# johannesschaeufele/CPUPathTrace

Hardware: AMD Instinct MI355X
Metric: Msamples/s (all bounces) (higher is better)
Workload: dtype f32

## Files before the change

cpupathtrace_amd/csrc/pt_api.cpp:

```cpp
#include "pt_host.h"

namespace pth {

thread_local std::string g_last_error;

int fail(int code, const std::string &msg) {
    g_last_error = msg;
    return code;
}

const std::string &last_error() {
    return g_last_error;
}

int device_count_quiet() {
    int n = 0;
    if(hipGetDeviceCount(&n) != hipSuccess) {
        (void)hipGetLastError();
        return 0;
    }
    return n;
}

int check_device(int device) {
// ... 367 lines not shown
            const float *sp = d->sph + 4 * static_cast<size_t>(i);
            spheres[i] = {sp[0], sp[1], sp[2], sp[3]};
            tris[PT_TRI_QUADS * (static_cast<size_t>(d->n_triangles) + 1 + i)] = spheres[i];
            sph_meta[i] = make_uint2(d->sph_material[i], s->sph_obj[i]);
        }
        std::vector<F4> pairs(4 * static_cast<size_t>(flat.n_pairs));
        std::memcpy(pairs.data(), flat.pairs.data(), flat.pairs.size() * sizeof(float));
        PT_HIP(s->pairs.upload(pairs));
        PT_HIP(s->tris.upload(tris));
        PT_HIP(s->tri_shade.upload(shade));
        PT_HIP(s->spheres.upload(spheres));
        PT_HIP(s->sph_meta.upload(sph_meta));
        s->build_ms[1] = ms_since(t_upload);
    }
    const auto t_rest = clock::now();

    std::vector<F4> materials(4 * static_cast<size_t>(d->n_materials));
    for(uint32_t i = 0; i < d->n_materials; i++) {
        const pt_material &m = d->materials[i];
        materials[4 * static_cast<size_t>(i) + 0] = {m.diffuse[0], m.diffuse[1], m.diffuse[2], m.diffuse[3]};
        materials[4 * static_cast<size_t>(i) + 1] = {m.specular[0], m.specular[1], m.specular[2], m.specular[3]};
        materials[4 * static_cast<size_t>(i) + 2] = {m.emission[0], m.emission[1], m.emission[2], m.emission[3]};
        materials[4 * static_cast<size_t>(i) + 3] = {m.ior, from_bits(static_cast<uint32_t>(m.bsdf)), from_bits(static_cast<uint32_t>(m.one_way != 0)), 0.0F};
        if(m.bsdf < PT_BSDF_LAMBERTIAN || m.bsdf > PT_BSDF_MIRROR) {
            return fail(PT_ERR_INVALID, "unknown BSDF kind");
        }
    }
    std::vector<F4> lights(2 * static_cast<size_t>(d->n_point_lights));
    for(uint32_t i = 0; i < d->n_point_lights; i++) {
        const float *p = d->light_pos + 3 * static_cast<size_t>(i);
        const float *c = d->light_spectrum + 4 * static_cast<size_t>(i);
        lights[2 * static_cast<size_t>(i) + 0] = {p[0], p[1], p[2], 0.0F};
        lights[2 * static_cast<size_t>(i) + 1] = {c[0], c[1], c[2], c[3]};
    }

    std::vector<F4> emis;
    std::vector<float> cdf;
    const float pi = static_cast<float>(M_PI);
    for(int32_t obj : dfs) {
        const uint32_t ref = leaf_ref[obj];
        const uint32_t idx = ref & PT_REF_INDEX;
        const bool is_sphere = (ref & PT_REF_SPHERE) != 0;
        const uint32_t mat = is_sphere ? d->sph_material[idx] : d->tri_material[idx];
        if(mat == PT_NO_MATERIAL) {
            continue;
        }
        const float *e = d->materials[mat].emission;
        const float emissive_power = (e[0] + e[1] + e[2]) * e[3];
        if(emissive_power <= 0.0F) {
            continue;
        }
        float area;
        if(is_sphere) {
            const float r = d->sph[4 * static_cast<size_t>(idx) + 3];
            area = 4.0F * pi * (r * r);
        }
        else {
            const float *p = d->tri_pos + 9 * static_cast<size_t>(idx);
            const Vec3 c = cross(sub(ld(p + 3), ld(p)), sub(ld(p + 6), ld(p)));
            area = std::sqrt(dot(c, c)) / 2.0F;
        }
        const float object_probability = emissive_power * area;
        if(object_probability <= 0.0F) {
            continue;
        }
        if(is_sphere) {
            const float *sp = d->sph + 4 * static_cast<size_t>(idx);
            emis.push_back({sp[0], sp[1], sp[2], sp[3]});
            emis.push_back({0.0F, 0.0F, 0.0F, 0.0F});
            emis.push_back({0.0F, from_bits(ref), 0.0F, from_bits(mat)});
        }
        else {
            const float *p = d->tri_pos + 9 * static_cast<size_t>(idx);
            emis.push_back({p[0], p[1], p[2], p[3]});
            emis.push_back({p[4], p[5], p[6], p[7]});
            emis.push_back({p[8], from_bits(ref), from_bits(d->tri_cull[idx] != 0 ? 1U : 0U), from_bits(mat)});
        }
        emis.push_back({e[0], e[1], e[2], e[3]});
        cdf.push_back(object_probability);
        s->emissive_obj.push_back(obj);
    }
    {
        float cumulative_probability = 0.0F;
        for(float &v : cdf) {
            const float probability = v;
            v += cumulative_probability;
            cumulative_probability += probability;
        }
        for(float &v : cdf) {
            v /= cumulative_probability;
        }
    }
    s->n_emissive = static_cast<uint32_t>(cdf.size());
    s->emissive_cdf = cdf;
    const int emissive_object_count = static_cast<int>(cdf.size());
    const int object_sample_count = std::min(2 + static_cast<int>(std::log10(emissive_object_count + 1)), emissive_object_count);
    if(d->n_point_lights + static_cast<uint32_t>(object_sample_count) > PT_MAX_NEE) {
        return fail(PT_ERR_UNSUPPORTED, "more than 32 light samples per path vertex (" + std::to_string(d->n_point_lights) + " point lights + " + std::to_string(object_sample_count) +
                                        " emitter samples): the visibility mask of a path vertex has 32 bits");
    }

    PT_HIP(s->materials.upload(materials));
    PT_HIP(s->lights.upload(lights));
    PT_HIP(s->emis.upload(emis));
    PT_HIP(s->emis_cdf.upload(cdf));

    const uint32_t sphere_base = d->n_triangles + 1U, leaf_count = sphere_base + d->n_spheres, pair_base = (leaf_count + 1U) & ~1U;
    if(static_cast<uint64_t>(pair_base) + n_pairs > PT_REF_INDEX) {
        return fail(PT_ERR_UNSUPPORTED, "too many records for 30-bit references");
    }
    PT_HIP(s->recs.ensure(4 * (static_cast<size_t>(pair_base) + n_pairs)));
    PT_HIP(hipMemcpyAsync(s->recs.ptr, s->tris.ptr, 4 * static_cast<size_t>(leaf_count) * sizeof(F4), hipMemcpyDeviceToDevice, s->stream));
    if(pair_base > leaf_count) {
        PT_HIP(hipMemsetAsync(s->recs.ptr + 4 * static_cast<size_t>(leaf_count), 0, 4 * sizeof(F4), s->stream));
    }
    if(n_pairs > 0) {
        PT_HIP(hipMemcpyAsync(s->recs.ptr + 4 * static_cast<size_t>(pair_base), s->pairs.ptr, 4 * static_cast<size_t>(n_pairs) * sizeof(F4), hipMemcpyDeviceToDevice, s->stream));
        PT_HIP(pt_link_records(s->stream, reinterpret_cast<float4 *>(s->recs.ptr), pair_base, n_pairs, sphere_base));
    }
    PT_HIP(hipStreamSynchronize(s->stream));
    s->tris.release();
    s->pairs.release();
    if(root_ref != PT_REF_NONE) {
        root_ref += (root_ref & PT_REF_LEAF) == 0 ? pair_base : ((root_ref & PT_REF_SPHERE) != 0 ? sphere_base : 0U);
    }

    PtDevScene &dev = s->dev;
    dev.recs = reinterpret_cast<const float4 *>(s->recs.ptr);
    dev.pairs = dev.recs + 4 * static_cast<size_t>(pair_base);
    dev.tris = dev.recs;
    dev.pair_base = pair_base;
    dev.tri_shade = reinterpret_cast<const float4 *>(s->tri_shade.ptr);
    dev.spheres = reinterpret_cast<const float4 *>(s->spheres.ptr);
    dev.sph_meta = s->sph_meta.ptr;
    dev.materials = reinterpret_cast<const float4 *>(s->materials.ptr);
    dev.lights = reinterpret_cast<const float4 *>(s->lights.ptr);
    dev.emis = reinterpret_cast<const float4 *>(s->emis.ptr);
    dev.emis_cdf = s->emis_cdf.ptr;
    for(int k = 0; k < 3; k++) {
        dev.root_lo[k] = root_lo[k];
        dev.root_hi[k] = root_hi[k];
    }
    dev.root_ref = root_ref;
    dev.n_pairs = n_pairs;
    dev.n_tris = d->n_triangles;
    dev.n_spheres = d->n_spheres;
    dev.n_lights = d->n_point_lights;
    dev.n_emis = s->n_emissive;
    dev.n_materials = d->n_materials;
    dev.n_object_samples = static_cast<uint32_t>(object_sample_count);
    const size_t small_bytes = (static_cast<size_t>(n_pairs) + pair_base) * 64;
    const int wide_word = d->n_point_lights + static_cast<uint32_t>(object_sample_count) > 8U ? 1 : 0;
    const size_t other_lds = pt_path_lds_bytes(wide_word, std::min(std::max(env_int("PT_ROWS", 4), 1), PT_MAX_ROWS), 4, 0U, 0U);
    const size_t room = other_lds < 40960 ? 40960 - other_lds : 0;
    if(small_bytes <= static_cast<size_t>(std::max(env_int("PT_LDS_SMALL_BYTES", static_cast<int>(room)), 0)) && env_int("PT_LDS_SMALL", 1) != 0) {
        dev.n_lds_pairs = n_pairs;
        dev.n_lds_tris = d->n_triangles;
    }
    else {
        dev.n_lds_pairs = 0;
        dev.n_lds_tris = 0;
    }

    int rc = setup_path(s.get());
    if(rc != PT_OK) {
        return rc;
    }
    s->build_ms[3] = ms_since(t_rest);
    if(env_int("PT_DEBUG", 0) != 0) {
        std::fprintf(stderr, "[pt] scene build (%s): %u objects, %u pair records, depth %u; host preparation %.1f ms, upload %.1f ms, device tree %.1f ms, rest %.1f ms\n",
                     s->device_built ? "device" : "host", d->n_objects, n_pairs, s->depth, s->build_ms[0], s->build_ms[1], s->build_ms[2], s->build_ms[3]);
    }
    *out = s.release();
    return PT_OK;
}

void pt_scene_destroy(pt_scene *scene) {
    if(scene == nullptr) {
        return;
    }
    (void)hipSetDevice(scene->device);
    if(scene->stream != nullptr) {
        (void)hipStreamSynchronize(scene->stream);
    }
    delete scene;
}

int pt_scene_info(const pt_scene *scene, uint64_t *n_nodes, uint32_t *depth, uint32_t *n_emissive) {
    if(scene == nullptr) {
        return fail(PT_ERR_INVALID, "null scene");
    }
    if(n_nodes != nullptr) {
        *n_nodes = scene->n_nodes;
    }
    if(depth != nullptr) {
        *depth = scene->depth;
    }
    if(n_emissive != nullptr) {
        *n_emissive = scene->n_emissive;
    }
    return PT_OK;
}

int pt_scene_emissive(const pt_scene *scene, int32_t *out_obj, float *out_cdf, uint64_t capacity, uint64_t *n_written) {
    if(scene == nullptr) {
        return fail(PT_ERR_INVALID, "null scene");
    }
    const uint64_t n = std::min<uint64_t>(scene->emissive_obj.size(), capacity);
    for(uint64_t i = 0; i < n; i++) {
        if(out_obj != nullptr) {
            out_obj[i] = scene->emissive_obj[i];
        }
        if(out_cdf != nullptr) {
            out_cdf[i] = scene->emissive_cdf[i];
        }
    }
    if(n_written != nullptr) {
        *n_written = scene->emissive_obj.size();
    }
    return PT_OK;
}

int pt_scene_bvh_dump(const pt_scene *scene, int32_t *out_obj, float *out_box, uint64_t capacity, uint64_t *n_written) {
    if(scene == nullptr || out_obj == nullptr || out_box == nullptr) {
        return fail(PT_ERR_INVALID, "null argument");
    }
    std::vector<int32_t> obj;
    std::vector<ptb::Box> box;
    if(!scene->device_built) {
        ptb::dump_preorder(scene->tree, obj, box);
    }
    else {
        const uint32_t pair_base = scene->dev.pair_base, sphere_base = scene->dev.n_tris + 1U;
        std::vector<F4> pairs(4 * static_cast<size_t>(scene->dev.n_pairs));
        if(hipSetDevice(scene->device) != hipSuccess ||
           hipMemcpy(pairs.data(), scene->dev.pairs, pairs.size() * sizeof(F4), hipMemcpyDeviceToHost) != hipSuccess) {
            return fail(PT_ERR_HIP, "downloading the pair records failed");
        }
        struct Item {
            uint32_t ref;
            ptb::Box box;
        };
        ptb::Box root;
        for(int k = 0; k < 3; k++) {
            root.lo[k] = scene->dev.root_lo[k];
            root.hi[k] = scene->dev.root_hi[k];
        }
        std::vector<Item> stack{{scene->dev.root_ref, root}};
        obj.reserve(scene->n_nodes);
        box.reserve(scene->n_nodes);
        while(!stack.empty()) {
            const Item it = stack.back();
            stack.pop_back();
            box.push_back(it.box);
            if((it.ref & PT_REF_LEAF) != 0) {
                const uint32_t idx = it.ref & PT_REF_INDEX;
                obj.push_back(static_cast<int32_t>((it.ref & PT_REF_SPHERE) != 0 ? scene->sph_obj[idx - sphere_base] : scene->tri_obj[idx]));
            }
            else {
                obj.push_back(-1);
                const float *q = &pairs[4 * static_cast<size_t>(it.ref - pair_base)].x;
                Item l, r;
                std::memcpy(&l.box, q, 24);
                std::memcpy(&r.box, q + 6, 24);
                std::memcpy(&l.ref, q + 12, 4);
                std::memcpy(&r.ref, q + 13, 4);
                stack.push_back(r);
                stack.push_back(l);
            }
        }
    }
    const uint64_t n = std::min<uint64_t>(obj.size(), capacity);
    for(uint64_t i = 0; i < n; i++) {
        out_obj[i] = obj[i];
        std::memcpy(out_box + 6 * i, &box[i], sizeof(float) * 6);
    }
    if(n_written != nullptr) {
        *n_written = obj.size();
    }
    return PT_OK;
}

int pt_intersect_batch(pt_scene *s, const float *rays, size_t n, float *out_t, int32_t *out_obj) {
    if(s == nullptr || (n > 0 && (rays == nullptr || out_t == nullptr || out_obj == nullptr))) {
        return fail(PT_ERR_INVALID, "null argument");
    }
    if(n == 0) {
        return PT_OK;
    }
    if(n > 0x7fffffffULL) {
        return fail(PT_ERR_INVALID, "too many rays in one batch");
    }
    std::lock_guard<std::mutex> lock(s->render_mutex);
    PT_HIP(hipSetDevice(s->device));
    const uint32_t n32 = static_cast<uint32_t>(n);
    {
        int rc = setup_path(s);
        if(rc != PT_OK) {
            return rc;
        }
        PtPathConfig cfg = s->path_cfg;
        PT_HIP(s->batch_rays.ensure(6 * n));
        PT_HIP(s->closest_out.ensure(n));
        PT_HIP(s->path_spill.ensure(((n + 255) / 256) * 256 * cfg.spill_depth));
        cfg.spill = s->path_spill.ptr;
        hipStream_t st = s->stream;
        PT_HIP(hipMemcpyAsync(s->batch_rays.ptr, rays, 6 * n * sizeof(float), hipMemcpyHostToDevice, st));
        pt_launch_closest(st, s->dev, s->batch_rays.ptr, n32, s->closest_out.ptr, cfg);
        PT_HIP(hipGetLastError());
        std::vector<uint2> hits(n);
        PT_HIP(hipMemcpyAsync(hits.data(), s->closest_out.ptr, n * sizeof(uint2), hipMemcpyDeviceToHost, st));
        PT_HIP(hipStreamSynchronize(st));
        for(size_t i = 0; i < n; i++) {
            const float t = from_bits(hits[i].x);
            const uint32_t ref = hits[i].y;
            out_t[i] = t;
            out_obj[i] = (t < 0.0F || ref == PT_REF_NONE) ? -1 : static_cast<int32_t>((ref & PT_REF_SPHERE) ? s->sph_obj[(ref & PT_REF_INDEX) - (s->dev.n_tris + 1U)] : s->tri_obj[ref & PT_REF_INDEX]);
        }
        return PT_OK;
    }
}

}
```

cpupathtrace_amd/csrc/pt_image.cpp:

```cpp
#include "pt_host.h"

using namespace pth;


static int post_check(int device, const float *rgba, int32_t width, int32_t height, uint32_t steps, float gamma) {
    if(width < 0 || height < 0 || (rgba == nullptr && static_cast<long long>(width) * height > 0)) {
        return fail(PT_ERR_INVALID, "bad image");
    }
    if((steps & ~(PT_POST_TONE_MAP | PT_POST_GAMMA)) != 0 || steps == 0) {
        return fail(PT_ERR_INVALID, "steps must be PT_POST_TONE_MAP and/or PT_POST_GAMMA");
    }
    if((steps & PT_POST_GAMMA) != 0 && !(gamma == gamma)) {
        return fail(PT_ERR_INVALID, "gamma is NaN");
    }
    return check_device(device);
}

extern "C" {

int pt_post_process_device(int device, float *d_rgba, int32_t width, int32_t height, uint32_t steps, float gamma, void *stream) {
    PT_TRY(post_check(device, d_rgba, width, height, steps, gamma));
    PT_HIP(hipSetDevice(device));
    static_assert(PT_POST_TONE_MAP == PT_POST_STEP_TONE_MAP && PT_POST_GAMMA == PT_POST_STEP_GAMMA, "step bits");
    PT_HIP(pt_post_run(static_cast<hipStream_t>(stream), reinterpret_cast<float4 *>(d_rgba), width, height, steps, gamma));
    return PT_OK;
}

int pt_post_process(int device, float *rgba, int32_t width, int32_t height, uint32_t steps, float gamma) {
    PT_TRY(post_check(device, rgba, width, height, steps, gamma));
    const size_t count = static_cast<size_t>(width) * static_cast<size_t>(height);
    if(count == 0) {
        return PT_OK;
    }
    PT_HIP(hipSetDevice(device));
    DevBuf<F4> frame;
    PT_HIP(frame.ensure(count));
    PT_HIP(hipMemcpy(frame.ptr, rgba, count * sizeof(F4), hipMemcpyHostToDevice));
    PT_HIP(pt_post_run(nullptr, reinterpret_cast<float4 *>(frame.ptr), width, height, steps, gamma));
    PT_HIP(hipMemcpy(rgba, frame.ptr, count * sizeof(F4), hipMemcpyDeviceToHost));
    return PT_OK;
}

}


static int features_launch(pt_scene *s, const pt_camera_params *camera, const pt_options *options, float4 *d_out) {
    PT_TRY(setup_path(s));
    PtDevCamera cam = derive_camera(camera);
    cam.aperture_kind = PT_APERTURE_NONE;
    PtPathConfig cfg = s->path_cfg;
    const size_t n = static_cast<size_t>(options->image_width) * static_cast<size_t>(options->image_height);
    PT_HIP(s->feature_spill.ensure(((n + 255) / 256) * 256 * cfg.spill_depth));
    cfg.spill = s->feature_spill.ptr;
    pt_launch_features(s->stream, s->dev, cam, options->image_width, options->image_height, d_out, cfg);
    PT_HIP(hipGetLastError());
    return PT_OK;
}

static int features_views_check(pt_scene *s, const pt_camera_params *cameras, int32_t n_views, const pt_options *options, const float *out) {
    if(n_views <= 0) {
        return fail(PT_ERR_INVALID, "a view batch needs at least one view");
    }
    if(options != nullptr && options->image_width > 0 && options->image_height > 0 &&
       static_cast<uint64_t>(n_views) * static_cast<uint64_t>(options->image_height) * static_cast<uint64_t>(options->image_width) > 0x0fffffffULL) {
        return fail(PT_ERR_INVALID, "more than 0x0fffffff pixels");
    }
    PT_TRY(check_render_args(s, cameras, options));
    if(out == nullptr) {
        return fail(PT_ERR_INVALID, "null argument");
    }
    return PT_OK;
}

int pth::features_views_launch(pt_scene *s, const pt_camera_params *cameras, int32_t n_views, const pt_options *options, float4 *d_out) {
    if(n_views == 1) {
        return features_launch(s, cameras, options, d_out);
    }
    PT_TRY(setup_path(s));
    std::vector<PtViewCamera> table(static_cast<size_t>(n_views));
    for(int32_t v = 0; v < n_views; v++) {
        table[static_cast<size_t>(v)] = PtViewCamera{derive_camera(cameras + v), {0, 0, 0}};
        table[static_cast<size_t>(v)].cam.aperture_kind = PT_APERTURE_NONE;
    }
    PT_HIP(s->feature_cams.ensure(table.size()));
    PT_HIP(hipMemcpyAsync(s->feature_cams.ptr, table.data(), table.size() * sizeof(PtViewCamera), hipMemcpyHostToDevice, s->stream));
    PT_HIP(hipStreamSynchronize(s->stream));
    PtPathConfig cfg = s->path_cfg;
    const size_t n = static_cast<size_t>(n_views) * static_cast<size_t>(options->image_width) * static_cast<size_t>(options->image_height);
    PT_HIP(s->feature_spill.ensure(((n + 255) / 256) * 256 * cfg.spill_depth));
    cfg.spill = s->feature_spill.ptr;
    pt_launch_features_views(s->stream, s->dev, s->feature_cams.ptr, n_views, options->image_width, options->image_height, d_out, cfg);
    PT_HIP(hipGetLastError());
    return PT_OK;
}

namespace pth {

DenoiseWorkspace &denoise_workspace(int device) {
    static std::mutex table_mutex;
    static std::vector<DenoiseWorkspace *> table;
    std::lock_guard<std::mutex> lock(table_mutex);
    if(static_cast<size_t>(device) >= table.size()) {
        table.resize(static_cast<size_t>(device) + 1, nullptr);
    }
    if(table[static_cast<size_t>(device)] == nullptr) {
        table[static_cast<size_t>(device)] = new DenoiseWorkspace();
    }
    return *table[static_cast<size_t>(device)];
}

template<typename T>
hipError_t regrow(T **p, size_t count) {
    if(*p != nullptr) {
        hipError_t e = hipFree(*p);
        *p = nullptr;
        if(e != hipSuccess) {
            return e;
        }
    }
    return hipMalloc(reinterpret_cast<void **>(p), std::max<size_t>(count, 1) * sizeof(T));
}

int denoise_ensure(DenoiseWorkspace &ws, size_t n, bool staged) {
    PtDenoiseScratch &d = ws.scratch;
    if(n > ws.pixels) {
        ws.pixels = 0;
        PT_HIP(regrow(&d.col[0], n));
        PT_HIP(regrow(&d.col[1], n));
        PT_HIP(regrow(&d.var[0], n));
        PT_HIP(regrow(&d.var[1], n));
        PT_HIP(regrow(&d.guide, n));
        PT_HIP(regrow(&d.grad, n));
        PT_HIP(regrow(&d.cls, n));
        ws.pixels = n;
    }
    if(staged && n > ws.staged) {
        ws.staged = 0;
        PT_HIP(regrow(&ws.in_rgba, n));
        PT_HIP(regrow(&ws.in_features, 3 * n));
        ws.staged = n;
    }
    return PT_OK;
}

int denoise_params_resolve(const pt_denoise_params *params, PtDenoiseParams *resolved) {
    pt_denoise_params p{};
    pt_denoise_params_default(&p);
    if(params != nullptr) {
        p = *params;
    }
    if(p.iterations < 0 || p.iterations > 10) {
        return fail(PT_ERR_INVALID, "iterations must be 0..10");
    }
    for(float sigma : {p.sigma_luminance, p.sigma_normal, p.sigma_depth}) {
        if(!std::isfinite(sigma) || sigma < 0.0F) {
            return fail(PT_ERR_INVALID, "sigmas must be finite and not negative");
        }
    }
    *resolved = PtDenoiseParams{p.iterations, p.sigma_luminance, p.sigma_normal, p.sigma_depth};
    return PT_OK;
}

int denoise_measured_params_resolve(const pt_denoise_measured_params *params, PtDenoiseParams *resolved, float *sigma_measured) {
    pt_denoise_measured_params p{};
    pt_denoise_measured_params_default(&p);
    if(params != nullptr) {
        p = *params;
    }
    PT_TRY(denoise_params_resolve(&p.base, resolved));
    if(!std::isfinite(p.sigma_measured) || p.sigma_measured < 0.0F) {
        return fail(PT_ERR_INVALID, "sigmas must be finite and not negative");
    }
    *sigma_measured = p.sigma_measured;
    return PT_OK;
}

}

static int denoise_views_check(int device, const void *rgba, const void *features, int32_t width, int32_t height, int32_t n_views, const pt_denoise_params *params,
                               const void *out, PtDenoiseParams *resolved) {
    if(n_views <= 0) {
        return fail(PT_ERR_INVALID, "a view batch needs at least one view");
    }
    if(width > 0 && height > 0 && static_cast<uint64_t>(n_views) * static_cast<uint64_t>(width) * static_cast<uint64_t>(height) > 0x0fffffffULL) {
        return fail(PT_ERR_INVALID, "more than 0x0fffffff pixels");
    }
    if(rgba == nullptr || features == nullptr || out == nullptr) {
        return fail(PT_ERR_INVALID, "null argument");
    }
    if(width <= 0 || height <= 0) {
        return fail(PT_ERR_INVALID, "image size must be positive");
    }
    PtDenoiseParams p{};
    PT_TRY(denoise_params_resolve(params, &p));
    PT_TRY(check_device(device));
    *resolved = p;
    return PT_OK;
}

extern "C" {

int pt_denoise_params_default(pt_denoise_params *out) {
    if(out == nullptr) {
        return fail(PT_ERR_INVALID, "null argument");
    }
    out->iterations = 5;
    out->sigma_luminance = 32.0F;
    out->sigma_normal = 128.0F;
    out->sigma_depth = 1.0F;
    return PT_OK;
}

int pt_render_features(pt_scene *s, const pt_camera_params *camera, const pt_options *options, float *out_features) {
    return pt_render_features_views(s, camera, 1, options, out_features);
}

int pt_render_features_device(pt_scene *s, const pt_camera_params *camera, const pt_options *options, float *d_out_features, void *stream) {
    return pt_render_features_views_device(s, camera, 1, options, d_out_features, stream);
}

int pt_render_features_views(pt_scene *s, const pt_camera_params *cameras, int32_t n_views, const pt_options *options, float *out_features) {
    PT_TRY(features_views_check(s, cameras, n_views, options, out_features));
    const size_t n = static_cast<size_t>(n_views) * static_cast<size_t>(options->image_width) * static_cast<size_t>(options->image_height);
    std::lock_guard<std::mutex> lock(s->render_mutex);
    PT_HIP(hipSetDevice(s->device));
    PT_HIP(s->features.ensure(3 * n));
    PT_TRY(features_views_launch(s, cameras, n_views, options, reinterpret_cast<float4 *>(s->features.ptr)));
    PT_HIP(hipMemcpyAsync(out_features, s->features.ptr, 3 * n * sizeof(F4), hipMemcpyDeviceToHost, s->stream));
    PT_HIP(hipStreamSynchronize(s->stream));
    return PT_OK;
}

int pt_render_features_views_device(pt_scene *s, const pt_camera_params *cameras, int32_t n_views, const pt_options *options, float *d_out_features, void *stream) {
    PT_TRY(features_views_check(s, cameras, n_views, options, d_out_features));
    std::lock_guard<std::mutex> lock(s->render_mutex);
    PT_HIP(hipSetDevice(s->device));
    StreamOrder order;
    PT_TRY(order.begin(stream, s->stream));
    PT_TRY(features_views_launch(s, cameras, n_views, options, reinterpret_cast<float4 *>(d_out_features)));
    PT_TRY(order.end());
    if(order.caller == nullptr) {
        PT_HIP(hipStreamSynchronize(s->stream));
    }
    return PT_OK;
}

int pt_denoise_device(int device, const float *d_rgba, const float *d_features, int32_t width, int32_t height, const pt_denoise_params *params, float *d_out_rgba,
                      void *stream) {
    return pt_denoise_views_device(device, d_rgba, d_features, width, height, 1, params, d_out_rgba, stream);
}

int pt_denoise(int device, const float *rgba, const float *features, int32_t width, int32_t height, const pt_denoise_params *params, float *out_rgba) {
    return pt_denoise_views(device, rgba, features, width, height, 1, params, out_rgba);
}

int pt_denoise_views_device(int device, const float *d_rgba, const float *d_features, int32_t width, int32_t height, int32_t n_views, const pt_denoise_params *params,
                            float *d_out_rgba, void *stream) {
    PtDenoiseParams p{};
    PT_TRY(denoise_views_check(device, d_rgba, d_features, width, height, n_views, params, d_out_rgba, &p));
    const size_t n = static_cast<size_t>(n_views) * static_cast<size_t>(width) * static_cast<size_t>(height);
    DenoiseWorkspace &ws = denoise_workspace(device);
    std::lock_guard<std::mutex> lock(ws.mutex);
    PT_HIP(hipSetDevice(device));
    PT_TRY(denoise_ensure(ws, n, false));
    hipStream_t st = static_cast<hipStream_t>(stream);
    PT_HIP(pt_denoise_views_run(st, reinterpret_cast<const float4 *>(d_rgba), reinterpret_cast<const float4 *>(d_features), nullptr, width, height, n_views, p,
                                ws.scratch, reinterpret_cast<float4 *>(d_out_rgba)));
    PT_HIP(hipStreamSynchronize(st));
    return PT_OK;
}

int pt_denoise_views(int device, const float *rgba, const float *features, int32_t width, int32_t height, int32_t n_views, const pt_denoise_params *params,
                     float *out_rgba) {
    PtDenoiseParams p{};
    PT_TRY(denoise_views_check(device, rgba, features, width, height, n_views, params, out_rgba, &p));
    const size_t n = static_cast<size_t>(n_views) * static_cast<size_t>(width) * static_cast<size_t>(height);
    DenoiseWorkspace &ws = denoise_workspace(device);
    std::lock_guard<std::mutex> lock(ws.mutex);
    PT_HIP(hipSetDevice(device));
    PT_TRY(denoise_ensure(ws, n, true));
    PT_HIP(hipMemcpy(ws.in_rgba, rgba, n * sizeof(F4), hipMemcpyHostToDevice));
    PT_HIP(hipMemcpy(ws.in_features, features, 3 * n * sizeof(F4), hipMemcpyHostToDevice));
    PT_HIP(pt_denoise_views_run(nullptr, ws.in_rgba, ws.in_features, nullptr, width, height, n_views, p, ws.scratch, ws.in_rgba));
    PT_HIP(hipMemcpy(out_rgba, ws.in_rgba, n * sizeof(F4), hipMemcpyDeviceToHost));
    return PT_OK;
}

static int denoise_measured_check(int device, const void *rgba, const void *features, const void *variance, int32_t width, int32_t height,
                                  const pt_denoise_measured_params *params, const void *out, PtDenoiseParams *resolved, float *sigma_measured) {
    if(rgba == nullptr || features == nullptr || variance == nullptr || out == nullptr) {
        return fail(PT_ERR_INVALID, "null argument");
    }
    if(width <= 0 || height <= 0) {
        return fail(PT_ERR_INVALID, "image size must be positive");
    }
    if(static_cast<uint64_t>(width) * static_cast<uint64_t>(height) > 0x0fffffffULL) {
        return fail(PT_ERR_INVALID, "more than 0x0fffffff pixels");
    }
    PT_TRY(denoise_measured_params_resolve(params, resolved, sigma_measured));
    return check_device(device);
}

int pt_denoise_measured_params_default(pt_denoise_measured_params *out) {
    if(out == nullptr) {
        return fail(PT_ERR_INVALID, "null argument");
    }
    pt_denoise_params_default(&out->base);
    out->sigma_measured = 16.0F;
    return PT_OK;
}

int pt_denoise_measured_device(int device, const float *d_rgba, const float *d_features, const float *d_variance, const int32_t *d_mask, int32_t width,
                               int32_t height, const pt_denoise_measured_params *params, float *d_out_rgba, void *stream) {
    PtDenoiseParams p{};
    float sigma_measured = 0.0F;
    PT_TRY(denoise_measured_check(device, d_rgba, d_features, d_variance, width, height, params, d_out_rgba, &p, &sigma_measured));
    const size_t n = static_cast<size_t>(width) * static_cast<size_t>(height);
    DenoiseWorkspace &ws = denoise_workspace(device);
    std::lock_guard<std::mutex> lock(ws.mutex);
    PT_HIP(hipSetDevice(device));
    PT_TRY(denoise_ensure(ws, n, false));
    hipStream_t st = static_cast<hipStream_t>(stream);
    PT_HIP(pt_denoise_measured_run(st, reinterpret_cast<const float4 *>(d_rgba), reinterpret_cast<const float4 *>(d_features),
                                   reinterpret_cast<const float4 *>(d_variance), d_mask, width, height, p, sigma_measured, ws.scratch,
                                   reinterpret_cast<float4 *>(d_out_rgba)));
    PT_HIP(hipStreamSynchronize(st));
    return PT_OK;
}

int pt_denoise_measured(int device, const float *rgba, const float *features, const float *variance, const int32_t *mask, int32_t width, int32_t height,
                        const pt_denoise_measured_params *params, float *out_rgba) {
    PtDenoiseParams p{};
    float sigma_measured = 0.0F;
    PT_TRY(denoise_measured_check(device, rgba, features, variance, width, height, params, out_rgba, &p, &sigma_measured));
    const size_t n = static_cast<size_t>(width) * static_cast<size_t>(height);
    DenoiseWorkspace &ws = denoise_workspace(device);
    std::lock_guard<std::mutex> lock(ws.mutex);
    PT_HIP(hipSetDevice(device));
    PT_TRY(denoise_ensure(ws, n, true));
    if(n > ws.staged_variance) {
        ws.staged_variance = 0;
        PT_HIP(regrow(&ws.in_variance, n));
        ws.staged_variance = n;
    }
    DevBuf<int32_t> d_mask;
    if(mask != nullptr) {
        PT_HIP(d_mask.ensure(n));
        PT_HIP(hipMemcpy(d_mask.ptr, mask, n * sizeof(int32_t), hipMemcpyHostToDevice));
    }
    PT_HIP(hipMemcpy(ws.in_rgba, rgba, n * sizeof(F4), hipMemcpyHostToDevice));
    PT_HIP(hipMemcpy(ws.in_features, features, 3 * n * sizeof(F4), hipMemcpyHostToDevice));
    PT_HIP(hipMemcpy(ws.in_variance, variance, n * sizeof(F4), hipMemcpyHostToDevice));
    PT_HIP(pt_denoise_measured_run(nullptr, ws.in_rgba, ws.in_features, ws.in_variance, mask != nullptr ? d_mask.ptr : nullptr, width, height, p, sigma_measured,
                                   ws.scratch, ws.in_rgba));
    PT_HIP(hipMemcpy(out_rgba, ws.in_rgba, n * sizeof(F4), hipMemcpyDeviceToHost));
    return PT_OK;
}

}


struct pt_temporal {
    int device = 0;
    int32_t width = 0, height = 0;
    PtTemporalParams params{};
    std::mutex mutex;
    DevBuf<float4> col[2], guide, col_hist, pos[2], nrm[2], in_rgba, in_features;
    DevBuf<float> var[2];
    DevBuf<float2> grad, moments[2];
    DevBuf<int32_t> len[2];
    DevBuf<uint32_t> cls[2];
    int cur = 0;
    bool has_prev = false;
    PtDevCamera prev{};
    float prev_rows[3][3] = {};
    PtDevCamera pending{};
    float pending_rows[3][3] = {};
};

namespace {

int temporal_camera(const pt_camera_params *c, int32_t height, PtDevCamera *cam, float rows[3][3], float *footprint) {
    const float scalars[] = {c->origin[0], c->origin[1], c->origin[2], c->look_at[0], c->look_at[1], c->look_at[2], c->up[0], c->up[1], c->up[2],
                             c->focal_length, c->height, c->aspect_ratio};
    for(float v : scalars) {
        if(!std::isfinite(v)) {
            return fail(PT_ERR_INVALID, "camera: non-finite parameter");
        }
    }
    *cam = derive_camera(c);
    const Vec3 f = ld(cam->forward), u = ld(cam->up), r = ld(cam->right);
    Vec3 row[3] = {cross(u, r), cross(r, f), cross(f, u)};
// ... 217 lines not shown
```

cpupathtrace_amd/csrc/pt_kernels.h:

```cpp
#ifndef PT_KERNELS_H
#define PT_KERNELS_H

#include <hip/hip_runtime.h>

#include "pt_types.h"

#define PT_F_DONE 1u
#define PT_F_IN_FLIGHT 2u
#define PT_F_HAS_EXT 4u
#define PT_F_COLLECTED 8u
#define PT_F_PIXEL 16u
#define PT_F_SAFE 64u
#define PT_F_OVERLAP 32u

#define PT_DEST_SHADOW 0x80000000u
#define PT_DEST_NULL 0xffffffffu


#define PT_LDS_TABLE_MAX 16
#define PT_LDS_TABLE_BYTES (PT_LDS_TABLE_MAX * (4 + 64 + 96 + 64))
#define PT_WALK_SAVE_WORDS 17
#define PT_MAX_ROWS 8
#define PT_F_STREAM 128u

#define PT_PLANE_RAY_O 0
#define PT_PLANE_RAY_D 1
#define PT_PLANE_PD 2
#define PT_PLANE_ENGINE 3
#define PT_PLANE_SPECTRUM 4
#define PT_PLANE_OUT 5
#define PT_PLANE_RECT 6
#define PT_SLOT_PLANES 7
struct PtSlots {
    uint32_t total;
    float4 *state;
    float4 *nee;
    uint32_t *nee_mask;
    uint32_t *cost;
    PtEstimator *est;
    PtCandidate *cand;
};

struct PtStreams {
    uint32_t n;
    const int4 *rect;
    uint64_t *rng;
    const int4 *tiles;
    const uint32_t *tile_offset;
    uint32_t n_tiles;
    uint64_t base_seed;
    uint32_t first_total;
    uint32_t first_lanes;
    uint32_t first_shift;
    uint32_t n_waves, first_spread;
    uint32_t tiles_per_row, chunks_per_tile;
    uint32_t *next;
    uint32_t *tile_left;
    uint32_t *tiles_done;
    uint32_t *cost;
    const uint32_t *place;
    const uint32_t *cancel;
    const uint2 *todo;
    const PtParkRecord *park_in;
    PtParkRecord *park_out;
    uint32_t *park_count;
    uint32_t park_cap;
    uint32_t *status;
    int32_t yield_at;
    uint32_t n_views, view_height;
    const PtViewCamera *views;
    const uint64_t *view_seed;
};

struct PtLocalQueue {
    float4 *ray_o;
    float4 *ray_d;
    uint32_t cap;
};

struct PtPathConfig {
    int grid;
    int rows;
    int slots_per_wave;
    int wide;
    int stack_lds;
    uint32_t spill_depth;
    uint2 *spill;
    uint32_t *walk_save;
    size_t lds_bytes;
    int in_lds;
    int refill_idle;
    int min_ready;
    int ready_shift;
    int pass_q_low;
    int early_ready;
    int compact_passes;
    int debug_lanes;
    int burst_steps;
    int first_lanes;
    int leaf_min;
    unsigned long long *wave_counters;
};

struct PtPathArgs {
    PtDevScene sc;
    PtDevCamera cam;
    PtDevOptions opt;
    PtSlots S;
    PtStreams T;
    PtLocalQueue Q;
    int rows, slots_per_wave, refill_idle, min_ready, burst_steps, leaf_min, ready_shift, pass_q_low, early_ready, compact_passes, debug_lanes;
    uint2 *spill;
    uint32_t spill_depth;
    uint32_t save_stride;
    uint32_t *walk_save;
    float4 *image;
    PtDevCounters *counters;
    unsigned long long *wave_counters;
};

void pt_launch_path(hipStream_t stream, const PtDevScene &scene, const PtDevCamera &camera, const PtDevOptions &options, PtSlots slots, PtStreams streams,
                    PtLocalQueue queue, const PtPathConfig &cfg, float4 *image, PtDevCounters *counters, PtPathArgs *host_args, PtPathArgs *d_args);
struct PtNoiseRule {
    PtDevOptions opt;
    float target;
    float floor;
};
int pt_launch_frame_compact(hipStream_t stream, const uint2 *todo, uint32_t n, uint32_t *status, const PtParkRecord *parked, uint2 *todo_out, uint32_t *block_counts,
                            unsigned long long *result, int32_t target, const PtParkRecord *park_in, PtParkRecord *park_out, uint32_t *park_count, uint32_t park_cap,
                            const PtNoiseRule &noise, int resort);
#define PT_NOISE_SUMMARY_WORDS 68
int pt_launch_frame_rate(hipStream_t stream, const uint2 *todo, uint32_t n, const PtParkRecord *park, const int4 *tiles, const uint32_t *tile_offset, uint32_t n_tiles,
                         int32_t width, const PtNoiseRule &noise, uint2 *out, uint32_t *summary);
int pt_launch_frame_noise_base(hipStream_t stream, float *map, const uint8_t *cover, uint32_t n_pixels);
int pt_launch_frame_noise_scatter(hipStream_t stream, const uint2 *rated, uint32_t n, float *map);
int pt_launch_frame_variance(hipStream_t stream, const uint2 *todo, uint32_t n, const PtParkRecord *park, const int4 *tiles, const uint32_t *tile_offset,
                             uint32_t n_tiles, int32_t width, const PtDevOptions &opt, float4 *out_var, int32_t *out_at);
int pt_launch_frame_variance_scatter(hipStream_t stream, const float4 *var, const int32_t *at, uint32_t n, float4 *map);
int pt_launch_frame_gather(hipStream_t stream, const uint2 *todo, uint32_t n, uint32_t n_parked, const PtParkRecord *park, const int4 *tiles,
                           const uint32_t *tile_offset, uint32_t n_tiles, int32_t width, float4 *out_rgba, int2 *out_at);
int pt_launch_frame_preview_base(hipStream_t stream, float4 *view, int32_t *samples, const uint8_t *cover, uint32_t n_pixels);
int pt_launch_frame_scatter(hipStream_t stream, const float4 *rgba, const int2 *at, uint32_t n, float4 *view, int32_t *samples);
int pt_path_blocks_per_cu(const PtPathConfig &cfg);
size_t pt_path_lds_bytes(int wide, int rows, int stack_lds, uint32_t n_lds_pairs, uint32_t n_lds_leaf_records);
int pt_path_stack_lds(int in_lds, size_t lds_bytes_with_default_window);
int pt_launch_replay(hipStream_t stream, const PtDevScene &scene, const PtLocalQueue &Q, uint32_t n_logs, uint32_t parts, int waves_per_simd, const PtPathConfig &cfg,
                     uint2 *spill, unsigned long long *out);
void pt_launch_closest(hipStream_t stream, const PtDevScene &scene, const float *rays6, uint32_t n, uint2 *out, const PtPathConfig &cfg);
void pt_launch_features(hipStream_t stream, const PtDevScene &scene, const PtDevCamera &camera, int32_t width, int32_t height, float4 *out, const PtPathConfig &cfg);
void pt_launch_features_views(hipStream_t stream, const PtDevScene &scene, const PtViewCamera *views, int32_t n_views, int32_t width, int32_t height, float4 *out,
                              const PtPathConfig &cfg);
void pt_launch_steptime(hipStream_t stream, const PtDevScene &scene, const float *rays6, uint32_t n, uint32_t lanes_per_wave, uint4 *out, uint2 *spill, uint32_t spill_depth, int flags);


#endif
```

cpupathtrace_amd/csrc/pt_path.hip:

```cpp
#include <type_traits>

#include "pt_device.h"
#include "pt_kernels.h"
#include "pt_shading.h"

using namespace ptd;

namespace {

typedef float f4v __attribute__((ext_vector_type(4)));
typedef float f2v __attribute__((ext_vector_type(2)));
typedef unsigned int u2v __attribute__((ext_vector_type(2)));
typedef const f4v __attribute__((address_space(3))) *lds_f4_cptr;
typedef const f4v __attribute__((address_space(1))) *glb_f4_cptr;
typedef u2v __attribute__((address_space(3))) *lds_u2_ptr;
typedef u2v __attribute__((address_space(1))) *glb_u2_ptr;
typedef unsigned int __attribute__((address_space(3))) *lds_u32_ptr;
typedef const PtPathArgs __attribute__((address_space(4))) *args_c4;

template<bool IN_LDS>
struct RecPtr {
    typedef glb_f4_cptr type;
};
template<>
struct RecPtr<true> {
    typedef lds_f4_cptr type;
};

PT_D float4 to_f4(f4v v) {
    return make_float4(v.x, v.y, v.z, v.w);
}

struct RootBox {
    float lo[3], hi[3];
    uint32_t ref;
};

#define PT_REF_POPPING 0xfffffffeu
struct Walk {
    V3 o, d, inv;
    f2v o_xy, o_zx, o_yz, i_xy, i_zx, i_yz;
    float thr;
    uint32_t dest;
    float best_t;
    uint32_t best_ref;
    float t_max;
    float t_lim;
    uint32_t cur;
    uint32_t sp;
    bool occluded;

    PT_D void pack() {
        o_xy = (f2v){o.x, o.y};
        o_zx = (f2v){o.z, o.x};
        o_yz = (f2v){o.y, o.z};
        i_xy = (f2v){inv.x, inv.y};
        i_zx = (f2v){inv.z, inv.x};
        i_yz = (f2v){inv.y, inv.z};
    }
    PT_D void set_t_max(float t) {
        t_max = t;
        t_lim = t > 0.0f ? __uint_as_float(__float_as_uint(t) - 1u) : -1.0f;
    }
};

#ifdef PT_STEP_STAMPS
#define PT_STAMP(k)                                                      \
    do {                                                                 \
        const unsigned long long now_ = __builtin_amdgcn_s_memtime();     \
        asm volatile("s_waitcnt lgkmcnt(0)" ::: "memory");               \
        stamp_acc[k] += now_ - stamp_last;                               \
        stamp_last = now_;                                               \
    } while(0)
#else
#define PT_STAMP(k) do { } while(0)
#endif

template<int STACK_LDS, bool IN_LDS>
struct Tracer {
    static_assert((STACK_LDS & (STACK_LDS - 1)) == 0, "the stack window is indexed with a mask");
#ifdef PT_STEP_STAMPS
    mutable unsigned long long stamp_acc[8] = {0, 0, 0, 0, 0, 0, 0, 0}, stamp_last = 0;
#endif
    typedef typename RecPtr<IN_LDS>::type rec_ptr;
    rec_ptr recs;
    lds_u2_ptr stack_l;
    glb_u2_ptr my_spill;

    struct Rec {
        f4v r0, r1, r2, r3;
    };
    PT_D void fetch(uint32_t cur, Rec &R) const {
        rec_ptr p = recs + 4 * (size_t)(cur & PT_REF_INDEX);
        R.r0 = p[0];
        R.r1 = p[1];
        R.r2 = p[2];
        R.r3 = p[3];
    }
    static PT_D void whole(const Rec &R) {
        asm volatile("" ::"v"(R.r0), "v"(R.r1), "v"(R.r2), "v"(R.r3));
    }

    static PT_D unsigned long long node_lanes(uint32_t cur) { return __builtin_amdgcn_uicmp(cur, 0x40000000u, 36); }
    static PT_D unsigned long long slow_lanes(uint32_t cur) { return __builtin_amdgcn_uicmp(cur + 1u, 0x40000000u, 34); }

    PT_D void start(Walk &w, Rec &R, const RootBox &root, float4 ro, float4 rd) const {
        w.o = v3(ro.x, ro.y, ro.z);
        w.d = v3(rd.x, rd.y, rd.z);
        w.thr = ro.w;
        w.dest = __float_as_uint(rd.w);
        w.inv = slab_inverse(w.d);
        w.pack();
        w.best_ref = PT_REF_NONE;
        w.best_t = -1.0f;
        w.set_t_max(FLT_MAX);
        uint32_t sent_ref, sent_t;
        asm volatile("v_mov_b32 %0, -1\n\tv_mov_b32 %1, -1.0" : "=v"(sent_ref), "=v"(sent_t));
        const u2v sentinel = {sent_ref, sent_t};
        stack_l[0] = sentinel;
        w.sp = 1;
        w.occluded = false;
        w.cur = PT_REF_NONE;
        if(root.ref != PT_REF_NONE) {
            const float t_root = slab_walk(ld3(root.lo), ld3(root.hi), w.o, w.inv);
            if(t_root >= 0.0f) {
                w.cur = root.ref;
                fetch(w.cur, R);
            }
        }
    }

    PT_D void node_step(Walk &w, Rec &R, unsigned long long node_mask, unsigned long long deep_mask) const {
        if(!__builtin_amdgcn_inverse_ballot_w64(node_mask)) {
            return;
        }
#ifdef PT_STEP_STAMPS
        asm volatile("s_waitcnt vmcnt(0)" ::: "memory");
#endif
        PT_STAMP(2);
        whole(R);
        const f4v q0 = R.r0, q1 = R.r1, q2 = R.r2;
        const uint32_t sp = w.sp;
        const u2v top = stack_l[((sp - 1u) & (uint32_t)(STACK_LDS - 1)) * 256u];
        const f2v a0 = ((f2v){q0.x, q0.y} - w.o_xy) * w.i_xy;
        const f2v a1 = ((f2v){q0.z, q0.w} - w.o_zx) * w.i_zx;
        const f2v a2 = ((f2v){q1.x, q1.y} - w.o_yz) * w.i_yz;
        const f2v a3 = ((f2v){q1.z, q1.w} - w.o_xy) * w.i_xy;
        const f2v a4 = ((f2v){q2.x, q2.y} - w.o_zx) * w.i_zx;
        const f2v a5 = ((f2v){q2.z, q2.w} - w.o_yz) * w.i_yz;
        const float l1 = a0.x, l2 = a1.y, l3 = a0.y, l4 = a2.x, l5 = a1.x, l6 = a2.y;
        const float r1 = a3.x, r2 = a4.y, r3 = a3.y, r4 = a5.x, r5 = a4.x, r6 = a5.y;
        const float l_min = __builtin_fmaxf(__builtin_fmaxf(__builtin_fminf(l1, l2), __builtin_fminf(l3, l4)), __builtin_fminf(l5, l6));
        const float l_max = __builtin_fminf(__builtin_fminf(__builtin_fmaxf(l1, l2), __builtin_fmaxf(l3, l4)), __builtin_fmaxf(l5, l6));
        const float r_min = __builtin_fmaxf(__builtin_fmaxf(__builtin_fminf(r1, r2), __builtin_fminf(r3, r4)), __builtin_fminf(r5, r6));
        const float r_max = __builtin_fminf(__builtin_fminf(__builtin_fmaxf(r1, r2), __builtin_fmaxf(r3, r4)), __builtin_fmaxf(r5, r6));
        const float left_t = __builtin_fmaxf(l_min, 0.0f), right_t = __builtin_fmaxf(r_min, 0.0f);
        const float inf = __builtin_inff();
        const float t_lim = w.t_lim;
        const float tl = left_t <= __builtin_fminf(l_max, t_lim) ? left_t : inf;
        const float tr = right_t <= __builtin_fminf(r_max, t_lim) ? right_t : inf;
        const bool left_first = tl < tr;
        const uint32_t left_ref = __float_as_uint(R.r3.x), right_ref = __float_as_uint(R.r3.y);
        const uint32_t near_ref = left_first ? left_ref : right_ref;
        const float near_t = __builtin_fminf(tl, tr), far_t = __builtin_fmaxf(tl, tr);
        const u2v far = {left_first ? right_ref : left_ref, __float_as_uint(far_t)};
        const bool both = far_t < inf, entered = near_t < inf;
        const uint32_t slot = (sp & (uint32_t)(STACK_LDS - 1)) * 256u;
        if(deep_mask == 0ULL) {
            stack_l[slot] = far;
        }
        else if(both) {
            if(sp >= (uint32_t)STACK_LDS) {
                my_spill[sp - STACK_LDS] = stack_l[slot];
            }
            stack_l[slot] = far;
        }
        const uint32_t popped = __uint_as_float(top.y) <= t_lim ? top.x : PT_REF_POPPING;
        const uint32_t next = entered ? near_ref : popped;
        w.sp = entered ? sp + (both ? 1u : 0u) : sp - 1u;
        w.cur = next;
        asm volatile("" ::"v"(w.sp), "v"(w.cur));
        PT_STAMP(3);
        if(next < PT_REF_POPPING) {
            fetch(next, R);
        }
        if(deep_mask != 0ULL) {
            if(!entered & (sp - 1u >= (uint32_t)STACK_LDS)) {
                stack_l[((sp - 1u) & (uint32_t)(STACK_LDS - 1)) * 256u] = my_spill[sp - 1u - STACK_LDS];
            }
        }
        PT_STAMP(4);
    }

    PT_D void slow_step(Walk &w, Rec &R, unsigned long long leaf_mask, uint32_t &n_leaves) const {
        uint32_t cur = w.cur;
        bool need_pop = cur == PT_REF_POPPING;
        bool moved = false;
        if(leaf_mask != 0ULL) {
            n_leaves += (uint32_t)__popcll(leaf_mask);
            if(__builtin_amdgcn_inverse_ballot_w64(leaf_mask)) {
                const float4 q0 = to_f4(R.r0), q1 = to_f4(R.r1), q2 = to_f4(R.r2);
                float t_leaf;
                if(cur & PT_REF_SPHERE) {
                    t_leaf = sphere_intersect(v3(q0.x, q0.y, q0.z), q0.w, w.o, w.d);
                }
                else {
                    const TriRec tr = tri_unpack(q0, q1, q2);
                    t_leaf = tri_intersect(tr.a, tr.ab, tr.ac, (tr.obj_cull >> 31) != 0, w.o, w.d);
                }
                need_pop = true;
                if(t_leaf >= 0.0f) {
                    if((w.dest & PT_DEST_SHADOW) && t_leaf < w.thr) {
                        w.occluded = true;
                        need_pop = false;
                    }
                    else {
                        if(w.best_ref == PT_REF_NONE || !(w.best_t < t_leaf)) {
                            w.best_t = t_leaf;
                            w.best_ref = cur;
                        }
                        w.set_t_max(fmin_std(w.t_max, t_leaf));
                    }
                }
                cur = PT_REF_NONE;
            }
        }
        if(__ballot(need_pop) != 0ULL) {
            uint32_t sp = w.sp;
            const float t_max = w.t_max;
            while(__ballot(need_pop) != 0ULL) {
                if(need_pop) {
                    sp--;
                    const uint32_t slot = (sp & (uint32_t)(STACK_LDS - 1)) * 256u;
                    const u2v e = stack_l[slot];
                    if(sp >= (uint32_t)STACK_LDS) {
                        stack_l[slot] = my_spill[sp - STACK_LDS];
                    }
                    if(__uint_as_float(e.y) < t_max) {
                        cur = e.x;
                        need_pop = false;
                        moved = true;
                    }
                }
            }
            w.sp = sp;
        }
        w.cur = cur;
        if(moved & (cur != PT_REF_NONE)) {
            fetch(cur, R);
        }
    }

    PT_D bool step(Walk &w, Rec &R, int leaf_min, uint32_t &n_nodes, uint32_t &n_leaves) const {
        PT_STAMP(0);
        PT_STAMP(7);
        const unsigned long long nodes = node_lanes(w.cur), slow = slow_lanes(w.cur);
        if((nodes | slow) == 0ULL) {
            return false;
        }
        PT_STAMP(1);
        if(nodes != 0ULL) {
            n_nodes += (uint32_t)__popcll(nodes);
            node_step(w, R, nodes, nodes & __builtin_amdgcn_uicmp(w.sp, (uint32_t)STACK_LDS, 35));
        }
        PT_STAMP(5);
        if(slow != 0ULL && (nodes == 0ULL || __popcll(slow) >= leaf_min)) {
            slow_step(w, R, slow & __builtin_amdgcn_uicmp(w.cur, PT_REF_POPPING, 36), n_leaves);
        }
        PT_STAMP(6);
        return true;
    }
};

template<bool WIDE>
struct SlotWord {
    typedef uint32_t T;
    typedef uint32_t __attribute__((address_space(3))) *lds_ptr;
    static constexpr uint32_t j_mask = 7u;
    static PT_D uint32_t vis(T w) { return w & 0xffu; }
    static PT_D uint32_t pending(T w) { return (w >> 8) & 0xffu; }
    static PT_D uint32_t flags(T w) { return (w >> 16) & 0xffu; }
    static PT_D T one_ray() { return 0x100u; }
    static PT_D T make(uint32_t flags, uint32_t rays, uint32_t vis, uint32_t waiting) { return (waiting << 24) | (flags << 16) | (rays << 8) | vis; }
    static PT_D uint32_t waiting(T w, const PtSlots &, size_t) { return w >> 24; }
    static PT_D void keep_waiting(const PtSlots &, size_t, uint32_t) {}
};
template<>
struct SlotWord<true> {
    typedef unsigned long long T;
    typedef unsigned long long __attribute__((address_space(3))) *lds_ptr;
    static constexpr uint32_t j_mask = 31u;
    static PT_D uint32_t vis(T w) { return (uint32_t)w; }
    static PT_D uint32_t pending(T w) { return (uint32_t)(w >> 32) & 0xffu; }
    static PT_D uint32_t flags(T w) { return (uint32_t)(w >> 40) & 0xffu; }
    static PT_D T one_ray() { return 1ULL << 32; }
    static PT_D T make(uint32_t flags, uint32_t rays, uint32_t vis, uint32_t) { return ((T)flags << 40) | ((T)rays << 32) | (T)vis; }
    static PT_D uint32_t waiting(T, const PtSlots &S, size_t p) { return S.nee_mask[p]; }
    static PT_D void keep_waiting(const PtSlots &S, size_t p, uint32_t mask) { S.nee_mask[p] = mask; }
};

#define PT_F_VIEW_RAY 256u
#define PT_DEST_SLOT_MASK 0xffffu
#define PT_NO_SLOT 0xffffffffu
#define PT_DEST_J_SHIFT 16

struct WaveCtx {
    uint32_t q_head;
    uint32_t q_count;
    uint32_t n_dead;
    bool pool_empty;
    uint32_t first_rows;
    uint32_t first_base;
    uint32_t wave;
};

PT_D void tile_stream(const PtStreams &T, uint32_t i, int4 &rect, uint64_t &rng, uint32_t &tile) {
    uint32_t lo = 0, hi = T.n_tiles;
    while(hi - lo > 1) {
        const uint32_t mid = (lo + hi) / 2;
        if(T.tile_offset[mid] <= i) {
            lo = mid;
        }
        else {
            hi = mid;
        }
    }
    const int4 t = T.tiles[lo];
    const uint32_t k = i - T.tile_offset[lo];
    const int32_t x = t.x + (int32_t)(k % (uint32_t)t.z), y = t.y + (int32_t)(k / (uint32_t)t.z);
    rect = make_int4(x, y, 1, 1);
    uint64_t base_seed = T.base_seed;
    int32_t seed_y = y;
    if(T.n_views > 1) {
        const uint32_t view = (uint32_t)y / T.view_height;
        base_seed = T.view_seed[view];
        seed_y = y - (int32_t)(view * T.view_height);
    }
    const uint64_t seed = pixel_seed(base_seed, x, seed_y);
    rng = seed ^ (~seed << 32);
    tile = lo;
}

struct EmisLds {
    const float __attribute__((address_space(3))) *cdf_l;
    lds_f4_cptr rec_l;
    lds_f4_cptr light_l;
    PT_D float cdf(int i) const { return cdf_l[i]; }
    PT_D float4 rec(int i, int k) const { return to_f4(rec_l[4 * i + k]); }
    PT_D V3 tri_normal_at(int i, uint32_t, V3 pos) const {
        uint32_t mat_unused;
        return tri_shade_normal(light_l + 6 * i, pos, mat_unused);
    }
};
struct ShadeTables {
    EmisLds emis;
    lds_f4_cptr materials_l;
    bool emis_in_lds, materials_in_lds;
};

PT_D void copy_words(void *dst, const void *src, uint32_t n) {
    uint32_t *d = static_cast<uint32_t *>(dst);
    const uint32_t *s = static_cast<const uint32_t *>(src);
#pragma unroll 1
    for(uint32_t i = 0; i < n; i++) {
        d[i] = s[i];
    }
}

PT_D uint32_t closed_candidate_words(int32_t n_candidates) {
    return (uint32_t)(n_candidates < PT_MAX_CANDIDATES ? n_candidates : PT_MAX_CANDIDATES) * (uint32_t)(sizeof(PtCandidate) / 4);
}

PT_D void park_stream(const PtStreams &T, const PtSlots &S, uint32_t p, uint32_t stream, uint64_t rng, int32_t cursor, bool have_pixel) {
    uint32_t status = PT_STREAM_FINISHED;
    if(have_pixel) {
        status = PT_STREAM_UNTOUCHED;
        const PtEstimator *e = S.est + p;
        if(e->pixel_sample > 0 || cursor > 0) {
            const uint32_t k = atomicAdd(T.park_count, 1u);
            if(k < T.park_cap) {
                PtParkRecord *rec = T.park_out + k;
                rec->stream = stream;
                rec->cursor = cursor;
                rec->rng[0] = (uint32_t)rng;
                rec->rng[1] = (uint32_t)(rng >> 32);
                copy_words(&rec->est, e, (uint32_t)(sizeof(PtEstimator) / 4));
                copy_words(rec->cand, S.cand + (size_t)p * PT_MAX_CANDIDATES, closed_candidate_words(e->n_candidates));
                status = PT_STREAM_PARKED + k;
            }
        }
    }
    T.status[stream] = status;
}

template<typename V>
PT_D V *slot_plane(const PtSlots &S, uint32_t k, uint32_t p) {
    return reinterpret_cast<V *>(reinterpret_cast<char *>(S.state) + (k * S.total + p) * (uint32_t)sizeof(float4));
}

template<bool WIDE>
PT_D void shade_row(const PtDevScene &sc, const PtDevCamera &cam, const PtDevOptions &opt, const PtSlots &S, const PtStreams &T, const PtLocalQueue &Q,
                    WaveCtx &ctx, uint32_t row, uint32_t ls_in, uint32_t lane, uint32_t slot_base, size_t queue_base, typename SlotWord<WIDE>::lds_ptr word_l, lds_u2_ptr hit_l,
                    float4 *__restrict__ image, PtDevCounters *counters, const ShadeTables &tb, bool stop, uint32_t &n_samples, uint32_t &n_vertices) {
    const bool have_slot = ls_in != PT_NO_SLOT;
    const uint32_t ls = have_slot ? ls_in : 0u;
    const uint32_t p = slot_base + ls;
    const unsigned long long lt = (1ULL << lane) - 1ULL;
    const uint32_t n_light_samples = sc.n_lights + sc.n_object_samples;
    typedef SlotWord<WIDE> SW;
    const typename SW::T word = word_l[ls];
    uint32_t flags = SW::flags(word);
    const uint32_t vis_bits = SW::vis(word);
    bool ready = have_slot && !(flags & PT_F_DONE) && SW::pending(word) == 0;
    if(__ballot(ready) == 0ULL) {
        return;
    }

    {
        const bool want = ready && !(flags & PT_F_STREAM);
        const unsigned long long want_mask = __ballot(want);
        if(want_mask != 0ULL) {
            uint32_t base = T.n;
            uint32_t mine;
            if((ctx.first_rows >> row) & 1u) {
                ctx.first_rows &= ~(1u << row);
                base = ctx.first_base + row * 64u;
                mine = base + lane;
                if(T.place != nullptr) {
                    base = 0;
                    mine = T.place[ctx.first_base + ls];
                }
                else if(T.first_spread) {
                    const uint32_t g = T.first_lanes, q = row * (64u / g) + lane / g;
                    uint32_t chunk = q * T.n_waves + ctx.wave;
                    if(T.tiles_per_row != 0) {
                        const uint32_t per_tile = T.chunks_per_tile * (64u / g), pieces = (T.first_total / T.n_waves) / g;
                        const uint32_t tile = chunk / per_tile, sub = chunk % per_tile;
                        const uint32_t step = T.tiles_per_row >= pieces ? T.tiles_per_row / pieces : 1u;
                        const uint32_t tx = (tile % T.tiles_per_row + q * T.first_shift * step) % T.tiles_per_row, ty = tile / T.tiles_per_row;
                        chunk = (ty * T.tiles_per_row + tx) * per_tile + sub;
                    }
                    base = 0;
                    mine = chunk * g + lane % g;
                }
            }
            else {
                ctx.pool_empty = ctx.pool_empty || stop;
                if(!ctx.pool_empty) {
                    if(lane == 0) {
                        base = T.first_total + atomicAdd(T.next, (uint32_t)__popcll(want_mask));
                    }
                    base = __builtin_amdgcn_readfirstlane(base);
                }
                mine = base + (uint32_t)__popcll(want_mask & lt);
                if(base >= T.n || base + (uint32_t)__popcll(want_mask) > T.n) {
                    ctx.pool_empty = true;
                }
            }
            const bool got = want && base < T.n && mine < T.n;
            if(got) {
                int4 rc;
                uint64_t r;
                uint32_t tile = 0;
                uint32_t park = PT_NO_PARK;
                int32_t cursor0 = 0;
                if(T.rect != nullptr) {
                    rc = T.rect[mine];
                    r = T.rng[mine];
                }
                else {
                    if(T.todo != nullptr) {
                        const uint2 entry = T.todo[mine];
                        mine = entry.x;
                        park = entry.y;
                    }
                    tile_stream(T, mine, rc, r, tile);
                }
                flags = PT_F_STREAM;
                if(park != PT_NO_PARK) {
                    const PtParkRecord *rec = T.park_in + park;
                    r = (uint64_t)rec->rng[0] | ((uint64_t)rec->rng[1] << 32);
                    cursor0 = rec->cursor;
                    copy_words(S.est + p, &rec->est, (uint32_t)(sizeof(PtEstimator) / 4));
                    copy_words(S.cand + (size_t)p * PT_MAX_CANDIDATES, rec->cand, closed_candidate_words(rec->est.n_candidates));
                    flags = PT_F_STREAM | PT_F_PIXEL | (estimator_safe_to_overlap(S.est[p], opt) ? PT_F_SAFE : 0u);
                }
                *slot_plane<int4>(S, PT_PLANE_RECT, p) = rc;
                *slot_plane<uint4>(S, PT_PLANE_ENGINE, p) = make_uint4((uint32_t)r, (uint32_t)(r >> 32), (uint32_t)cursor0, mine);
                if(T.cost != nullptr) {
                    __hip_atomic_store(&S.cost[p], 0u, __ATOMIC_RELAXED, __HIP_MEMORY_SCOPE_AGENT);
                }
            }
            else if(want) {
                flags = PT_F_DONE;
                ready = false;
                word_l[ls] = SW::make(PT_F_DONE, 0u, 0u, 0u);
            }
            ctx.n_dead += (uint32_t)__popcll(__ballot(want && !got));
        }
    }
    const bool alive = ready;
    uint32_t lane_samples = 0;

    uint64_t rng = 0;
    C4 out = c4(0, 0, 0, 0), spectrum = c4(1, 1, 1, 1);
    V3 ro = v3(0, 0, 0), rd = v3(0, 0, 1);
    float contribution_unweighted = 1.0f;
    double divisor = 1.0, bounce_pd = 1.0;
    int path_length = 0;
    bool shade_vertex = false;
    bool start_sample = false;
    float hit_t = -1.0f;
    uint32_t hit_ref = PT_REF_NONE;
    int4 rect = make_int4(0, 0, 0, 0);
    int32_t cursor = 0;
    uint32_t stream = 0;
    bool stream_finished = false;
    bool stream_abandoned = false;

    if(alive) {
        const uint4 engine = *slot_plane<uint4>(S, PT_PLANE_ENGINE, p);
        rng = (uint64_t)engine.x | ((uint64_t)engine.y << 32);
        cursor = (int32_t)engine.z;
        stream = engine.w;
        rect = *slot_plane<int4>(S, PT_PLANE_RECT, p);
        if(flags & PT_F_IN_FLIGHT) {
            const float4 out4 = *slot_plane<float4>(S, PT_PLANE_OUT, p);
            uint32_t mask = SW::waiting(word, S, p);
            const uint32_t lit = mask & vis_bits;
            float4 nee0 = make_float4(0, 0, 0, 0), nee1 = make_float4(0, 0, 0, 0);
            if(lit & 1u) {
                nee0 = S.nee[p];
            }
            if(lit & 2u) {
                nee1 = S.nee[S.total + p];
            }
            const float4 o4 = *slot_plane<float4>(S, PT_PLANE_RAY_O, p), d4 = *slot_plane<float4>(S, PT_PLANE_RAY_D, p);
            const float4 spectrum4 = *slot_plane<float4>(S, PT_PLANE_SPECTRUM, p);
            const double2 pd_in = *slot_plane<double2>(S, PT_PLANE_PD, p);
            uint32_t warm = 0;
            if(flags & PT_F_HAS_EXT) {
                const u2v h = hit_l[ls];
                hit_t = __uint_as_float(h.x);
                hit_ref = h.y;
                if(!(hit_t < 0.0f) && !(hit_ref & PT_REF_SPHERE)) {
                    warm = *reinterpret_cast<const uint32_t *>(sc.tri_shade + 8 * (size_t)(hit_ref & PT_REF_INDEX));
                }
            }
            out = c4(out4);
            if(lit & 1u) {
                out = out + c4(nee0);
            }
            if(lit & 2u) {
                out = out + c4(nee1);
            }
            mask >>= 2;
            for(uint32_t j = 2; mask != 0; j++, mask >>= 1) {
                if((mask & 1u) && ((vis_bits >> j) & 1u)) {
                    out = out + c4(S.nee[(size_t)j * S.total + p]);
                }
            }
            asm volatile("" ::"v"(warm));
            if(flags & PT_F_OVERLAP) {
                PtEstimator e = S.est[p];
                out.a = 1.0f;
// ... 33 lines not shown
                flags &= ~(PT_F_IN_FLIGHT | PT_F_HAS_EXT | PT_F_COLLECTED | PT_F_SAFE);
                if((flags & PT_F_PIXEL) && estimator_safe_to_overlap(e, opt)) {
                    flags |= PT_F_SAFE;
                }
                start_sample = true;
            }
            else {
                ro = v3(o4.x, o4.y, o4.z);
                rd = v3(d4.x, d4.y, d4.z);
                contribution_unweighted = o4.w;
                spectrum = c4(spectrum4);
                divisor = pd_in.x;
                bounce_pd = pd_in.y;
                path_length = __float_as_int(d4.w);
            }
        }
        else {
            start_sample = true;
        }
    }

    bool emit_ext = false;
    Ray ext;
    ext.o = v3(0, 0, 0);
    ext.d = v3(0, 0, 1);
    auto shoot_camera = [&](const int4 rc, int32_t cur) {
        const int32_t px = rc.x + cur % rc.z, py = rc.y + cur / rc.z;
        const float one_half = 1.0f / 2.0f;
        const float x_camera = 2 * (((float)px + one_half) / (float)opt.image_width - one_half);
        float y_camera = 2 * (((float)py + one_half) / (float)opt.image_height - one_half);
        y_camera = -y_camera;
        return camera_shoot(cam, x_camera, y_camera, opt.pixel_width, opt.pixel_height, rng);
    };
    const bool batch = T.n_views > 1;
    if(start_sample) {
        bool have_pixel = false;
        while(cursor < rect.z * rect.w) {
            if(!(flags & PT_F_PIXEL)) {
                PtEstimator e;
                estimator_reset(e, opt);
                S.est[p] = e;
                flags = (flags | PT_F_PIXEL) & ~PT_F_SAFE;
                if(estimator_safe_to_overlap(e, opt)) {
                    flags |= PT_F_SAFE;
                }
                if(opt.max_sample_count <= 0) {
                    const int32_t px = rect.x + cursor % rect.z, py = rect.y + cursor / rect.z;
                    image[(size_t)py * opt.image_width + px] = make_float4(0.0f, 0.0f, 0.0f, 0.0f);
                    cursor++;
                    flags &= ~PT_F_PIXEL;
                    continue;
                }
            }
            have_pixel = true;
            break;
        }
        const bool yield = T.yield_at != 0 && have_pixel && S.est[p].pixel_sample >= T.yield_at;
        if(!have_pixel || stop || yield) {
            stream_finished = !have_pixel;
            stream_abandoned = have_pixel;
            if(T.status != nullptr) {
                park_stream(T, S, p, stream, rng, cursor, have_pixel);
            }
            flags = 0;
        }
        else {
            if(batch) {
                flags |= PT_F_VIEW_RAY;
                ext.o = v3(0, 0, 0);
                ext.d = v3(0, 0, 1);
            }
            else {
                ext = shoot_camera(rect, cursor);
            }
            emit_ext = true;
            out = c4(0, 0, 0, 0);
            spectrum = c4(1, 1, 1, 1);
            contribution_unweighted = 1.0f;
            divisor = 1.0;
            bounce_pd = 1.0;
            path_length = 0;
            flags |= PT_F_IN_FLIGHT | PT_F_HAS_EXT;
        }
    }
    {
        const unsigned long long fin_mask = __ballot(stream_finished);
        if(fin_mask != 0ULL) {
            if(stream_finished) {
                const uint32_t si = stream;
                if(T.rng != nullptr) {
                    T.rng[si] = rng;
                }
                if(T.cost != nullptr) {
                    T.cost[si] = __hip_atomic_load(&S.cost[p], __ATOMIC_RELAXED, __HIP_MEMORY_SCOPE_AGENT);
                }
                if(T.tile_left != nullptr) {
                    int4 rc_unused;
                    uint64_t r_unused;
                    uint32_t tile = 0;
                    tile_stream(T, si, rc_unused, r_unused, tile);
                    if(atomicSub(&T.tile_left[tile], 1u) == 1u) {
                        __hip_atomic_fetch_add(T.tiles_done, 1u, __ATOMIC_RELAXED, __HIP_MEMORY_SCOPE_SYSTEM);
                    }
                }
            }
            if(lane == 0) {
                atomicAdd(&counters->streams_done, (unsigned long long)__popcll(fin_mask));
            }
        }
        if(stop || T.yield_at != 0) {
            const unsigned long long drop_mask = __ballot(stream_abandoned);
            if(lane == 0 && drop_mask != 0ULL) {
                atomicAdd(&counters->streams_abandoned, (unsigned long long)__popcll(drop_mask));
            }
        }
    }

    V3 pos = v3(0, 0, 0), n = v3(0, 1, 0);
    Material mat;
    mat.bsdf = 0;
    bool do_bounce = false;
    float bounce_probability = 1.0f;
    bool want_nee = false;
    bool safe_overlap = false;
    if(shade_vertex) {
        path_length++;
        flags |= PT_F_COLLECTED;
        pos = ro + rd * hit_t;
        uint32_t material_index;
        n = object_normal(sc, hit_ref, pos, material_index);
        mat = tb.materials_in_lds ? material_load(tb.materials_l, material_index) : material_load(sc.materials, material_index);

        out = out + (spectrum * mat.emission) / (float)(divisor * bounce_pd);

        bounce_probability = path_length <= 4 ? 1.0f : 0.1f + 0.1f * fmin_std(contribution_unweighted * get_contribution(spectrum), 1.0f);
        do_bounce = rng_uniform01(rng) < bounce_probability;
        want_nee = mat.bsdf == 0 && n_light_samples > 0;
        safe_overlap = (flags & PT_F_SAFE) != 0 && !stop;
        emit_ext = do_bounce || safe_overlap;
    }

    uint32_t tail = ctx.q_head + ctx.q_count;
    const unsigned long long ext_mask = __ballot(emit_ext);
    const uint32_t ext_pos = tail + (uint32_t)__popcll(ext_mask & lt);
    tail += (uint32_t)__popcll(ext_mask);
    ctx.q_count += (uint32_t)__popcll(ext_mask);
    auto ring = [&](uint32_t i) -> size_t { return queue_base + (i >= Q.cap ? i - Q.cap : i); };

    uint32_t nee_out_mask = 0;
    uint32_t vis_init = 0;
    uint32_t n_rays = 0;
    const float epsilon = opt.epsilon;
    for(uint32_t j = 0; j < n_light_samples; j++) {
        bool need_ray = false;
        float4 so = make_float4(0, 0, 0, 0), sd = make_float4(0, 0, 0, 0);
        if(shade_vertex) {
            V3 light_pos;
            C4 light_spectrum;
            float lpd;
            bool valid;
            if(j < sc.n_lights) {
                const float4 lp = sc.lights[2 * j];
                light_pos = v3(lp.x, lp.y, lp.z);
                light_spectrum = c4(sc.lights[2 * j + 1]);
                lpd = 1.0f;
                valid = true;
            }
            else {
                valid = tb.emis_in_lds ? sample_emissive(sc, tb.emis, pos, rng, light_pos, light_spectrum, lpd)
                                       : sample_emissive(sc, EmisGlobal{sc}, pos, rng, light_pos, light_spectrum, lpd);
            }
            if(valid && want_nee) {
                const V3 to_light = light_pos - pos;
                const V3 light_dir = normalize(to_light);
                float shading_factor, shadow_ray_pd;
                const C4 base_spectrum = bsdf_spectrum(mat, rd, light_dir, n, light_spectrum, true, shading_factor, shadow_ray_pd);
                if(shadow_ray_pd > 0.0f) {
                    const C4 combined = (base_spectrum * shading_factor) * spectrum;
                    const C4 weighed = combined / (float)(divisor * bounce_pd * lpd * shadow_ray_pd);
                    if(!(weighed.r == 0.0f && weighed.g == 0.0f && weighed.b == 0.0f)) {
                        S.nee[(size_t)j * S.total + p] = f4(weighed);
                        nee_out_mask |= 1u << j;
                        const float threshold = len(to_light) - epsilon;
                        if(threshold <= 0.0f) {
                            vis_init |= 1u << j;
                        }
                        else {
                            need_ray = true;
                            const V3 o2 = pos + light_dir * epsilon;
                            so = make_float4(o2.x, o2.y, o2.z, threshold);
                            sd = make_float4(light_dir.x, light_dir.y, light_dir.z, __uint_as_float(PT_DEST_SHADOW | (j << PT_DEST_J_SHIFT) | ls));
                        }
                    }
                }
            }
        }
        const unsigned long long ray_mask = __ballot(need_ray);
        if(ray_mask != 0ULL) {
            if(need_ray) {
                const size_t at = ring(tail + (uint32_t)__popcll(ray_mask & lt));
                Q.ray_o[at] = so;
                Q.ray_d[at] = sd;
                n_rays++;
            }
            tail += (uint32_t)__popcll(ray_mask);
            ctx.q_count += (uint32_t)__popcll(ray_mask);
        }
    }

    if(shade_vertex) {
        bool cancel_ext = false;
        if(!do_bounce) {
        }
        else {
            bounce_pd *= bounce_probability;
            if(bounce_pd <= 1E-20) {
                cancel_ext = true;
            }
            else {
                float ray_factor, ray_pd;
                const Ray next_ray = bsdf_propagate(mat, rd, pos, n, epsilon, rng, ray_factor, ray_pd);
                divisor *= ray_pd;
                divisor /= ray_factor;
                contribution_unweighted *= ray_factor;
                float shading_factor, shading_pd;
                const C4 shaded = bsdf_spectrum(mat, rd, next_ray.d, n, spectrum, false, shading_factor, shading_pd);
                divisor *= shading_pd;
                divisor /= shading_factor;
                contribution_unweighted *= shading_factor;
                spectrum = shaded;
                if(divisor <= 1E-20) {
                    cancel_ext = true;
                }
                else {
                    ext = next_ray;
                }
            }
        }
        const bool path_ends = !do_bounce || cancel_ext;
        if(path_ends && safe_overlap) {
            if(batch) {
                flags |= PT_F_VIEW_RAY;
                ext.o = v3(0, 0, 0);
                ext.d = v3(0, 0, 1);
            }
            else {
                ext = shoot_camera(rect, cursor);
            }
            spectrum = c4(1, 1, 1, 1);
            contribution_unweighted = 1.0f;
            divisor = 1.0;
            bounce_pd = 1.0;
            path_length = 0;
            flags |= PT_F_OVERLAP;
        }
        else if(path_ends && emit_ext) {
            Q.ray_d[ring(ext_pos)] = make_float4(0.0f, 0.0f, 0.0f, __uint_as_float(PT_DEST_NULL));
            emit_ext = false;
        }
        if(emit_ext) {
            flags |= PT_F_HAS_EXT;
        }
        else {
            flags &= ~PT_F_HAS_EXT;
        }
    }

    if(flags & PT_F_VIEW_RAY) {
        flags &= ~PT_F_VIEW_RAY;
        const int32_t px = rect.x + cursor % rect.z, row = rect.y + cursor / rect.z;
        const uint32_t view = (uint32_t)row / (uint32_t)opt.image_height;
        const int32_t py = row - (int32_t)(view * (uint32_t)opt.image_height);
        const float one_half = 1.0f / 2.0f;
        const float x_camera = 2 * (((float)px + one_half) / (float)opt.image_width - one_half);
        float y_camera = 2 * (((float)py + one_half) / (float)opt.image_height - one_half);
        y_camera = -y_camera;
        ext = camera_shoot_lane(T.views[view].cam, x_camera, y_camera, opt.pixel_width, opt.pixel_height, rng);
    }

    if(emit_ext) {
        const size_t at = ring(ext_pos);
        Q.ray_o[at] = make_float4(ext.o.x, ext.o.y, ext.o.z, 0.0f);
        Q.ray_d[at] = make_float4(ext.d.x, ext.d.y, ext.d.z, __uint_as_float(ls));
        n_rays++;
    }
    if(alive) {
        word_l[ls] = SW::make(flags, n_rays, vis_init, nee_out_mask);
        SW::keep_waiting(S, p, nee_out_mask);
        *slot_plane<uint3>(S, PT_PLANE_ENGINE, p) = make_uint3((uint32_t)rng, (uint32_t)(rng >> 32), (uint32_t)cursor);
        if(flags & PT_F_IN_FLIGHT) {
            *slot_plane<float4>(S, PT_PLANE_RAY_O, p) = make_float4(ext.o.x, ext.o.y, ext.o.z, contribution_unweighted);
            *slot_plane<float4>(S, PT_PLANE_RAY_D, p) = make_float4(ext.d.x, ext.d.y, ext.d.z, __int_as_float(path_length));
            *slot_plane<float4>(S, PT_PLANE_SPECTRUM, p) = f4(spectrum);
            *slot_plane<float4>(S, PT_PLANE_OUT, p) = f4(out);
            *slot_plane<double2>(S, PT_PLANE_PD, p) = make_double2(divisor, bounce_pd);
        }
    }
    n_samples += (uint32_t)__popcll(__ballot(lane_samples & 1u)) + 2u * (uint32_t)__popcll(__ballot((lane_samples & 2u) != 0u));
    n_vertices += (uint32_t)__popcll(__ballot(shade_vertex));
}


#define PT_PATH_STACK_LDS 8
#define PT_PATH_STACK_LDS_SMALL 4
#ifndef PT_COST_LDS_BYTES
#define PT_COST_LDS_BYTES 1024
#endif
#ifndef PT_PATH_WAVES
#define PT_PATH_WAVES 4
#endif

PT_D uint32_t lane_afresh() {
    uint32_t l;
    asm volatile("v_mbcnt_lo_u32_b32 %0, -1, 0\n\tv_mbcnt_hi_u32_b32 %0, -1, %0" : "=v"(l));
    return l;
}

template<bool WIDE, bool IN_LDS, int STACK_LDS>
__global__ __launch_bounds__(256, PT_PATH_WAVES) void pt_path_kernel(const PtPathArgs *__restrict__ args) {
    typedef SlotWord<WIDE> SW;
    const args_c4 A4 = (args_c4)args;
    const PtPathArgs *A = (const PtPathArgs *)A4;
    const int rows = A->rows, slots_per_wave = A->slots_per_wave, refill_idle = A->refill_idle, min_ready = A->min_ready, burst_steps = A->burst_steps,
              leaf_min = A->leaf_min, ready_shift = A->ready_shift, pass_q_low = A->early_ready > 0 ? A->pass_q_low : 0, early_ready = A->early_ready;
    const unsigned long long lane_cap = A->debug_lanes >= 64 ? ~0ULL : ((1ULL << A->debug_lanes) - 1ULL);
    PtLocalQueue Q = A->Q;
    RootBox root;
    root.ref = A->sc.root_ref;
    for(int k = 0; k < 3; k++) {
        root.lo[k] = A->sc.root_lo[k];
        root.hi[k] = A->sc.root_hi[k];
    }
    extern __shared__ __align__(16) unsigned char lds_raw[];
    const int tid = threadIdx.x;
    uint32_t lane = (uint32_t)tid & 63u;
    const uint32_t wave_in_block = __builtin_amdgcn_readfirstlane((uint32_t)tid >> 6);
    const uint32_t wave = blockIdx.x * 4u + wave_in_block;
    const uint32_t n_slots = (uint32_t)rows * 64u;
    unsigned char *at = lds_raw;
    const lds_u2_ptr stack_base = (lds_u2_ptr)reinterpret_cast<uint2 *>(at) + wave_in_block * 64u;
    at += (size_t)STACK_LDS * 256 * sizeof(uint2);
    lds_u2_ptr hit_l = (lds_u2_ptr)reinterpret_cast<uint2 *>(at) + wave_in_block * n_slots;
    at += (size_t)4 * n_slots * sizeof(uint2);
    typename SW::lds_ptr word_l = (typename SW::lds_ptr)reinterpret_cast<typename SW::T *>(at) + wave_in_block * n_slots;
    at += (size_t)4 * n_slots * sizeof(typename SW::T);
    float *cdf_l = reinterpret_cast<float *>(at);
    at += (size_t)PT_LDS_TABLE_MAX * sizeof(float);
    float4 *emis_l = reinterpret_cast<float4 *>(at);
    at += (size_t)PT_LDS_TABLE_MAX * 4 * sizeof(float4);
    float4 *light_l = reinterpret_cast<float4 *>(at);
    at += (size_t)PT_LDS_TABLE_MAX * 6 * sizeof(float4);
    float4 *materials_l = reinterpret_cast<float4 *>(at);
    at += (size_t)PT_LDS_TABLE_MAX * 4 * sizeof(float4);
    typedef uint32_t __attribute__((address_space(3))) *lds_u32_ptr;
    const lds_u32_ptr born_base = (lds_u32_ptr)reinterpret_cast<uint32_t *>(at) + wave_in_block * 64u;
    lds_u32_ptr born_l = born_base + lane;
    typedef unsigned char __attribute__((address_space(3))) *lds_u8_ptr;
    lds_u8_ptr list_l = (lds_u8_ptr)reinterpret_cast<unsigned char *>(at) + wave_in_block * 256u;
    at += (size_t)PT_COST_LDS_BYTES;
    float4 *lds_recs = reinterpret_cast<float4 *>(at);
    const bool cost_on = PT_COST_LDS_BYTES != 0 && A->T.cost != nullptr;
    uint32_t *const slot_cost = A->S.cost;

    ShadeTables tb;
    tb.emis.cdf_l = (const float __attribute__((address_space(3))) *)cdf_l;
    tb.emis.rec_l = (lds_f4_cptr)emis_l;
    tb.emis.light_l = (lds_f4_cptr)light_l;
    tb.materials_l = (lds_f4_cptr)materials_l;
    {
        const uint32_t n_emis = A->sc.n_emis, n_materials = A->sc.n_materials;
        tb.emis_in_lds = n_emis > 0 && n_emis <= PT_LDS_TABLE_MAX;
        tb.materials_in_lds = n_materials > 0 && n_materials <= PT_LDS_TABLE_MAX;
        if(tb.emis_in_lds) {
            const float4 *src_emis = A->sc.emis, *src_shade = A->sc.tri_shade;
            const float *src_cdf = A->sc.emis_cdf;
            for(uint32_t i = tid; i < n_emis; i += 256) {
                cdf_l[i] = src_cdf[i];
            }
            for(uint32_t i = tid; i < 4 * n_emis; i += 256) {
                emis_l[i] = src_emis[i];
            }
            for(uint32_t i = tid; i < 6 * n_emis; i += 256) {
                const uint32_t ref = __float_as_uint(src_emis[4 * (i / 6) + 2].y);
                light_l[i] = (ref & PT_REF_SPHERE) ? make_float4(0, 0, 0, 0) : src_shade[8 * (size_t)(ref & PT_REF_INDEX) + i % 6];
            }
        }
        if(tb.materials_in_lds) {
            const float4 *src_materials = A->sc.materials;
            for(uint32_t i = tid; i < 4 * n_materials; i += 256) {
                materials_l[i] = src_materials[i];
            }
        }
    }

    if(IN_LDS) {
        const uint32_t n_lds_quads = 4u * (A->sc.pair_base + A->sc.n_pairs);
        const float4 *src_recs = A->sc.recs;
        for(uint32_t i = tid; i < n_lds_quads; i += 256) {
            lds_recs[i] = src_recs[i];
        }
    }
    for(uint32_t i = lane; i < n_slots; i += 64) {
        word_l[i] = i < (uint32_t)slots_per_wave ? (typename SW::T)0 : SW::make(PT_F_DONE, 0u, 0u, 0u);
    }
    __syncthreads();

    Tracer<STACK_LDS, IN_LDS> tr;
    if(IN_LDS) {
        tr.recs = (typename RecPtr<IN_LDS>::type)(lds_f4_cptr)lds_recs;
    }
    else {
        tr.recs = (typename RecPtr<IN_LDS>::type)(glb_f4_cptr)A->sc.recs;
    }
    auto bind_lane = [&](const PtPathArgs *B, uint32_t l) {
        lane = l;
        tr.stack_l = stack_base + l;
        tr.my_spill = (glb_u2_ptr)(B->spill + ((size_t)wave * 64 + l) * B->spill_depth);
        born_l = born_base + l;
    };

    const size_t slot_base = (size_t)wave * n_slots;
    const size_t queue_base = (size_t)wave * Q.cap;
    WaveCtx ctx;
    ctx.q_head = 0;
    ctx.q_count = 0;
    ctx.n_dead = n_slots - (uint32_t)slots_per_wave;
    ctx.pool_empty = false;
    ctx.first_rows = (1u << rows) - 1u;
    ctx.first_base = wave * (uint32_t)slots_per_wave;
    ctx.wave = wave;

    bool active = false;
    Walk w;
    w.o = v3(0, 0, 0);
    w.d = v3(0, 0, 1);
    w.inv = v3(0, 0, 0);
    w.pack();
    w.thr = 0.0f;
    w.dest = 0;
    w.best_t = 0.0f;
    w.best_ref = PT_REF_NONE;
    w.set_t_max(FLT_MAX);
    w.cur = PT_REF_NONE;
    w.sp = 0;
    w.occluded = false;
    typename Tracer<STACK_LDS, IN_LDS>::Rec rec;
    rec.r0 = rec.r1 = rec.r2 = rec.r3 = (f4v){0.0f, 0.0f, 0.0f, 0.0f};
    float4 win_o = make_float4(0, 0, 0, 0), win_d = make_float4(0, 0, 0, __uint_as_float(PT_DEST_NULL));
    uint32_t n_nodes = 0, n_leaves = 0, n_rays = 0, n_shadow = 0, n_samples = 0, n_vertices = 0;
    uint32_t w_steps = 0, w_passes = 0;
#ifdef PT_PATH_TIMING
    unsigned long long t_shade = 0, t_burst = 0;
    const unsigned long long t_begin = __builtin_amdgcn_s_memtime();
#endif

    bool want_pass = false;
    for(;;) {
        if(want_pass) {
            want_pass = false;
            w_passes++;
#ifdef PT_PATH_TIMING
            const unsigned long long t_pass = __builtin_amdgcn_s_memtime();
#endif
            size_t pass_offset = 0;
            asm volatile("" : "+s"(pass_offset));
            const PtPathArgs *P = (const PtPathArgs *)(args_c4)((const char __attribute__((address_space(4))) *)A4 + pass_offset);
            uint32_t *const walk_save = P->walk_save;
            const size_t save_stride = P->save_stride;
            const uint32_t lane_s = lane_afresh();

            {
                uint32_t *sv = walk_save + (size_t)wave * 64 + lane_s;
                const size_t st = save_stride;
                sv[0 * st] = __float_as_uint(w.o.x);
                sv[1 * st] = __float_as_uint(w.o.y);
                sv[2 * st] = __float_as_uint(w.o.z);
                sv[3 * st] = __float_as_uint(w.d.x);
                sv[4 * st] = __float_as_uint(w.d.y);
                sv[5 * st] = __float_as_uint(w.d.z);
                sv[6 * st] = __float_as_uint(w.thr);
                sv[7 * st] = w.dest;
                sv[8 * st] = __float_as_uint(w.best_t);
                sv[9 * st] = w.best_ref;
                sv[10 * st] = __float_as_uint(w.t_max);
                sv[11 * st] = w.cur;
                sv[12 * st] = w.sp | (w.occluded ? 0x80000000u : 0u);
                sv[13 * st] = n_nodes;
                sv[14 * st] = n_leaves;
                sv[15 * st] = n_rays;
                sv[16 * st] = n_shadow;
            }
            uint32_t n_listed = 0;
            bool compact = false;
            if(PT_COST_LDS_BYTES >= 1024 && !cost_on && P->compact_passes != 0 && rows > 1 && rows <= 4 && ctx.first_rows == 0u) {
                uint32_t rows_used = 0;
                for(uint32_t r = 0; r < (uint32_t)rows; r++) {
                    const typename SW::T word = word_l[r * 64 + lane_s];
                    const bool is_ready = !(SW::flags(word) & PT_F_DONE) && SW::pending(word) == 0;
                    const unsigned long long m = __ballot(is_ready);
                    if(is_ready) {
                        list_l[n_listed + (uint32_t)__popcll(m & ((1ULL << lane_s) - 1ULL))] = (unsigned char)(r * 64 + lane_s);
                    }
                    n_listed += (uint32_t)__popcll(m);
                    rows_used += m != 0ULL ? 1u : 0u;
                }
                compact = (n_listed + 63u) / 64u < rows_used;
                __builtin_amdgcn_fence(__ATOMIC_ACQ_REL, "workgroup");
            }
            const uint32_t n_chunks = compact ? (n_listed + 63u) / 64u : (uint32_t)rows;
            uint32_t stop_word = 0;
            if(P->T.cancel != nullptr) {
                stop_word = __hip_atomic_load(P->T.cancel, __ATOMIC_RELAXED, __HIP_MEMORY_SCOPE_SYSTEM);
            }
            const bool stop = __builtin_amdgcn_readfirstlane(stop_word) != 0u;
#pragma unroll 1
            for(uint32_t k = 0; k < n_chunks; k++) {
                uint32_t ls = k * 64u + lane_s;
                if(compact) {
                    ls = ls < n_listed ? (uint32_t)list_l[ls] : PT_NO_SLOT;
                }
                shade_row<WIDE>(P->sc, P->cam, P->opt, P->S, P->T, P->Q, ctx, k, ls, lane_s, (uint32_t)slot_base, queue_base, word_l, hit_l, P->image, P->counters, tb, stop, n_samples, n_vertices);
            }
            __builtin_amdgcn_fence(__ATOMIC_ACQ_REL, "workgroup");
            __builtin_amdgcn_s_waitcnt(0);
            {
                asm volatile("" : "+s"(pass_offset));
                const PtPathArgs *R = (const PtPathArgs *)(args_c4)((const char __attribute__((address_space(4))) *)A4 + pass_offset);
                const uint32_t *sv = R->walk_save + (size_t)wave * 64 + lane_afresh();
                const size_t st = R->save_stride;
                w.o = v3(__uint_as_float(sv[0 * st]), __uint_as_float(sv[1 * st]), __uint_as_float(sv[2 * st]));
                w.d = v3(__uint_as_float(sv[3 * st]), __uint_as_float(sv[4 * st]), __uint_as_float(sv[5 * st]));
                w.inv = slab_inverse(w.d);
                w.pack();
                w.thr = __uint_as_float(sv[6 * st]);
                w.dest = sv[7 * st];
                w.best_t = __uint_as_float(sv[8 * st]);
                w.best_ref = sv[9 * st];
                w.set_t_max(__uint_as_float(sv[10 * st]));
                w.cur = sv[11 * st];
                const uint32_t packed = sv[12 * st];
                w.sp = packed & 0x7fffffffu;
                w.occluded = (packed >> 31) != 0;
                n_nodes = sv[13 * st];
                n_leaves = sv[14 * st];
                n_rays = sv[15 * st];
                n_shadow = sv[16 * st];
            }
#ifdef PT_PATH_TIMING
            t_shade += __builtin_amdgcn_s_memtime() - t_pass;
#endif
            win_o = make_float4(0, 0, 0, 0);
            win_d = make_float4(0, 0, 0, __uint_as_float(PT_DEST_NULL));
            const uint32_t lane_w = lane_afresh();
            if(lane_w < ctx.q_count) {
                uint32_t i = ctx.q_head + lane_w;
                i = i >= Q.cap ? i - Q.cap : i;
                win_o = Q.ray_o[queue_base + i];
                win_d = Q.ray_d[queue_base + i];
            }
            rec.r0 = rec.r1 = rec.r2 = rec.r3 = (f4v){0.0f, 0.0f, 0.0f, 0.0f};
                    if(active && w.cur < PT_REF_POPPING) {
                tr.fetch(w.cur, rec);
            }
        }

        {
            size_t bind_offset = 0;
            asm volatile("" : "+s"(bind_offset));
            bind_lane((const PtPathArgs *)(args_c4)((const char __attribute__((address_space(4))) *)A4 + bind_offset), lane_afresh());
        }
        bool finished = false;
        for(;;) {
            if(active && w.cur == PT_REF_NONE) {
                const uint32_t ls = w.dest & PT_DEST_SLOT_MASK;
                if(w.dest & PT_DEST_SHADOW) {
                    const uint32_t j = (w.dest >> PT_DEST_J_SHIFT) & SW::j_mask;
                    __hip_atomic_fetch_add(&word_l[ls], (typename SW::T)(w.occluded ? 0u : (1u << j)) - SW::one_ray(), __ATOMIC_RELAXED, __HIP_MEMORY_SCOPE_WORKGROUP);
                }
                else {
                    const u2v h = {__float_as_uint(w.best_ref == PT_REF_NONE ? -1.0f : w.best_t), w.best_ref};
                    hit_l[ls] = h;
                    __hip_atomic_fetch_add(&word_l[ls], (typename SW::T)0 - SW::one_ray(), __ATOMIC_RELAXED, __HIP_MEMORY_SCOPE_WORKGROUP);
                }
                if(cost_on) {
                    __hip_atomic_fetch_add(&slot_cost[slot_base + ls], w_steps - *born_l, __ATOMIC_RELAXED, __HIP_MEMORY_SCOPE_AGENT);
                }
                active = false;
            }

            const unsigned long long idle_mask = __ballot(!active) & lane_cap;
            const uint32_t n_idle = (uint32_t)__popcll(idle_mask);
            if(n_idle >= (uint32_t)refill_idle) {
                if(ctx.q_count <= (uint32_t)pass_q_low && ctx.n_dead < n_slots) {
                    uint32_t n_ready = 0;
                    for(uint32_t r = 0; r < (uint32_t)rows; r++) {
                        const typename SW::T word = word_l[r * 64 + lane];
                        n_ready += (uint32_t)__popcll(__ballot(!(SW::flags(word) & PT_F_DONE) && SW::pending(word) == 0));
                    }
                    const uint32_t live_share = (n_slots - ctx.n_dead) >> ready_shift;
                    const uint32_t need = live_share < (uint32_t)min_ready ? (live_share > 1u ? live_share : 1u) : (uint32_t)min_ready;
                    if(ctx.q_count == 0 ? (n_ready >= need || n_idle == (uint32_t)__popcll(lane_cap)) : n_ready >= (uint32_t)early_ready) {
                        want_pass = true;
                        break;
                    }
                }
                if(ctx.q_count > 0) {
                    const uint32_t take = ctx.q_count < n_idle ? ctx.q_count : n_idle;
                    const uint32_t rank = (uint32_t)__popcll(idle_mask & ((1ULL << lane) - 1ULL));
                    const int src = (int)(rank & 63u);
                    auto from = [src](float v) { return __int_as_float(__builtin_amdgcn_ds_bpermute(src << 2, __float_as_int(v))); };
                    const float4 ro = make_float4(from(win_o.x), from(win_o.y), from(win_o.z), from(win_o.w));
                    const float4 rd = make_float4(from(win_d.x), from(win_d.y), from(win_d.z), from(win_d.w));
                    if(!active && rank < take && __float_as_uint(rd.w) != PT_DEST_NULL) {
                        tr.start(w, rec, root, ro, rd);
                        if(cost_on) {
                            *born_l = w_steps;
                        }
                        active = true;
                        n_rays++;
                        n_shadow += (w.dest & PT_DEST_SHADOW) ? 1u : 0u;
                    }
                    ctx.q_head += take;
                    ctx.q_head = ctx.q_head >= Q.cap ? ctx.q_head - Q.cap : ctx.q_head;
                    ctx.q_count -= take;
                    if(lane < ctx.q_count) {
                        uint32_t i = ctx.q_head + lane;
                        i = i >= Q.cap ? i - Q.cap : i;
                        win_o = Q.ray_o[queue_base + i];
                        win_d = Q.ray_d[queue_base + i];
                    }
                }
            }
            if(__ballot(active) == 0ULL) {
                if(ctx.q_count == 0 && ctx.n_dead >= n_slots) {
                    finished = true;
                    break;
                }
                continue;
            }

#ifdef PT_PATH_TIMING
            const unsigned long long t_b0 = __builtin_amdgcn_s_memtime();
#endif
#pragma unroll 1
            for(int burst = 0; burst < burst_steps; burst++) {
                w_steps++;
                if(!tr.step(w, rec, leaf_min, n_nodes, n_leaves)) {
                    w_steps--;
                    break;
                }
            }
#ifdef PT_PATH_TIMING
            t_burst += __builtin_amdgcn_s_memtime() - t_b0;
#endif
        }
        if(finished) {
            break;
        }
    }

    for(int off = 32; off > 0; off >>= 1) {
        n_rays += __shfl_down(n_rays, off);
        n_shadow += __shfl_down(n_shadow, off);
    }
    if(lane == 0) {
        unsigned long long *slot = A->wave_counters + 8 * (size_t)wave;
        slot[0] += n_nodes;
        slot[1] += n_leaves;
        slot[2] += n_rays;
        slot[3] += n_shadow;
        slot[4] += w_steps;
        slot[5] += w_passes;
        slot[6] += n_samples;
        slot[7] += n_vertices;
#ifdef PT_PATH_TIMING
        slot[5] = (unsigned long long)w_passes | ((t_shade >> 10) << 32);
        slot[4] = (unsigned long long)w_steps | ((t_burst >> 10) << 32);
        slot[3] = (unsigned long long)n_shadow | (((__builtin_amdgcn_s_memtime() - t_begin) >> 10) << 32);
#endif
    }
}

template<int STACK_LDS, bool IN_LDS>
__global__ __launch_bounds__(256) void pt_closest_kernel(PtDevScene sc, const float *__restrict__ rays6, uint32_t n, uint2 *__restrict__ out, uint2 *__restrict__ spill,
                                                         uint32_t spill_depth) {
    extern __shared__ __align__(16) unsigned char lds_raw[];
    const int tid = threadIdx.x;
    lds_u2_ptr stack_l = (lds_u2_ptr)reinterpret_cast<uint2 *>(lds_raw) + tid;
    float4 *lds_recs = reinterpret_cast<float4 *>(lds_raw + (size_t)STACK_LDS * 256 * sizeof(uint2));
    if(IN_LDS) {
        for(uint32_t i = tid; i < 4u * (sc.pair_base + sc.n_pairs); i += 256) {
            lds_recs[i] = sc.recs[i];
        }
        __syncthreads();
    }
    Tracer<STACK_LDS, IN_LDS> tr;
    if(IN_LDS) {
        tr.recs = (typename RecPtr<IN_LDS>::type)(lds_f4_cptr)lds_recs;
    }
    else {
        tr.recs = (typename RecPtr<IN_LDS>::type)(glb_f4_cptr)sc.recs;
    }
    tr.stack_l = stack_l;
    const size_t gid = (size_t)blockIdx.x * 256 + tid;
    tr.my_spill = (glb_u2_ptr)(spill + gid * spill_depth);
    if(gid >= n) {
        return;
    }
    const float *r = rays6 + 6 * gid;
    Walk w;
    typename Tracer<STACK_LDS, IN_LDS>::Rec rec;
    rec.r0 = rec.r1 = rec.r2 = rec.r3 = (f4v){0.0f, 0.0f, 0.0f, 0.0f};
    RootBox root;
    root.ref = sc.root_ref;
    for(int k = 0; k < 3; k++) {
        root.lo[k] = sc.root_lo[k];
        root.hi[k] = sc.root_hi[k];
    }
    tr.start(w, rec, root, make_float4(r[0], r[1], r[2], 0.0f), make_float4(r[3], r[4], r[5], __uint_as_float(0u)));
    uint32_t n_nodes = 0, n_leaves = 0;
    while(tr.step(w, rec, 1, n_nodes, n_leaves)) {
    }
    out[gid] = make_uint2(__float_as_uint(w.best_ref == PT_REF_NONE ? -1.0f : w.best_t), w.best_ref);
}

template<int STACK_LDS, bool IN_LDS, bool kViews>
__global__ __launch_bounds__(256) void pt_feature_kernel(PtDevScene sc, PtDevCamera cam, int32_t width, int32_t height, float4 *__restrict__ out, uint2 *__restrict__ spill,
                                                         uint32_t spill_depth, const PtViewCamera *__restrict__ views, int32_t view_height) {
    extern __shared__ __align__(16) unsigned char lds_raw[];
    const int tid = threadIdx.x;
    lds_u2_ptr stack_l = (lds_u2_ptr)reinterpret_cast<uint2 *>(lds_raw) + tid;
    float4 *lds_recs = reinterpret_cast<float4 *>(lds_raw + (size_t)STACK_LDS * 256 * sizeof(uint2));
    if(IN_LDS) {
        for(uint32_t i = tid; i < 4u * (sc.pair_base + sc.n_pairs); i += 256) {
            lds_recs[i] = sc.recs[i];
        }
        __syncthreads();
    }
    Tracer<STACK_LDS, IN_LDS> tr;
    if(IN_LDS) {
        tr.recs = (typename RecPtr<IN_LDS>::type)(lds_f4_cptr)lds_recs;
    }
    else {
        tr.recs = (typename RecPtr<IN_LDS>::type)(glb_f4_cptr)sc.recs;
    }
    tr.stack_l = stack_l;
    const size_t gid = (size_t)blockIdx.x * 256 + tid;
    tr.my_spill = (glb_u2_ptr)(spill + gid * spill_depth);
    if(gid >= (size_t)width * (size_t)height) {
        return;
    }
    const int32_t px = (int32_t)(gid % (size_t)width);
    int32_t py = (int32_t)(gid / (size_t)width);
    const PtDevCamera *lane_cam = &cam;
    int32_t frame_height = height;
    if constexpr(kViews) {
        const int32_t view = py / view_height;
        py -= view * view_height;
        lane_cam = &views[view].cam;
        frame_height = view_height;
    }
    RootBox root;
    root.ref = sc.root_ref;
    for(int k = 0; k < 3; k++) {
        root.lo[k] = sc.root_lo[k];
        root.hi[k] = sc.root_hi[k];
    }
    float4 acc0 = make_float4(0.0f, 0.0f, 0.0f, 0.0f), acc1 = acc0, acc2 = acc0, emis = acc0;
    for(int k = 0; k < 4; k++) {
        const float dx = (k & 1) ? 0.25f : -0.25f, dy = (k & 2) ? 0.25f : -0.25f;
        const float one_half = 1.0f / 2.0f;
        const float x_camera = 2 * (((float)px + one_half + dx) / (float)width - one_half);
        float y_camera = 2 * (((float)py + one_half + dy) / (float)frame_height - one_half);
        y_camera = -y_camera;
        uint64_t rng = 0;
        const Ray ray = camera_shoot(*lane_cam, x_camera, y_camera, 0.0f, 0.0f, rng);
        Walk w;
        typename Tracer<STACK_LDS, IN_LDS>::Rec rec;
        rec.r0 = rec.r1 = rec.r2 = rec.r3 = (f4v){0.0f, 0.0f, 0.0f, 0.0f};
        tr.start(w, rec, root, make_float4(ray.o.x, ray.o.y, ray.o.z, 0.0f), make_float4(ray.d.x, ray.d.y, ray.d.z, __uint_as_float(0u)));
        uint32_t n_nodes = 0, n_leaves = 0;
        while(tr.step(w, rec, 1, n_nodes, n_leaves)) {
        }
        float4 a = make_float4(0.0f, 0.0f, 0.0f, 0.0f), n4 = a, p4 = a, e4 = a;
        if(w.best_ref != PT_REF_NONE) {
            const float t = w.best_t;
            const V3 pos = ray.o + ray.d * t;
            uint32_t material_index;
            const V3 n = object_normal(sc, w.best_ref, pos, material_index);
            const Material mat = material_load(sc.materials, material_index);
            const bool lambertian = mat.bsdf == 0;
            a = make_float4(lambertian ? mat.diffuse.r : mat.specular.r, lambertian ? mat.diffuse.g : mat.specular.g, lambertian ? mat.diffuse.b : mat.specular.b, 1.0f);
            n4 = make_float4(n.x, n.y, n.z, t);
            p4 = make_float4(pos.x, pos.y, pos.z, 0.0f);
            e4 = make_float4(mat.emission.r, mat.emission.g, mat.emission.b, 0.0f);
        }
        acc0 = make_float4(acc0.x + a.x, acc0.y + a.y, acc0.z + a.z, acc0.w + a.w);
        acc1 = make_float4(acc1.x + n4.x, acc1.y + n4.y, acc1.z + n4.z, acc1.w + n4.w);
        acc2 = make_float4(acc2.x + p4.x, acc2.y + p4.y, acc2.z + p4.z, 0.0f);
        emis = make_float4(emis.x + e4.x, emis.y + e4.y, emis.z + e4.z, 0.0f);
    }
    const float q = 0.25f;
    const float er = emis.x * q, eg = emis.y * q, eb = emis.z * q;
    float4 *o = out + 3 * gid;
    o[0] = make_float4(acc0.x * q, acc0.y * q, acc0.z * q, acc0.w * q);
    o[1] = make_float4(acc1.x * q, acc1.y * q, acc1.z * q, acc1.w * q);
    o[2] = make_float4(acc2.x * q, acc2.y * q, acc2.z * q, (0.2126f * er + 0.7152f * eg) + 0.0722f * eb);
}

template<int STACK_LDS, bool STAMP>
__global__ __launch_bounds__(256) void pt_steptime_kernel(PtDevScene sc, const float *__restrict__ rays6, uint32_t n, uint32_t lanes_per_wave, uint4 *__restrict__ out,
                                                          uint2 *__restrict__ spill, uint32_t spill_depth) {
    extern __shared__ __align__(16) unsigned char lds_raw[];
    const int tid = threadIdx.x;
    const uint32_t lane = (uint32_t)tid & 63u;
    const uint32_t wave = blockIdx.x * 4u + ((uint32_t)tid >> 6);
    Tracer<STACK_LDS, false> tr;
    tr.recs = (glb_f4_cptr)sc.recs;
    tr.stack_l = (lds_u2_ptr)reinterpret_cast<uint2 *>(lds_raw) + tid;
    const size_t gid = (size_t)blockIdx.x * 256 + tid;
    tr.my_spill = (glb_u2_ptr)(spill + gid * spill_depth);
    const uint32_t ray = wave * lanes_per_wave + lane;
    if(lane >= lanes_per_wave || ray >= n) {
        return;
    }
    const float *r = rays6 + 6 * (size_t)ray;
    Walk w;
    typename Tracer<STACK_LDS, false>::Rec rec;
    rec.r0 = rec.r1 = rec.r2 = rec.r3 = (f4v){0.0f, 0.0f, 0.0f, 0.0f};
    RootBox root;
    root.ref = sc.root_ref;
    for(int k = 0; k < 3; k++) {
        root.lo[k] = sc.root_lo[k];
        root.hi[k] = sc.root_hi[k];
    }
    const unsigned long long t_begin = __builtin_amdgcn_s_memtime();
    const unsigned long long t_again = __builtin_amdgcn_s_memtime();
#ifdef PT_STEP_STAMPS
    tr.stamp_last = t_again;
#endif
    tr.start(w, rec, root, make_float4(r[0], r[1], r[2], 0.0f), make_float4(r[3], r[4], r[5], __uint_as_float(0u)));
    uint32_t n_nodes = 0, n_leaves = 0, steps = 0;
    unsigned long long waiting = 0;
    for(;;) {
        if(STAMP) {
            const unsigned long long t1 = __builtin_amdgcn_s_memtime();
            asm volatile("s_waitcnt vmcnt(0) lgkmcnt(0)" ::: "memory");
            const unsigned long long t2 = __builtin_amdgcn_s_memtime();
            asm volatile("s_waitcnt lgkmcnt(0)" ::: "memory");
            waiting += t2 - t1;
        }
        if(!tr.step(w, rec, 1, n_nodes, n_leaves)) {
            break;
        }
        steps += 1u;
    }
    const unsigned long long t_end = __builtin_amdgcn_s_memtime();
    out[ray] = make_uint4(steps, (uint32_t)waiting, (uint32_t)(t_end - t_begin), (uint32_t)(t_again - t_begin));
#ifdef PT_STEP_STAMPS
    unsigned long long *seg = reinterpret_cast<unsigned long long *>(out + n) + 8 * (size_t)ray;
    for(int k = 0; k < 8; k++) {
        seg[k] = tr.stamp_acc[k];
    }
#endif
}

template<int STACK_LDS, int WAVES>
__global__ __launch_bounds__(256, WAVES) void pt_replay_kernel(PtDevScene sc, PtLocalQueue Q, uint32_t n_logs, uint32_t parts, int refill_idle, int burst_steps,
                                                                int leaf_min, uint2 *__restrict__ spill, uint32_t spill_depth,
                                                                unsigned long long *__restrict__ out) {
    extern __shared__ __align__(16) unsigned char lds_raw[];
    const int tid = threadIdx.x;
    const uint32_t lane = (uint32_t)tid & 63u;
    const uint32_t wave = blockIdx.x * 4u + ((uint32_t)tid >> 6);
    if(wave >= n_logs * parts) {
        return;
    }
    Tracer<STACK_LDS, false> tr;
    tr.recs = (glb_f4_cptr)sc.recs;
    tr.stack_l = (lds_u2_ptr)reinterpret_cast<uint2 *>(lds_raw) + tid;
    tr.my_spill = (glb_u2_ptr)(spill + ((size_t)wave * 64 + lane) * spill_depth);
    RootBox root;
    root.ref = sc.root_ref;
    for(int k = 0; k < 3; k++) {
        root.lo[k] = sc.root_lo[k];
        root.hi[k] = sc.root_hi[k];
    }
    const size_t base = (size_t)(wave % n_logs) * Q.cap;
    uint32_t lo = 0, hi = Q.cap;
    while(lo < hi) {
        const uint32_t mid = (lo + hi) / 2;
        if(__float_as_uint(Q.ray_d[base + mid].x) == 0xffffffffu) {
            hi = mid;
        }
        else {
            lo = mid + 1;
        }
    }
    const uint32_t part = wave / n_logs;
    uint32_t pos = (uint32_t)((unsigned long long)lo * part / parts);
    const uint32_t end = (uint32_t)((unsigned long long)lo * (part + 1) / parts);

    bool active = false;
    Walk w;
    w.o = v3(0, 0, 0);
    w.d = v3(0, 0, 1);
    w.inv = v3(0, 0, 0);
    w.pack();
    w.thr = 0.0f;
    w.dest = 0;
    w.best_t = 0.0f;
    w.best_ref = PT_REF_NONE;
    w.set_t_max(FLT_MAX);
    w.cur = PT_REF_NONE;
    w.sp = 0;
    w.occluded = false;
    typename Tracer<STACK_LDS, false>::Rec rec;
    rec.r0 = rec.r1 = rec.r2 = rec.r3 = (f4v){0.0f, 0.0f, 0.0f, 0.0f};
    uint32_t n_nodes = 0, n_leaves = 0, n_rays = 0, checksum = 0, w_steps = 0;
    for(;;) {
        if(active && w.cur == PT_REF_NONE) {
            checksum += (w.dest & PT_DEST_SHADOW) ? (w.occluded ? 1u : 2u) : (w.best_ref ^ __float_as_uint(w.best_t));
            active = false;
        }
        const unsigned long long idle_mask = __ballot(!active);
        const uint32_t n_idle = (uint32_t)__popcll(idle_mask);
        if(n_idle >= (uint32_t)refill_idle && pos < end) {
            const uint32_t left = end - pos;
            const uint32_t take = left < n_idle ? left : n_idle;
            if(!active) {
                const uint32_t rank = (uint32_t)__popcll(idle_mask & ((1ULL << lane) - 1ULL));
                if(rank < take) {
                    const float4 ro = Q.ray_o[base + pos + rank];
                    const float4 rd = Q.ray_d[base + pos + rank];
                    if(__float_as_uint(rd.w) != PT_DEST_NULL) {
                        tr.start(w, rec, root, ro, rd);
                        active = true;
                        n_rays++;
                    }
                }
            }
            pos += take;
        }
        if(__ballot(active) == 0ULL) {
            if(pos >= end) {
                break;
            }
            continue;
        }
#pragma unroll 1
        for(int burst = 0; burst < burst_steps; burst++) {
            w_steps++;
            if(!tr.step(w, rec, leaf_min, n_nodes, n_leaves)) {
                w_steps--;
                break;
            }
        }
    }
    for(int off = 32; off > 0; off >>= 1) {
        n_rays += __shfl_down(n_rays, off);
        checksum += __shfl_down(checksum, off);
    }
    if(lane == 0) {
        atomicAdd(&out[0], (unsigned long long)n_rays);
        atomicAdd(&out[1], (unsigned long long)n_nodes);
        atomicAdd(&out[2], (unsigned long long)n_leaves);
        atomicAdd(&out[3], (unsigned long long)w_steps);
        atomicAdd(&out[4], (unsigned long long)checksum);
    }
}

template<int STACK_LDS, int WAVES>
int launch_replay(hipStream_t stream, const PtDevScene &scene, const PtLocalQueue &Q, uint32_t n_logs, uint32_t parts, const PtPathConfig &cfg, uint2 *spill,
                  unsigned long long *out) {
    const size_t lds = (size_t)STACK_LDS * 256 * sizeof(uint2);
    int blocks = 0;
    if(hipOccupancyMaxActiveBlocksPerMultiprocessor(&blocks, pt_replay_kernel<STACK_LDS, WAVES>, 256, lds) != hipSuccess) {
        blocks = -1;
    }
    const uint32_t waves = n_logs * parts;
    hipLaunchKernelGGL((pt_replay_kernel<STACK_LDS, WAVES>), dim3((waves + 3) / 4), dim3(256), lds, stream, scene, Q, n_logs, parts, cfg.refill_idle,
                       cfg.burst_steps, cfg.leaf_min, spill, cfg.spill_depth, out);
    return blocks;
}

template<bool WIDE, bool IN_LDS, int STACK_LDS>
void launch_path(hipStream_t stream, const PtPathConfig &cfg, const PtPathArgs *d_args) {
    hipLaunchKernelGGL((pt_path_kernel<WIDE, IN_LDS, STACK_LDS>), dim3(cfg.grid), dim3(256), cfg.lds_bytes, stream, d_args);
}

template<bool WIDE, bool IN_LDS, int STACK_LDS>
void occupancy(size_t lds_bytes, int *out) {
    int blocks = 0;
    const hipError_t err = hipOccupancyMaxActiveBlocksPerMultiprocessor(&blocks, pt_path_kernel<WIDE, IN_LDS, STACK_LDS>, 256, lds_bytes);
    *out = (err != hipSuccess || blocks < 1) ? 1 : blocks;
}

template<int STACK_LDS, bool IN_LDS>
void launch_closest(hipStream_t stream, const PtDevScene &scene, const float *rays6, uint32_t n, uint2 *out, const PtPathConfig &cfg) {
    const size_t lds = (size_t)STACK_LDS * 256 * sizeof(uint2) + (IN_LDS ? ((size_t)scene.n_lds_pairs + scene.pair_base) * 64 : 0);
    hipLaunchKernelGGL((pt_closest_kernel<STACK_LDS, IN_LDS>), dim3((n + 255) / 256), dim3(256), lds, stream, scene, rays6, n, out, cfg.spill, cfg.spill_depth);
}

template<int STACK_LDS, bool IN_LDS>
void launch_features(hipStream_t stream, const PtDevScene &scene, const PtDevCamera &cam, int32_t width, int32_t height, float4 *out, const PtPathConfig &cfg,
                     const PtViewCamera *views = nullptr, int32_t view_height = 0) {
    const size_t lds = (size_t)STACK_LDS * 256 * sizeof(uint2) + (IN_LDS ? ((size_t)scene.n_lds_pairs + scene.pair_base) * 64 : 0);
    const size_t n = (size_t)width * (size_t)height;
    if(views != nullptr) {
        hipLaunchKernelGGL((pt_feature_kernel<STACK_LDS, IN_LDS, true>), dim3((unsigned)((n + 255) / 256)), dim3(256), lds, stream, scene, cam, width, height, out,
                           cfg.spill, cfg.spill_depth, views, view_height);
    }
    else {
        hipLaunchKernelGGL((pt_feature_kernel<STACK_LDS, IN_LDS, false>), dim3((unsigned)((n + 255) / 256)), dim3(256), lds, stream, scene, cam, width, height, out,
                           cfg.spill, cfg.spill_depth, nullptr, 0);
    }
}

}

#define PT_DISPATCH_PATH(fn, cfg, ...)                                              \
    do {                                                                            \
        if((cfg).in_lds && (cfg).stack_lds == PT_PATH_STACK_LDS_SMALL) {            \
            if((cfg).wide) {                                                        \
                fn<true, true, PT_PATH_STACK_LDS_SMALL>(__VA_ARGS__);               \
            }                                                                       \
            else {                                                                  \
                fn<false, true, PT_PATH_STACK_LDS_SMALL>(__VA_ARGS__);              \
            }                                                                       \
        }                                                                           \
        else if((cfg).in_lds) {                                                     \
            if((cfg).wide) {                                                        \
                fn<true, true, PT_PATH_STACK_LDS>(__VA_ARGS__);                     \
            }                                                                       \
            else {                                                                  \
                fn<false, true, PT_PATH_STACK_LDS>(__VA_ARGS__);                    \
            }                                                                       \
        }                                                                           \
        else {                                                                      \
            if((cfg).wide) {                                                        \
                fn<true, false, PT_PATH_STACK_LDS>(__VA_ARGS__);                    \
            }                                                                       \
            else {                                                                  \
                fn<false, false, PT_PATH_STACK_LDS>(__VA_ARGS__);                   \
            }                                                                       \
        }                                                                           \
    } while(0)

void pt_launch_path(hipStream_t stream, const PtDevScene &scene, const PtDevCamera &camera, const PtDevOptions &options, PtSlots slots, PtStreams streams,
                    PtLocalQueue queue, const PtPathConfig &cfg, float4 *image, PtDevCounters *counters, PtPathArgs *host_args, PtPathArgs *d_args) {
    PtPathArgs &a = *host_args;
    a.sc = scene;
    a.cam = camera;
    a.opt = options;
    a.S = slots;
    a.T = streams;
    a.Q = queue;
    a.rows = cfg.rows;
    a.slots_per_wave = cfg.slots_per_wave;
    a.refill_idle = cfg.refill_idle;
    a.min_ready = cfg.min_ready;
    a.burst_steps = cfg.burst_steps;
    a.leaf_min = cfg.leaf_min;
    a.ready_shift = cfg.ready_shift;
    a.pass_q_low = cfg.pass_q_low;
    a.early_ready = cfg.early_ready;
    a.compact_passes = cfg.compact_passes;
    a.debug_lanes = cfg.debug_lanes;
    a.spill = cfg.spill;
    a.spill_depth = cfg.spill_depth;
    a.save_stride = (uint32_t)cfg.grid * 256u;
    a.walk_save = cfg.walk_save;
    a.image = image;
    a.counters = counters;
    a.wave_counters = cfg.wave_counters;
    (void)hipMemcpyAsync(d_args, host_args, sizeof(PtPathArgs), hipMemcpyHostToDevice, stream);
    PT_DISPATCH_PATH(launch_path, cfg, stream, cfg, d_args);
}

void pt_launch_steptime(hipStream_t stream, const PtDevScene &scene, const float *rays6, uint32_t n, uint32_t lanes_per_wave, uint4 *out, uint2 *spill, uint32_t spill_depth, int flags) {
    const uint32_t waves = (n + lanes_per_wave - 1) / lanes_per_wave;
    if(flags & 2) {
        hipLaunchKernelGGL((pt_steptime_kernel<8, true>), dim3((waves + 3) / 4), dim3(256), (size_t)8 * 256 * sizeof(uint2), stream, scene, rays6, n, lanes_per_wave, out, spill, spill_depth);
    }
    else {
        hipLaunchKernelGGL((pt_steptime_kernel<8, false>), dim3((waves + 3) / 4), dim3(256), (size_t)8 * 256 * sizeof(uint2), stream, scene, rays6, n, lanes_per_wave, out, spill, spill_depth);
    }
}

void pt_launch_closest(hipStream_t stream, const PtDevScene &scene, const float *rays6, uint32_t n, uint2 *out, const PtPathConfig &cfg) {
    if(n == 0) {
        return;
    }
    if(cfg.in_lds && cfg.stack_lds == PT_PATH_STACK_LDS_SMALL) {
        launch_closest<PT_PATH_STACK_LDS_SMALL, true>(stream, scene, rays6, n, out, cfg);
    }
    else if(cfg.in_lds) {
        launch_closest<PT_PATH_STACK_LDS, true>(stream, scene, rays6, n, out, cfg);
    }
    else {
        launch_closest<PT_PATH_STACK_LDS, false>(stream, scene, rays6, n, out, cfg);
    }
}

void pt_launch_features(hipStream_t stream, const PtDevScene &scene, const PtDevCamera &camera, int32_t width, int32_t height, float4 *out, const PtPathConfig &cfg) {
    if(width <= 0 || height <= 0) {
        return;
    }
    if(cfg.in_lds && cfg.stack_lds == PT_PATH_STACK_LDS_SMALL) {
        launch_features<PT_PATH_STACK_LDS_SMALL, true>(stream, scene, camera, width, height, out, cfg);
    }
    else if(cfg.in_lds) {
        launch_features<PT_PATH_STACK_LDS, true>(stream, scene, camera, width, height, out, cfg);
    }
    else {
        launch_features<PT_PATH_STACK_LDS, false>(stream, scene, camera, width, height, out, cfg);
    }
}

void pt_launch_features_views(hipStream_t stream, const PtDevScene &scene, const PtViewCamera *views, int32_t n_views, int32_t width, int32_t height, float4 *out,
                              const PtPathConfig &cfg) {
    if(width <= 0 || height <= 0 || n_views <= 0) {
        return;
    }
    const PtDevCamera none{};
    const int32_t rows = n_views * height;
    if(cfg.in_lds && cfg.stack_lds == PT_PATH_STACK_LDS_SMALL) {
        launch_features<PT_PATH_STACK_LDS_SMALL, true>(stream, scene, none, width, rows, out, cfg, views, height);
    }
    else if(cfg.in_lds) {
        launch_features<PT_PATH_STACK_LDS, true>(stream, scene, none, width, rows, out, cfg, views, height);
    }
    else {
        launch_features<PT_PATH_STACK_LDS, false>(stream, scene, none, width, rows, out, cfg, views, height);
    }
}

int pt_launch_replay(hipStream_t stream, const PtDevScene &scene, const PtLocalQueue &Q, uint32_t n_logs, uint32_t parts, int waves_per_simd, const PtPathConfig &cfg,
                     uint2 *spill, unsigned long long *out) {
    switch(waves_per_simd) {
    case 4: return launch_replay<8, 4>(stream, scene, Q, n_logs, parts, cfg, spill, out);
    case 5: return launch_replay<8, 5>(stream, scene, Q, n_logs, parts, cfg, spill, out);
    case 6: return launch_replay<8, 6>(stream, scene, Q, n_logs, parts, cfg, spill, out);
    case 7: return launch_replay<8, 7>(stream, scene, Q, n_logs, parts, cfg, spill, out);
    default: return launch_replay<8, 8>(stream, scene, Q, n_logs, parts, cfg, spill, out);
    }
}

size_t pt_path_lds_bytes(int wide, int rows, int stack_lds, uint32_t n_lds_pairs, uint32_t n_lds_leaf_records) {
    const size_t scene = ((size_t)n_lds_pairs + n_lds_leaf_records) * 64;
    return (size_t)stack_lds * 256 * sizeof(uint2) + (size_t)4 * rows * 64 * (sizeof(uint2) + (wide ? sizeof(unsigned long long) : sizeof(uint32_t))) + PT_LDS_TABLE_BYTES + PT_COST_LDS_BYTES + scene;
}

int pt_path_blocks_per_cu(const PtPathConfig &cfg) {
    int blocks = 1;
    PT_DISPATCH_PATH(occupancy, cfg, cfg.lds_bytes, &blocks);
    return blocks;
}

int pt_path_stack_lds(int in_lds, size_t lds_bytes_with_default_window) {
    return (in_lds && lds_bytes_with_default_window > 40960) ? PT_PATH_STACK_LDS_SMALL : PT_PATH_STACK_LDS;
}
```

cpupathtrace_amd/csrc/pt_render.cpp:

```cpp
#include "pt_host.h"

namespace pth {

int setup_path(pt_scene *s) {
    PtPathConfig &cfg = s->path_cfg;
    if(cfg.rows != 0) {
        return PT_OK;
    }
    cfg.in_lds = (s->dev.n_lds_pairs == s->dev.n_pairs && s->dev.n_lds_tris == s->dev.n_tris && s->dev.n_lds_pairs + s->dev.n_lds_tris > 0) ? 1 : 0;
    cfg.wide = s->dev.n_lights + s->dev.n_object_samples > 8U ? 1 : 0;
    cfg.rows = std::min(std::max(env_int("PT_ROWS", 4), 1), PT_MAX_ROWS);
    cfg.stack_lds = pt_path_stack_lds(cfg.in_lds, pt_path_lds_bytes(cfg.wide, cfg.rows, 8, cfg.in_lds ? s->dev.n_lds_pairs : 0U, cfg.in_lds ? s->dev.pair_base : 0U));
    if(cfg.in_lds && env_int("PT_STACK_WINDOW", 0) > 0) {
        cfg.stack_lds = env_int("PT_STACK_WINDOW", 0) <= 4 ? 4 : 8;
    }
    cfg.lds_bytes = pt_path_lds_bytes(cfg.wide, cfg.rows, cfg.stack_lds, cfg.in_lds ? s->dev.n_lds_pairs : 0U, cfg.in_lds ? s->dev.pair_base : 0U);
    const int per_cu = pt_path_blocks_per_cu(cfg);
    const int limit = env_int("PT_BLOCKS_PER_CU", 0);
    s->path_blocks_per_cu = (limit > 0 && limit < per_cu) ? limit : per_cu;
    cfg.spill_depth = s->depth + 2U > static_cast<uint32_t>(cfg.stack_lds) ? s->depth + 2U - static_cast<uint32_t>(cfg.stack_lds) : 1U;
    cfg.refill_idle = std::min(std::max(env_int("PT_REFILL_IDLE", 12), 1), 64);
    cfg.min_ready = std::min(std::max(env_int("PT_MIN_READY", 32), 1), 64 * PT_MAX_ROWS);
    cfg.ready_shift = std::min(std::max(env_int("PT_READY_SHIFT", 1), 0), 31);
    cfg.pass_q_low = std::max(env_int("PT_PASS_Q_LOW", 0), 0);
    cfg.early_ready = std::min(std::max(env_int("PT_EARLY_READY", 0), 0), 64 * PT_MAX_ROWS);
    cfg.compact_passes = env_int("PT_COMPACT", 1) != 0 ? 1 : 0;
    cfg.debug_lanes = std::min(std::max(env_int("PT_DEBUG_LANES", 64), 1), 64);
    cfg.burst_steps = 24;
    cfg.leaf_min = 8;
    if(env_int("PT_DEBUG", 0) != 0) {
        std::fprintf(stderr, "[pt] path kernel: %d CUs x %d workgroups, %d rows of slots per wavefront, stack_lds %d, scene %s, lds %zu B, spill depth %u\n", s->cu_count,
                     s->path_blocks_per_cu, cfg.rows, cfg.stack_lds, cfg.in_lds ? "in LDS" : "in HBM", cfg.lds_bytes, cfg.spill_depth);
    }
    return PT_OK;
}

struct PathPlan {
    uint32_t waves = 0, slots_per_wave = 0;
    const uint32_t *d_place = nullptr;
};

namespace {

int ensure_path_buffers(pt_scene *s, PtPathConfig &cfg, uint32_t waves, uint32_t total, uint32_t cap, uint32_t rays_per_slot, int ring_log) {
    if(static_cast<unsigned long long>(total) * PT_SLOT_PLANES * sizeof(F4) > 0xffffffffULL) {
        return fail(PT_ERR_UNSUPPORTED, "path kernel: " + std::to_string(total) + " slots do not fit the 4 GiB the slot state may occupy");
    }
    PT_HIP(s->sl_state.ensure(static_cast<size_t>(total) * PT_SLOT_PLANES));
    PT_HIP(s->sl_nee.ensure(static_cast<size_t>(total) * std::max<uint32_t>(rays_per_slot - 1U, 1U)));
    PT_HIP(s->sl_nee_mask.ensure(total));
    PT_HIP(s->sl_cost.ensure(total));
    PT_HIP(s->sl_est.ensure(total));
    PT_HIP(s->sl_cand.ensure(static_cast<size_t>(total) * PT_MAX_CANDIDATES));
    PT_HIP(s->lq_ray_o.ensure(static_cast<size_t>(waves) * cap));
    PT_HIP(s->lq_ray_d.ensure(static_cast<size_t>(waves) * cap));
    if(ring_log > 0) {
        PT_HIP(hipMemsetAsync(s->lq_ray_d.ptr, 0xff, static_cast<size_t>(waves) * cap * 4 * sizeof(float), s->stream));
    }
    PT_HIP(s->path_spill.ensure(static_cast<size_t>(waves) * 64U * cfg.spill_depth));
    PT_HIP(s->path_wave_counters.ensure(static_cast<size_t>(waves) * 8U));
    PT_HIP(s->walk_save.ensure(static_cast<size_t>(waves) * 64U * PT_WALK_SAVE_WORDS));
    PT_HIP(s->pull_counter.ensure(64));
    PT_HIP(s->counters.ensure(1));
    cfg.spill = s->path_spill.ptr;
    cfg.walk_save = s->walk_save.ptr;
    cfg.wave_counters = s->path_wave_counters.ptr;
    return PT_OK;
}

}

int ensure_path_workspace(pt_scene *s, uint32_t n, PtPathConfig *out_cfg, const PathPlan *plan) {
    PT_TRY(setup_path(s));
    PtPathConfig cfg = s->path_cfg;
    const uint32_t max_grid = static_cast<uint32_t>(s->cu_count) * static_cast<uint32_t>(s->path_blocks_per_cu);
    const uint32_t spread = std::min<uint32_t>(max_grid * 4U, static_cast<uint32_t>(std::max(env_int("PT_SPREAD_WAVES", 1024), 4)));
    uint32_t waves_wanted = (n + 63U) / 64U;
    if(waves_wanted < spread) {
        waves_wanted = std::min<uint32_t>(spread, n);
    }
    uint32_t grid = std::max<uint32_t>(1U, std::min<uint32_t>(max_grid, (waves_wanted + 3U) / 4U));
    if(plan != nullptr) {
        grid = std::max<uint32_t>(1U, std::min<uint32_t>(max_grid, plan->waves / 4U));
    }
    const uint32_t waves = grid * 4U;
    uint32_t slots_per_wave = std::min<uint32_t>(static_cast<uint32_t>(cfg.rows) * 64U, std::max<uint32_t>(1U, (n + waves - 1U) / waves));
    if(plan != nullptr) {
        if(waves != plan->waves || plan->slots_per_wave == 0 || plan->slots_per_wave > static_cast<uint32_t>(cfg.rows) * 64U) {
            return fail(PT_ERR_INVALID, "placement: " + std::to_string(plan->waves) + " wavefronts x " + std::to_string(plan->slots_per_wave) + " slots do not fit this device");
        }
        slots_per_wave = plan->slots_per_wave;
    }
    const bool single_round = plan != nullptr || (static_cast<uint64_t>(waves) * slots_per_wave >= n && slots_per_wave <= 128U);
    uint32_t first_lanes = plan != nullptr ? 1U : static_cast<uint32_t>(env_int("PT_FIRST_LANES", single_round ? 1 : 8));
    if(first_lanes == 0 || first_lanes > 64 || (first_lanes & (first_lanes - 1U)) != 0) {
        first_lanes = single_round ? 1 : 8;
    }
    if(slots_per_wave % first_lanes != 0) {
        if(slots_per_wave >= 64U) {
            slots_per_wave = (slots_per_wave + first_lanes - 1U) / first_lanes * first_lanes;
        }
        else {
            first_lanes = 1;
        }
    }
    cfg.first_lanes = static_cast<int>(first_lanes);
    int burst_default = 24;
    if(cfg.in_lds) {
        burst_default = slots_per_wave > 64U ? 12 : 24;
    }
    else if(slots_per_wave >= 64U) {
        burst_default = s->depth <= 12U ? 12 : (s->depth <= 18U ? 16 : 24);
    }
    cfg.burst_steps = std::min(std::max(env_int("PT_BURST", burst_default), 1), 64);
    int leaf_default = cfg.in_lds ? (slots_per_wave >= 64U ? 16 : 8) : static_cast<int>(std::min<uint32_t>(std::max<uint32_t>(slots_per_wave / 8U, 2U), 8U));
    if(!cfg.in_lds && slots_per_wave >= 64U && s->depth <= 24U) {
        leaf_default = 12;
    }
    cfg.leaf_min = std::min(std::max(env_int("PT_LEAF_MIN", leaf_default), 1), 64);
    const uint32_t rows = (slots_per_wave + 63U) / 64U;
    const uint32_t total = waves * rows * 64U;
    const uint32_t rays_per_slot = 1U + s->dev.n_lights + s->dev.n_object_samples;
    uint32_t cap = rows * 64U * rays_per_slot;
    const int ring_log = env_int("PT_RING_LOG_RAYS", 0);
    if(ring_log > 0) {
        cap = std::max<uint32_t>(cap, static_cast<uint32_t>(ring_log));
    }
    cfg.grid = static_cast<int>(grid);
    cfg.rows = static_cast<int>(rows);
    cfg.slots_per_wave = static_cast<int>(slots_per_wave);
    PT_TRY(ensure_path_buffers(s, cfg, waves, total, cap, rays_per_slot, ring_log));
    s->path_slots = total;
    s->path_waves = waves;
    s->path_cap = cap;
    s->path_cfg.burst_steps = cfg.burst_steps;
    s->path_cfg.leaf_min = cfg.leaf_min;
    *out_cfg = cfg;
    return PT_OK;
}

RenderStop::RenderStop(pt_render_control *ctl_, Clock::time_point start) : ctl(ctl_ != nullptr ? ctl_ : &none) {
    if(ctl->budget_ms > 0.0) {
        has_deadline = true;
        deadline = start + std::chrono::duration_cast<Clock::duration>(std::chrono::duration<double, std::milli>(ctl->budget_ms));
    }
    poll();
}

void RenderStop::enlist(uint32_t *word) {
    std::lock_guard<std::mutex> lock(mutex);
    __atomic_store_n(word, requested.load() ? 1U : 0U, __ATOMIC_SEQ_CST);
    words.push_back(word);
}

void RenderStop::retire(uint32_t *word, Clock::time_point end) {
    std::lock_guard<std::mutex> lock(mutex);
    words.erase(std::remove(words.begin(), words.end(), word), words.end());
    if(requested.load()) {
        drain_ms = std::max(drain_ms, std::chrono::duration<double, std::milli>(end - requested_at).count());
    }
}

void RenderStop::poll() {
    if(requested.load(std::memory_order_relaxed)) {
        return;
    }
    const Clock::time_point now = Clock::now();
    if(__atomic_load_n(&ctl->cancel, __ATOMIC_ACQUIRE) == 0 && !(has_deadline && now >= deadline)) {
        return;
    }
    std::lock_guard<std::mutex> lock(mutex);
    if(!requested.load()) {
        requested_at = now;
        requested.store(true);
        for(uint32_t *w : words) {
            __atomic_store_n(w, 1U, __ATOMIC_SEQ_CST);
        }
    }
}

namespace {

uint64_t unclaimed_streams(uint64_t n, uint64_t first_total, uint64_t pulled) {
    const uint64_t first = std::min(n, first_total);
    return n - first - std::min(pulled, n - first);
}

int check_tally(bool controlled, const StreamTally &t, uint64_t n) {
    if(controlled && t.finished + t.abandoned + t.unclaimed != n) {
        return fail(PT_ERR_HIP, "path kernel ended with " + std::to_string(t.finished) + " finished, " + std::to_string(t.abandoned) + " abandoned and " +
                                    std::to_string(t.unclaimed) + " unclaimed of " + std::to_string(n) + " streams");
    }
    if(!controlled && t.finished != n) {
        return fail(PT_ERR_HIP, "path kernel ended with " + std::to_string(t.finished) + " of " + std::to_string(n) + " streams finished");
    }
    return PT_OK;
}

}

int finish_path(pt_scene *s, StreamTally *tally) {
    PT_HIP(hipStreamSynchronize(s->stream));
    if(s->host_streams_done == nullptr || s->streams_expected == 0) {
        return PT_OK;
    }
    const volatile unsigned long long *h = static_cast<volatile unsigned long long *>(s->host_streams_done);
    const uint64_t expected = s->streams_expected;
    const bool controlled = s->streams_controlled;
    s->streams_expected = 0;
    s->streams_controlled = false;
    StreamTally t;
    t.finished = h[0];
    if(controlled) {
        t.abandoned = h[1];
        t.unclaimed = unclaimed_streams(expected, s->streams_first_total, static_cast<uint32_t>(h[2]));
    }
    const int rc = check_tally(controlled, t, expected);
    if(rc == PT_OK && controlled && tally != nullptr) {
        *tally = t;
    }
    return rc;
}


namespace {

int path_placement(pt_scene *s, PathPlan *plan) {
    if(s->debug_place.empty()) {
        return PT_OK;
    }
    PT_HIP(s->place.ensure(s->debug_place.size()));
    PT_HIP(hipMemcpyAsync(s->place.ptr, s->debug_place.data(), s->debug_place.size() * sizeof(uint32_t), hipMemcpyHostToDevice, s->stream));
    PT_HIP(hipStreamSynchronize(s->stream));
    plan->waves = s->debug_place_waves;
    plan->slots_per_wave = s->debug_place_slots;
    plan->d_place = s->place.ptr;
    s->debug_place.clear();
    return PT_OK;
}

int path_arguments(pt_scene *s, const PtPathConfig &cfg, const PathPlan *plan, bool watched, PtStreams *streams) {
    PtStreams &T = *streams;
    T.place = plan != nullptr ? plan->d_place : nullptr;
    T.cost = nullptr;
    if(s->debug_collect_costs) {
        PT_HIP(s->stream_cost.ensure(std::max<uint32_t>(T.n, 1U)));
        T.cost = s->stream_cost.ptr;
    }
    T.next = s->pull_counter.ptr;
    T.first_total = plan != nullptr ? T.n : s->path_waves * static_cast<uint32_t>(cfg.slots_per_wave);
    T.n_waves = s->path_waves;
    T.first_spread = env_int("PT_FIRST_SPREAD", 1) != 0 ? 1U : 0U;
    T.first_lanes = static_cast<uint32_t>(cfg.first_lanes);
    T.first_shift = static_cast<uint32_t>(std::max(env_int("PT_FIRST_SHIFT", 1), 0));
    {
        const uint32_t pieces = static_cast<uint32_t>(cfg.slots_per_wave) / T.first_lanes;
        const unsigned long long per_grid_row = static_cast<unsigned long long>(T.chunks_per_tile) * (64U / T.first_lanes) * T.tiles_per_row;
        if(env_int("PT_FIRST_SPREAD", 1) == 2 || per_grid_row == 0 || s->path_waves % per_grid_row != 0 || T.first_total > T.n || (T.tiles_per_row % pieces != 0 && pieces % T.tiles_per_row != 0)) {
            T.tiles_per_row = 0;
        }
    }
    uint32_t *const own_left = T.tile_left;
    T.tile_left = nullptr;
    T.tiles_done = nullptr;
    T.cancel = nullptr;
    if(watched && T.rect == nullptr && T.n_tiles > 0) {
        if(s->host_tiles_done == nullptr) {
            PT_HIP(hipHostMalloc(reinterpret_cast<void **>(&s->host_tiles_done), 64, hipHostMallocDefault));
        }
        *s->host_tiles_done = 0;
        T.tiles_done = s->host_tiles_done;
        T.tile_left = own_left != nullptr ? own_left : s->tile_left.ptr;
    }
    return PT_OK;
}

struct Enlisted {
    RenderStop *stop = nullptr;
    uint32_t *word = nullptr;
    ~Enlisted() {
        if(stop != nullptr) {
            stop->retire(word, RenderStop::Clock::now());
        }
    }
};

int path_launch(pt_scene *s, const PtDevCamera &cam, const PtDevOptions &opt, PtStreams &T, const PtPathConfig &cfg, float4 *d_image, RenderStop *stop, Event &ev_begin,
                Event &ev_end, Enlisted *enlisted) {
    hipStream_t st = s->stream;
    PtSlots S{};
    S.total = s->path_slots;
    S.state = reinterpret_cast<float4 *>(s->sl_state.ptr);
    S.nee = reinterpret_cast<float4 *>(s->sl_nee.ptr);
    S.nee_mask = s->sl_nee_mask.ptr;
    S.cost = s->sl_cost.ptr;
    S.est = s->sl_est.ptr;
    S.cand = s->sl_cand.ptr;
    PtLocalQueue Q{};
    Q.ray_o = reinterpret_cast<float4 *>(s->lq_ray_o.ptr);
    Q.ray_d = reinterpret_cast<float4 *>(s->lq_ray_d.ptr);
    Q.cap = s->path_cap;
    PT_HIP(hipMemsetAsync(s->counters.ptr, 0, sizeof(PtDevCounters), st));
    PT_HIP(hipMemsetAsync(s->pull_counter.ptr, 0, 64 * sizeof(uint32_t), st));
    PT_HIP(hipMemsetAsync(s->path_wave_counters.ptr, 0, static_cast<size_t>(s->path_waves) * 8U * sizeof(unsigned long long), st));
    PT_HIP(ev_begin.create());
    PT_HIP(ev_end.create());
    PT_HIP(hipEventRecord(ev_begin.e, st));
    PT_HIP(s->path_args.ensure(1));
    if(stop != nullptr) {
        if(s->host_cancel == nullptr) {
            PT_HIP(hipHostMalloc(reinterpret_cast<void **>(&s->host_cancel), 64, hipHostMallocCoherent | hipHostMallocMapped));
            PT_HIP(hipHostGetDevicePointer(reinterpret_cast<void **>(&s->dev_cancel), s->host_cancel, 0));
        }
        T.cancel = s->dev_cancel;
        enlisted->stop = stop;
        enlisted->word = s->host_cancel;
        stop->enlist(s->host_cancel);
    }
    pt_launch_path(st, s->dev, cam, opt, S, T, Q, cfg, d_image, s->counters.ptr, &s->host_path_args, s->path_args.ptr);
    PT_HIP(hipGetLastError());
    PT_HIP(hipEventRecord(ev_end.e, st));
    if(s->host_streams_done == nullptr) {
        PT_HIP(hipHostMalloc(reinterpret_cast<void **>(&s->host_streams_done), 64, hipHostMallocDefault));
    }
    *s->host_streams_done = ~0ULL;
    s->streams_expected = T.n;
    PT_HIP(hipMemcpyAsync(s->host_streams_done, &s->counters.ptr->streams_done, sizeof(unsigned long long), hipMemcpyDeviceToHost, st));
    s->streams_controlled = stop != nullptr;
    if(stop != nullptr) {
        s->host_streams_done[1] = ~0ULL;
        s->host_streams_done[2] = ~0ULL;
        s->streams_first_total = T.first_total;
        PT_HIP(hipMemcpyAsync(s->host_streams_done + 1, &s->counters.ptr->streams_abandoned, sizeof(unsigned long long), hipMemcpyDeviceToHost, st));
        PT_HIP(hipMemcpyAsync(s->host_streams_done + 2, s->pull_counter.ptr, sizeof(uint32_t), hipMemcpyDeviceToHost, st));
    }
    return PT_OK;
}

int path_host_loop(pt_scene *s, const PtStreams &T, Event &ev_end, pt_progress_fn progress, void *progress_user, RenderStop *stop, Enlisted *enlisted) {
    const int total = static_cast<int>(T.n_tiles);
    int reported = 0;
    for(;;) {
        const hipError_t q = hipEventQuery(ev_end.e);
        const int done = std::min(static_cast<int>(*static_cast<volatile uint32_t *>(s->host_tiles_done)), total);
        while(progress != nullptr && reported < done) {
            progress(++reported, total, progress_user);
        }
        if(q == hipSuccess) {
            break;
        }
        if(q != hipErrorNotReady) {
            return fail(PT_ERR_HIP, std::string("path kernel: ") + hipGetErrorString(q));
        }
        if(stop != nullptr) {
            stop->poll();
        }
        std::this_thread::sleep_for(std::chrono::microseconds(500));
    }
    if(stop != nullptr) {
        stop->retire(s->host_cancel, RenderStop::Clock::now());
        enlisted->stop = nullptr;
    }
    return PT_OK;
}

void print_path_stats(const pt_scene *s, const PtPathConfig &cfg, float ms, const unsigned long long *sum, const std::vector<unsigned long long> &slots) {
    std::fprintf(stderr, "[pt] path kernel: %.2f ms, grid %d x 256, %d rows; wave steps %llu (%.1f lanes of 64 busy per step), shading passes %llu, rays %llu\n", ms, cfg.grid,
                 cfg.rows, sum[4], sum[4] ? static_cast<double>(sum[0] + sum[1]) / static_cast<double>(sum[4]) : 0.0, sum[5], sum[2]);
    std::vector<unsigned long long> steps(s->path_waves);
    for(size_t w = 0; w < steps.size(); w++) {
        steps[w] = slots[8 * w + 4] & 0xffffffffULL;
    }
    std::sort(steps.begin(), steps.end());
    const double mean = static_cast<double>(sum[4]) / static_cast<double>(steps.size());
    std::fprintf(stderr, "[pt] wave steps per wavefront: mean %.0f, min %llu, median %llu, 90 %% %llu, 99 %% %llu, max %llu (max / mean %.3f)\n", mean, steps.front(),
                 steps[steps.size() / 2], steps[steps.size() * 9 / 10], steps[steps.size() * 99 / 100], steps.back(), static_cast<double>(steps.back()) / mean);
}

int path_stats(pt_scene *s, const PtStreams &T, const PtPathConfig &cfg, bool controlled, Event &ev_begin, Event &ev_end, pt_stats *stats) {
    PT_HIP(hipEventSynchronize(ev_end.e));
    float ms = 0.0F;
    PT_HIP(hipEventElapsedTime(&ms, ev_begin.e, ev_end.e));
    std::vector<unsigned long long> slots(static_cast<size_t>(s->path_waves) * 8U);
    PT_HIP(hipMemcpy(slots.data(), s->path_wave_counters.ptr, slots.size() * sizeof(unsigned long long), hipMemcpyDeviceToHost));
    unsigned long long sum[8] = {0, 0, 0, 0, 0, 0, 0, 0}, kcycles[3] = {0, 0, 0};
    for(size_t i = 0; i < slots.size(); i++) {
        const size_t k = i & 7U;
        sum[k] += (k >= 3 && k <= 5) ? (slots[i] & 0xffffffffULL) : slots[i];
        if(k >= 3 && k <= 5) {
            kcycles[k - 3] += slots[i] >> 32;
        }
    }
    if(kcycles[0] != 0 && env_int("PT_DEBUG", 0) != 0) {
        std::fprintf(stderr, "[pt] wave time: %.1f %% in shading passes, %.1f %% in traversal bursts (of the waves' lifetimes; %llu kilo-cycles in all)\n",
                     100.0 * static_cast<double>(kcycles[2]) / static_cast<double>(kcycles[0]), 100.0 * static_cast<double>(kcycles[1]) / static_cast<double>(kcycles[0]), kcycles[0]);
    }
    PtDevCounters done{};
    PT_HIP(hipMemcpy(&done, s->counters.ptr, sizeof(done), hipMemcpyDeviceToHost));
    StreamTally t;
    t.finished = done.streams_done;
    if(controlled) {
        uint32_t pulled = 0;
        PT_HIP(hipMemcpy(&pulled, s->pull_counter.ptr, sizeof(pulled), hipMemcpyDeviceToHost));
        t.abandoned = done.streams_abandoned;
        t.unclaimed = unclaimed_streams(T.n, T.first_total, pulled);
    }
    PT_TRY(check_tally(controlled, t, T.n));
    stats->node_visits = sum[0];
    stats->leaf_tests = sum[1];
    stats->rays_traced = sum[2];
    stats->shadow_rays_traced = sum[3];
    stats->samples = sum[6];
    stats->vertices = sum[7];
    stats->launches = 1;
    stats->kernel_ms = ms;
    stats->wave_steps = sum[4];
    stats->shading_passes = sum[5];
    stats->wavefronts = s->path_waves;
    stats->slot_rows = static_cast<uint64_t>(cfg.rows);
    if(env_int("PT_DEBUG", 0) != 0) {
        print_path_stats(s, cfg, ms, sum, slots);
    }
    return PT_OK;
}

}

int run_path(pt_scene *s, const PtDevCamera &cam, const PtDevOptions &opt, PtStreams T, float4 *d_image, pt_stats *stats, pt_progress_fn progress, void *progress_user,
             RenderStop *stop) {
    PathPlan placed;
    PT_TRY(path_placement(s, &placed));
    const PathPlan *plan = placed.d_place != nullptr ? &placed : nullptr;
    PtPathConfig cfg;
    PT_TRY(ensure_path_workspace(s, T.n, &cfg, plan));
    PT_TRY(path_arguments(s, cfg, plan, progress != nullptr || stop != nullptr, &T));
    Event ev_begin, ev_end;
    Enlisted enlisted;
    PT_TRY(path_launch(s, cam, opt, T, cfg, d_image, stop, ev_begin, ev_end, &enlisted));
    if(T.tiles_done != nullptr) {
        PT_TRY(path_host_loop(s, T, ev_end, progress, progress_user, stop, &enlisted));
    }
    if(stats != nullptr) {
        PT_TRY(path_stats(s, T, cfg, stop != nullptr, ev_begin, ev_end, stats));
    }
    return PT_OK;
}

}

using namespace pth;

extern "C" int pt_debug_collect_costs(pt_scene *s, int on) {
    if(s == nullptr) {
        return fail(PT_ERR_INVALID, "null scene");
    }
    s->debug_collect_costs = on != 0;
    return PT_OK;
}

extern "C" int pt_debug_stream_costs(pt_scene *s, uint32_t *out, size_t n) {
    if(s == nullptr || out == nullptr || n > s->stream_cost.count) {
        return fail(PT_ERR_INVALID, "no costs of that many streams");
    }
    PT_HIP(hipSetDevice(s->device));
    PT_HIP(hipStreamSynchronize(s->stream));
    PT_HIP(hipMemcpy(out, s->stream_cost.ptr, n * sizeof(uint32_t), hipMemcpyDeviceToHost));
    return PT_OK;
}

extern "C" int pt_debug_set_place(pt_scene *s, uint32_t waves, uint32_t slots_per_wave, const uint32_t *table) {
    if(s == nullptr || table == nullptr || waves == 0 || waves % 4U != 0 || slots_per_wave == 0) {
        return fail(PT_ERR_INVALID, "placement table");
    }
    s->debug_place.assign(table, table + static_cast<size_t>(waves) * slots_per_wave);
    s->debug_place_waves = waves;
    s->debug_place_slots = slots_per_wave;
    return PT_OK;
}

extern "C" int pt_debug_step_timing(pt_scene *s, const float *rays, size_t n, int lanes_per_wave, int flags, uint32_t *out) {
    if(s == nullptr || rays == nullptr || out == nullptr || n == 0 || n > 0x3fffffULL || lanes_per_wave < 1 || lanes_per_wave > 64) {
        return fail(PT_ERR_INVALID, "bad argument");
    }
    std::lock_guard<std::mutex> lock(s->render_mutex);
    PT_HIP(hipSetDevice(s->device));
    PT_TRY(setup_path(s));
    if(s->path_cfg.in_lds) {
        return fail(PT_ERR_UNSUPPORTED, "step timing is for scenes in HBM");
    }
    const size_t waves = (n + static_cast<size_t>(lanes_per_wave) - 1) / static_cast<size_t>(lanes_per_wave);
    const size_t threads = (waves + 3) / 4 * 256;
    DevBuf<float> d_rays;
    DevBuf<uint4> d_out;
    DevBuf<uint2> d_spill;
    PT_HIP(d_rays.ensure(6 * n));
    PT_HIP(d_out.ensure(5 * n));
    PT_HIP(hipMemsetAsync(d_out.ptr, 0, 5 * n * sizeof(uint4), s->stream));
    PT_HIP(d_spill.ensure(threads * s->path_cfg.spill_depth));
    hipStream_t st = s->stream;
    PT_HIP(hipMemcpyAsync(d_rays.ptr, rays, 6 * n * sizeof(float), hipMemcpyHostToDevice, st));
    pt_launch_steptime(st, s->dev, d_rays.ptr, static_cast<uint32_t>(n), static_cast<uint32_t>(lanes_per_wave), d_out.ptr, d_spill.ptr, s->path_cfg.spill_depth, flags);
    PT_HIP(hipGetLastError());
    PT_HIP(hipMemcpyAsync(out, d_out.ptr, 5 * n * sizeof(uint4), hipMemcpyDeviceToHost, st));
    PT_HIP(hipStreamSynchronize(st));
    return PT_OK;
}

extern "C" int pt_debug_replay_rays(pt_scene *s, int waves_per_simd, int parts, unsigned long long *out, float *out_ms, int *out_blocks) {
    if(s == nullptr || out == nullptr || out_ms == nullptr || out_blocks == nullptr || parts < 1 || s->path_waves == 0) {
        return fail(PT_ERR_INVALID, "nothing to replay");
    }
    std::lock_guard<std::mutex> lock(s->render_mutex);
    PT_HIP(hipSetDevice(s->device));
    PtPathConfig cfg = s->path_cfg;
    const uint32_t waves = s->path_waves * static_cast<uint32_t>(parts);
    PT_HIP(s->path_spill.ensure(static_cast<size_t>(waves) * 64U * cfg.spill_depth));
    PT_HIP(s->path_wave_counters.ensure(8));
    PT_HIP(hipMemsetAsync(s->path_wave_counters.ptr, 0, 8 * sizeof(unsigned long long), s->stream));
    PtLocalQueue Q{};
    Q.ray_o = reinterpret_cast<float4 *>(s->lq_ray_o.ptr);
    Q.ray_d = reinterpret_cast<float4 *>(s->lq_ray_d.ptr);
    Q.cap = s->path_cap;
    Event e0, e1;
    PT_HIP(e0.create());
    PT_HIP(e1.create());
    PT_HIP(hipEventRecord(e0.e, s->stream));
    *out_blocks = pt_launch_replay(s->stream, s->dev, Q, s->path_waves, static_cast<uint32_t>(parts), waves_per_simd, cfg, s->path_spill.ptr, s->path_wave_counters.ptr);
    PT_HIP(hipGetLastError());
    PT_HIP(hipEventRecord(e1.e, s->stream));
    PT_HIP(hipMemcpyAsync(out, s->path_wave_counters.ptr, 5 * sizeof(unsigned long long), hipMemcpyDeviceToHost, s->stream));
    PT_HIP(hipStreamSynchronize(s->stream));
    PT_HIP(hipEventElapsedTime(out_ms, e0.e, e1.e));
    return PT_OK;
}

extern "C" {

int pt_render_streams(pt_scene *s, const pt_camera_params *camera, const pt_options *options, const pt_stream *streams, size_t n, float *out_image,
                      uint64_t *out_states, pt_stats *stats) {
    PT_TRY(check_render_args(s, camera, options));
    if(n > 0 && (streams == nullptr || out_image == nullptr)) {
        return fail(PT_ERR_INVALID, "null argument");
    }
    if(stats != nullptr) {
        std::memset(stats, 0, sizeof(*stats));
    }
    if(n == 0) {
        return PT_OK;
    }
    if(n > 0x0fffffffULL) {
        return fail(PT_ERR_INVALID, "too many streams");
    }
    PtDevOptions opt;
    PT_TRY(derive_options(options, &opt));
    const PtDevCamera cam = derive_camera(camera);
    std::vector<int4> rects(n);
    std::vector<uint64_t> states(n);
    for(size_t i = 0; i < n; i++) {
        const pt_stream &t = streams[i];
        if(t.w < 0 || t.h < 0 || t.x < 0 || t.y < 0 || t.x + t.w > options->image_width || t.y + t.h > options->image_height) {
            return fail(PT_ERR_INVALID, "stream rectangle outside the image");
        }
        rects[i] = make_int4(t.x, t.y, t.w, t.h);
        states[i] = t.rng_state;
    }
    std::lock_guard<std::mutex> lock(s->render_mutex);
    PT_HIP(hipSetDevice(s->device));
    const uint32_t n32 = static_cast<uint32_t>(n);
    const size_t pixels = static_cast<size_t>(options->image_width) * static_cast<size_t>(options->image_height);
    PT_HIP(s->image.ensure(pixels));
    hipStream_t st = s->stream;
    {
        PT_HIP(s->st_rect.ensure(n));
        PT_HIP(s->st_rng.ensure(n));
        PT_HIP(hipMemcpyAsync(s->image.ptr, out_image, pixels * sizeof(F4), hipMemcpyHostToDevice, st));
        PT_HIP(hipMemcpyAsync(s->st_rect.ptr, rects.data(), n * sizeof(int4), hipMemcpyHostToDevice, st));
        PT_HIP(hipMemcpyAsync(s->st_rng.ptr, states.data(), n * sizeof(uint64_t), hipMemcpyHostToDevice, st));
        PtStreams T{};
        T.n = n32;
        T.rect = s->st_rect.ptr;
        T.rng = s->st_rng.ptr;
        const int rc = run_path(s, cam, opt, T, reinterpret_cast<float4 *>(s->image.ptr), stats, nullptr, nullptr);
        if(rc != PT_OK) {
            (void)hipStreamSynchronize(st);
            return rc;
        }
        PT_HIP(hipMemcpyAsync(out_image, s->image.ptr, pixels * sizeof(F4), hipMemcpyDeviceToHost, st));
        if(out_states != nullptr) {
            PT_HIP(hipMemcpyAsync(out_states, s->st_rng.ptr, n * sizeof(uint64_t), hipMemcpyDeviceToHost, st));
        }
        return finish_path(s);
    }
}

}

namespace pth {

void tile_grid(const pt_tile *tiles, size_t n_tiles, uint32_t *tiles_per_row, uint32_t *chunks_per_tile) {
    *tiles_per_row = 0;
    *chunks_per_tile = 0;
    if(n_tiles > 0 && (static_cast<uint32_t>(tiles[0].w) * static_cast<uint32_t>(tiles[0].h)) % 64U == 0) {
        bool regular = true;
        uint32_t per_row = 0;
        for(size_t k = 0; k < n_tiles && regular; k++) {
            regular = tiles[k].w == tiles[0].w && tiles[k].h == tiles[0].h;
            if(per_row == 0 && k > 0 && tiles[k].y != tiles[0].y) {
                per_row = static_cast<uint32_t>(k);
            }
        }
        if(per_row == 0) {
            per_row = static_cast<uint32_t>(n_tiles);
        }
        for(size_t k = 0; k < n_tiles && regular; k++) {
            regular = tiles[k].x == tiles[0].x + static_cast<int32_t>(k % per_row) * tiles[0].w && tiles[k].y == tiles[0].y + static_cast<int32_t>(k / per_row) * tiles[0].h;
        }
        if(regular && n_tiles % per_row == 0 && per_row % 4 == 0) {
            *tiles_per_row = per_row;
            *chunks_per_tile = static_cast<uint32_t>(tiles[0].w) * static_cast<uint32_t>(tiles[0].h) / 64U;
        }
    }
}

int check_tiles(const pt_tile *tiles, size_t n_tiles, int32_t width, int32_t rows, uint64_t *total, const char *unit) {
    uint64_t pixels = 0;
    for(size_t k = 0; k < n_tiles; k++) {
        const pt_tile &t = tiles[k];
        if(t.w <= 0 || t.h <= 0 || t.x < 0 || t.y < 0 || t.x + t.w > width || t.y + t.h > rows) {
            return fail(PT_ERR_INVALID, "tile outside the image or empty");
        }
        pixels += static_cast<uint64_t>(t.w) * static_cast<uint64_t>(t.h);
    }
    if(total != nullptr) {
        if(pixels > 0x0fffffffULL) {
            return fail(PT_ERR_INVALID, std::string("too many pixels in one ") + unit);
        }
        *total = pixels;
    }
    return PT_OK;
}

TileTable::TileTable(const pt_tile *tiles, size_t n_tiles) : rects(n_tiles), offsets(n_tiles), left(n_tiles) {
    uint32_t at = 0;
    for(size_t k = 0; k < n_tiles; k++) {
        const pt_tile &t = tiles[k];
        rects[k] = make_int4(t.x, t.y, t.w, t.h);
        offsets[k] = at;
        left[k] = static_cast<uint32_t>(t.w) * static_cast<uint32_t>(t.h);
        at += left[k];
    }
}

void set_tile_streams(PtStreams *T, uint32_t n, const int4 *d_tiles, const uint32_t *d_offset, size_t n_tiles, uint64_t base_seed, int32_t n_views, int32_t view_height,
                      const PtViewCamera *d_view_cams, const uint64_t *d_view_seeds) {
    T->n = n;
    T->tiles = d_tiles;
    T->tile_offset = d_offset;
    T->n_tiles = static_cast<uint32_t>(n_tiles);
    T->base_seed = base_seed;
    if(n_views > 1) {
        T->n_views = static_cast<uint32_t>(n_views);
        T->view_height = static_cast<uint32_t>(view_height);
        T->views = d_view_cams;
        T->view_seed = d_view_seeds;
    }
}

}

static int render_tiles_impl(pt_scene *s, const pt_camera_params *camera, const pt_options *options, const pt_tile *tiles, size_t n_tiles, uint64_t base_seed,
                             float4 *d_image, pt_stats *stats, pt_progress_fn progress = nullptr, void *progress_user = nullptr, RenderStop *stop = nullptr,
                             const ViewSet *views = nullptr) {
    PtDevOptions opt;
    PT_TRY(derive_options(options, &opt));
    const PtDevCamera cam = derive_camera(camera);
    const int32_t rows = views != nullptr ? views->rows(options) : options->image_height;
    uint64_t total = 0;
    PT_TRY(check_tiles(tiles, n_tiles, options->image_width, rows, &total));
    const TileTable table(tiles, n_tiles);
    PT_HIP(s->tiles.ensure(n_tiles));
    PT_HIP(s->tile_offset.ensure(n_tiles));
    hipStream_t st = s->stream;
    PT_HIP(hipMemcpyAsync(s->tiles.ptr, table.rects.data(), n_tiles * sizeof(int4), hipMemcpyHostToDevice, st));
    PT_HIP(hipMemcpyAsync(s->tile_offset.ptr, table.offsets.data(), n_tiles * sizeof(uint32_t), hipMemcpyHostToDevice, st));
    if(progress != nullptr || stop != nullptr) {
        PT_HIP(s->tile_left.ensure(n_tiles));
        PT_HIP(hipMemcpyAsync(s->tile_left.ptr, table.left.data(), n_tiles * sizeof(uint32_t), hipMemcpyHostToDevice, st));
    }
    if(views != nullptr) {
        PT_HIP(s->view_cams.ensure(views->cams.size()));
        PT_HIP(s->view_seeds.ensure(views->seeds.size()));
        PT_HIP(hipMemcpyAsync(s->view_cams.ptr, views->cams.data(), views->cams.size() * sizeof(PtViewCamera), hipMemcpyHostToDevice, st));
        PT_HIP(hipMemcpyAsync(s->view_seeds.ptr, views->seeds.data(), views->seeds.size() * sizeof(uint64_t), hipMemcpyHostToDevice, st));
    }
    PT_HIP(hipStreamSynchronize(st));
    PtStreams T{};
    set_tile_streams(&T, static_cast<uint32_t>(total), s->tiles.ptr, s->tile_offset.ptr, n_tiles, base_seed, views != nullptr ? static_cast<int32_t>(views->cams.size()) : 1,
                     options->image_height, s->view_cams.ptr, s->view_seeds.ptr);
    tile_grid(tiles, n_tiles, &T.tiles_per_row, &T.chunks_per_tile);
    return run_path(s, cam, opt, T, d_image, stats, progress, progress_user, stop);
}

extern "C" {

int pt_render_tiles(pt_scene *s, const pt_camera_params *camera, const pt_options *options, const pt_tile *tiles, size_t n_tiles, uint64_t base_seed,
                    float *out_image, pt_stats *stats) {
    return pt_render_tiles_progress(s, camera, options, tiles, n_tiles, base_seed, out_image, stats, nullptr, nullptr);
}

int pt_render_tiles_progress(pt_scene *s, const pt_camera_params *camera, const pt_options *options, const pt_tile *tiles, size_t n_tiles, uint64_t base_seed,
                             float *out_image, pt_stats *stats, pt_progress_fn progress, void *progress_user) {
    PT_TRY(check_render_args(s, camera, options));
    if(stats != nullptr) {
        std::memset(stats, 0, sizeof(*stats));
    }
    if(n_tiles == 0) {
        return PT_OK;
    }
    if(tiles == nullptr || out_image == nullptr) {
        return fail(PT_ERR_INVALID, "null argument");
    }
    std::lock_guard<std::mutex> lock(s->render_mutex);
    PT_HIP(hipSetDevice(s->device));
    const size_t pixels = static_cast<size_t>(options->image_width) * static_cast<size_t>(options->image_height);
    PT_HIP(s->image.ensure(pixels));
    PT_HIP(hipMemcpyAsync(s->image.ptr, out_image, pixels * sizeof(F4), hipMemcpyHostToDevice, s->stream));
    PT_TRY(render_tiles_impl(s, camera, options, tiles, n_tiles, base_seed, reinterpret_cast<float4 *>(s->image.ptr), stats, progress, progress_user));
    PT_HIP(hipMemcpyAsync(out_image, s->image.ptr, pixels * sizeof(F4), hipMemcpyDeviceToHost, s->stream));
    return finish_path(s);
}

int pt_render_item(pt_scene *s, const pt_camera_params *camera, const pt_options *options, const pt_stream *item, float *out_tile, uint64_t *out_state,
                   pt_stats *stats) {
    PT_TRY(check_render_args(s, camera, options));
    if(item == nullptr) {
        return fail(PT_ERR_INVALID, "null argument");
    }
    if(stats != nullptr) {
        std::memset(stats, 0, sizeof(*stats));
    }
    if(item->w < 0 || item->h < 0 || item->x < 0 || item->y < 0 || item->x + item->w > options->image_width || item->y + item->h > options->image_height) {
        return fail(PT_ERR_INVALID, "work item outside the image");
    }
    if(out_state != nullptr) {
        *out_state = item->rng_state;
    }
    if(item->w == 0 || item->h == 0) {
        return PT_OK;
    }
    if(out_tile == nullptr) {
        return fail(PT_ERR_INVALID, "null argument");
    }
    PtDevOptions opt;
    PT_TRY(derive_options(options, &opt));
    const PtDevCamera cam = derive_camera(camera);
    std::lock_guard<std::mutex> lock(s->render_mutex);
    PT_HIP(hipSetDevice(s->device));
    const size_t pixels = static_cast<size_t>(options->image_width) * static_cast<size_t>(options->image_height);
    PT_HIP(s->image.ensure(pixels));
    PT_HIP(s->st_rect.ensure(1));
    PT_HIP(s->st_rng.ensure(1));
    hipStream_t st = s->stream;
    const int4 rect = make_int4(item->x, item->y, item->w, item->h);
    PT_HIP(hipMemcpyAsync(s->st_rect.ptr, &rect, sizeof(rect), hipMemcpyHostToDevice, st));
    PT_HIP(hipMemcpyAsync(s->st_rng.ptr, &item->rng_state, sizeof(uint64_t), hipMemcpyHostToDevice, st));
    PT_HIP(hipStreamSynchronize(st));
    PtStreams T{};
    T.n = 1;
    T.rect = s->st_rect.ptr;
    T.rng = s->st_rng.ptr;
    PT_TRY(run_path(s, cam, opt, T, reinterpret_cast<float4 *>(s->image.ptr), stats, nullptr, nullptr));
    const F4 *first = s->image.ptr + static_cast<size_t>(item->y) * static_cast<size_t>(options->image_width) + static_cast<size_t>(item->x);
    PT_HIP(hipMemcpy2DAsync(out_tile, static_cast<size_t>(item->w) * sizeof(F4), first, static_cast<size_t>(options->image_width) * sizeof(F4),
                            static_cast<size_t>(item->w) * sizeof(F4), static_cast<size_t>(item->h), hipMemcpyDeviceToHost, st));
    if(out_state != nullptr) {
        PT_HIP(hipMemcpyAsync(out_state, s->st_rng.ptr, sizeof(uint64_t), hipMemcpyDeviceToHost, st));
    }
    return finish_path(s);
}

}

namespace pth {

std::vector<int> tile_owners(const pt_tile *tiles, size_t n_tiles, int n_scenes) {
    size_t per_row = 0;
    while(per_row < n_tiles && tiles[per_row].y == tiles[0].y) {
        per_row++;
    }
    const bool diagonal = n_scenes > 1 && per_row > 0 && n_tiles % per_row == 0 && per_row % static_cast<size_t>(n_scenes) == 0;
    std::vector<int> owners(n_tiles);
    for(size_t k = 0; k < n_tiles; k++) {
        owners[k] = static_cast<int>((diagonal ? k % per_row + k / per_row : k) % static_cast<size_t>(n_scenes));
    }
    return owners;
}

int for_each_replica(int n, const std::function<int(int)> &fn) {
    std::vector<int> rcs(static_cast<size_t>(n), PT_OK);
    std::vector<std::string> errors(static_cast<size_t>(n));
    auto work = [&](int i) {
        rcs[static_cast<size_t>(i)] = fn(i);
        if(rcs[static_cast<size_t>(i)] != PT_OK) {
            errors[static_cast<size_t>(i)] = last_error();
        }
    };
    std::vector<std::thread> threads;
    for(int i = 1; i < n; i++) {
        threads.emplace_back(work, i);
    }
    work(0);
    for(std::thread &t : threads) {
        t.join();
    }
    for(int i = 0; i < n; i++) {
        if(rcs[static_cast<size_t>(i)] != PT_OK) {
            return fail(rcs[static_cast<size_t>(i)], "scene " + std::to_string(i) + ": " + errors[static_cast<size_t>(i)]);
        }
    }
// ... 228 lines not shown
```

Measured before the change: 470.7.

## Use non-power-of-two LDS stack ring window for HBM scenes

Replaces the mask-indexed LDS traversal stack window with a ring buffer tracked by an explicit position, so the window size no longer has to be a power of two. HBM-resident, non-wide scenes now get an 11-entry window, and wide ones keep 8. The aim is fewer spills of the BVH stack to global memory, paid for with more LDS per wave and extra ring-position bookkeeping. Auxiliary kernels keep the old window and get a spill depth enlarged by the difference. Optional stack-event counters are compiled in only under a debug macro.

```diff
diff --git a/cpupathtrace_amd/csrc/pt_api.cpp b/cpupathtrace_amd/csrc/pt_api.cpp
--- a/cpupathtrace_amd/csrc/pt_api.cpp
+++ b/cpupathtrace_amd/csrc/pt_api.cpp
@@ -693,7 +693,7 @@
         PtPathConfig cfg = s->path_cfg;
         PT_HIP(s->batch_rays.ensure(6 * n));
         PT_HIP(s->closest_out.ensure(n));
-        PT_HIP(s->path_spill.ensure(((n + 255) / 256) * 256 * cfg.spill_depth));
+        PT_HIP(s->path_spill.ensure(((n + 255) / 256) * 256 * pt_aux_spill_depth(cfg)));
         cfg.spill = s->path_spill.ptr;
         hipStream_t st = s->stream;
         PT_HIP(hipMemcpyAsync(s->batch_rays.ptr, rays, 6 * n * sizeof(float), hipMemcpyHostToDevice, st));
diff --git a/cpupathtrace_amd/csrc/pt_image.cpp b/cpupathtrace_amd/csrc/pt_image.cpp
--- a/cpupathtrace_amd/csrc/pt_image.cpp
+++ b/cpupathtrace_amd/csrc/pt_image.cpp
@@ -50,7 +50,7 @@
     cam.aperture_kind = PT_APERTURE_NONE;
     PtPathConfig cfg = s->path_cfg;
     const size_t n = static_cast<size_t>(options->image_width) * static_cast<size_t>(options->image_height);
-    PT_HIP(s->feature_spill.ensure(((n + 255) / 256) * 256 * cfg.spill_depth));
+    PT_HIP(s->feature_spill.ensure(((n + 255) / 256) * 256 * pt_aux_spill_depth(cfg)));
     cfg.spill = s->feature_spill.ptr;
     pt_launch_features(s->stream, s->dev, cam, options->image_width, options->image_height, d_out, cfg);
     PT_HIP(hipGetLastError());
@@ -87,7 +87,7 @@
     PT_HIP(hipStreamSynchronize(s->stream));
     PtPathConfig cfg = s->path_cfg;
     const size_t n = static_cast<size_t>(n_views) * static_cast<size_t>(options->image_width) * static_cast<size_t>(options->image_height);
-    PT_HIP(s->feature_spill.ensure(((n + 255) / 256) * 256 * cfg.spill_depth));
+    PT_HIP(s->feature_spill.ensure(((n + 255) / 256) * 256 * pt_aux_spill_depth(cfg)));
     cfg.spill = s->feature_spill.ptr;
     pt_launch_features_views(s->stream, s->dev, s->feature_cams.ptr, n_views, options->image_width, options->image_height, d_out, cfg);
     PT_HIP(hipGetLastError());
diff --git a/cpupathtrace_amd/csrc/pt_kernels.h b/cpupathtrace_amd/csrc/pt_kernels.h
--- a/cpupathtrace_amd/csrc/pt_kernels.h
+++ b/cpupathtrace_amd/csrc/pt_kernels.h
@@ -78,6 +78,10 @@
     uint32_t cap;
 };
 
+struct PtPathConfig;
+int pt_aux_stack_lds(const PtPathConfig &cfg);
+uint32_t pt_aux_spill_depth(const PtPathConfig &cfg);
+
 struct PtPathConfig {
     int grid;
     int rows;
@@ -143,7 +147,7 @@
 int pt_launch_frame_scatter(hipStream_t stream, const float4 *rgba, const int2 *at, uint32_t n, float4 *view, int32_t *samples);
 int pt_path_blocks_per_cu(const PtPathConfig &cfg);
 size_t pt_path_lds_bytes(int wide, int rows, int stack_lds, uint32_t n_lds_pairs, uint32_t n_lds_leaf_records);
-int pt_path_stack_lds(int in_lds, size_t lds_bytes_with_default_window);
+int pt_path_stack_lds(int in_lds, int wide, size_t lds_bytes_with_default_window);
 int pt_launch_replay(hipStream_t stream, const PtDevScene &scene, const PtLocalQueue &Q, uint32_t n_logs, uint32_t parts, int waves_per_simd, const PtPathConfig &cfg,
                      uint2 *spill, unsigned long long *out);
 void pt_launch_closest(hipStream_t stream, const PtDevScene &scene, const float *rays6, uint32_t n, uint2 *out, const PtPathConfig &cfg);
diff --git a/cpupathtrace_amd/csrc/pt_path.hip b/cpupathtrace_amd/csrc/pt_path.hip
--- a/cpupathtrace_amd/csrc/pt_path.hip
+++ b/cpupathtrace_amd/csrc/pt_path.hip
@@ -48,6 +48,7 @@
     float t_lim;
     uint32_t cur;
     uint32_t sp;
+    uint32_t pos;
     bool occluded;
 
     PT_D void pack() {
@@ -76,9 +77,38 @@
 #define PT_STAMP(k) do { } while(0)
 #endif
 
+#ifdef PT_STACK_COUNTS
+#define PT_STACK_COUNT_LDS 1024
+__device__ unsigned long long pt_stack_counts[64];
+#define PT_COUNT_EVENT(k, cond) count_event(k, cond)
+#define PT_COUNT_LANES(k, cond) count_lanes(k, cond)
+#else
+#define PT_STACK_COUNT_LDS 0
+#define PT_COUNT_EVENT(k, cond) do { } while(0)
+#define PT_COUNT_LANES(k, cond) do { } while(0)
+#endif
+
 template<int STACK_LDS, bool IN_LDS>
 struct Tracer {
-    static_assert((STACK_LDS & (STACK_LDS - 1)) == 0, "the stack window is indexed with a mask");
+#ifdef PT_STACK_COUNTS
+    lds_u32_ptr cnt_l = nullptr;
+    bool cnt_on = false;
+    PT_D void count_event(uint32_t k, bool cond) const {
+        if(cnt_on) {
+            const unsigned long long m = __ballot(cond);
+            const uint32_t l = __builtin_amdgcn_mbcnt_hi(~0u, __builtin_amdgcn_mbcnt_lo(~0u, 0u));
+            if(cond && (m & ((1ULL << l) - 1ULL)) == 0ULL) {
+                __hip_atomic_fetch_add(&cnt_l[k], 1u, __ATOMIC_RELAXED, __HIP_MEMORY_SCOPE_WORKGROUP);
+            }
+        }
+    }
+    PT_D void count_lanes(uint32_t k, bool cond) const {
+        if(cnt_on && cond) {
+            __hip_atomic_fetch_add(&cnt_l[k], 1u, __ATOMIC_RELAXED, __HIP_MEMORY_SCOPE_WORKGROUP);
+        }
+    }
+#endif
+    static_assert(STACK_LDS >= 2, "the slot above the top and the top itself are two slots");
 #ifdef PT_STEP_STAMPS
     mutable unsigned long long stamp_acc[8] = {0, 0, 0, 0, 0, 0, 0, 0}, stamp_last = 0;
 #endif
@@ -86,6 +116,10 @@
     rec_ptr recs;
     lds_u2_ptr stack_l;
     glb_u2_ptr my_spill;
+
+    static PT_D uint32_t ring_next(uint32_t pos) { return pos == (uint32_t)STACK_LDS - 1u ? 0u : pos + 1u; }
+    static PT_D uint32_t ring_prev(uint32_t pos) { return (pos == 0u ? (uint32_t)STACK_LDS : pos) - 1u; }
+    static PT_D uint32_t ring_of(uint32_t sp) { return sp % (uint32_t)STACK_LDS; }
 
     struct Rec {
         f4v r0, r1, r2, r3;
@@ -119,8 +153,10 @@
         const u2v sentinel = {sent_ref, sent_t};
         stack_l[0] = sentinel;
         w.sp = 1;
+        w.pos = 1u;
         w.occluded = false;
         w.cur = PT_REF_NONE;
+        PT_COUNT_LANES(13, true);
         if(root.ref != PT_REF_NONE) {
             const float t_root = slab_walk(ld3(root.lo), ld3(root.hi), w.o, w.inv);
             if(t_root >= 0.0f) {
@@ -138,10 +174,14 @@
         asm volatile("s_waitcnt vmcnt(0)" ::: "memory");
 #endif
         PT_STAMP(2);
+        const uint32_t sp = w.sp, slot = w.pos;
+        uint32_t top_slot = ring_prev(slot), next_slot = ring_next(slot);
+        asm volatile("" : "+v"(top_slot), "+v"(next_slot));
+        lds_u2_ptr top_p = stack_l + top_slot * 256u, slot_p = stack_l + slot * 256u;
+        asm volatile("" : "+v"(top_p), "+v"(slot_p));
         whole(R);
         const f4v q0 = R.r0, q1 = R.r1, q2 = R.r2;
-        const uint32_t sp = w.sp;
-        const u2v top = stack_l[((sp - 1u) & (uint32_t)(STACK_LDS - 1)) * 256u];
+        const u2v top = *top_p;
         const f2v a0 = ((f2v){q0.x, q0.y} - w.o_xy) * w.i_xy;
         const f2v a1 = ((f2v){q0.z, q0.w} - w.o_zx) * w.i_zx;
         const f2v a2 = ((f2v){q1.x, q1.y} - w.o_yz) * w.i_yz;
@@ -165,28 +205,35 @@
         const float near_t = __builtin_fminf(tl, tr), far_t = __builtin_fmaxf(tl, tr);
         const u2v far = {left_first ? right_ref : left_ref, __float_as_uint(far_t)};
         const bool both = far_t < inf, entered = near_t < inf;
-        const uint32_t slot = (sp & (uint32_t)(STACK_LDS - 1)) * 256u;
+        PT_COUNT_EVENT(2, both && sp >= (uint32_t)STACK_LDS);
+        PT_COUNT_LANES(7, both && sp >= (uint32_t)STACK_LDS);
+        PT_COUNT_LANES(10, both);
+        PT_COUNT_LANES(16u + (sp < 32u ? sp : 32u), both);
+        PT_COUNT_EVENT(3, !entered && sp - 1u >= (uint32_t)STACK_LDS);
+        PT_COUNT_LANES(8, !entered && sp - 1u >= (uint32_t)STACK_LDS);
+        PT_COUNT_LANES(12, !entered);
         if(deep_mask == 0ULL) {
-            stack_l[slot] = far;
+            *slot_p = far;
         }
         else if(both) {
             if(sp >= (uint32_t)STACK_LDS) {
-                my_spill[sp - STACK_LDS] = stack_l[slot];
-            }
-            stack_l[slot] = far;
+                my_spill[sp - STACK_LDS] = *slot_p;
+            }
+            *slot_p = far;
         }
         const uint32_t popped = __uint_as_float(top.y) <= t_lim ? top.x : PT_REF_POPPING;
         const uint32_t next = entered ? near_ref : popped;
         w.sp = entered ? sp + (both ? 1u : 0u) : sp - 1u;
+        w.pos = entered ? (both ? next_slot : slot) : top_slot;
         w.cur = next;
-        asm volatile("" ::"v"(w.sp), "v"(w.cur));
+        asm volatile("" ::"v"(w.sp), "v"(w.pos), "v"(w.cur));
         PT_STAMP(3);
         if(next < PT_REF_POPPING) {
             fetch(next, R);
         }
         if(deep_mask != 0ULL) {
             if(!entered & (sp - 1u >= (uint32_t)STACK_LDS)) {
-                stack_l[((sp - 1u) & (uint32_t)(STACK_LDS - 1)) * 256u] = my_spill[sp - 1u - STACK_LDS];
+                *top_p = my_spill[sp - 1u - STACK_LDS];
             }
         }
         PT_STAMP(4);
@@ -226,15 +273,20 @@
             }
         }
         if(__ballot(need_pop) != 0ULL) {
-            uint32_t sp = w.sp;
+            uint32_t sp = w.sp, slot = w.pos;
             const float t_max = w.t_max;
+            PT_COUNT_EVENT(6, true);
             while(__ballot(need_pop) != 0ULL) {
+                PT_COUNT_EVENT(4, need_pop);
+                PT_COUNT_LANES(11, need_pop);
+                PT_COUNT_EVENT(5, need_pop && sp - 1u >= (uint32_t)STACK_LDS);
+                PT_COUNT_LANES(9, need_pop && sp - 1u >= (uint32_t)STACK_LDS);
                 if(need_pop) {
                     sp--;
-                    const uint32_t slot = (sp & (uint32_t)(STACK_LDS - 1)) * 256u;
-                    const u2v e = stack_l[slot];
+                    slot = ring_prev(slot);
+                    const u2v e = stack_l[slot * 256u];
                     if(sp >= (uint32_t)STACK_LDS) {
-                        stack_l[slot] = my_spill[sp - STACK_LDS];
+                        stack_l[slot * 256u] = my_spill[sp - STACK_LDS];
                     }
                     if(__uint_as_float(e.y) < t_max) {
                         cur = e.x;
@@ -244,6 +296,7 @@
                 }
             }
             w.sp = sp;
+            w.pos = slot;
         }
         w.cur = cur;
         if(moved & (cur != PT_REF_NONE)) {
@@ -261,6 +314,8 @@
         PT_STAMP(1);
         if(nodes != 0ULL) {
             n_nodes += (uint32_t)__popcll(nodes);
+            PT_COUNT_EVENT(0, true);
+            PT_COUNT_EVENT(1, (nodes & __builtin_amdgcn_uicmp(w.sp, (uint32_t)STACK_LDS, 35)) != 0ULL);
             node_step(w, R, nodes, nodes & __builtin_amdgcn_uicmp(w.sp, (uint32_t)STACK_LDS, 35));
         }
         PT_STAMP(5);
@@ -900,6 +955,10 @@
 
 
 #define PT_PATH_STACK_LDS 8
+#ifndef PT_PATH_STACK_HBM
+#define PT_PATH_STACK_HBM 11
+#endif
+#define PT_PATH_STACK_HBM_WIDE 8
 #define PT_PATH_STACK_LDS_SMALL 4
 #ifndef PT_COST_LDS_BYTES
 #define PT_COST_LDS_BYTES 1024
@@ -956,6 +1015,11 @@
     typedef unsigned char __attribute__((address_space(3))) *lds_u8_ptr;
     lds_u8_ptr list_l = (lds_u8_ptr)reinterpret_cast<unsigned char *>(at) + wave_in_block * 256u;
     at += (size_t)PT_COST_LDS_BYTES;
+#ifdef PT_STACK_COUNTS
+    const lds_u32_ptr count_base = (lds_u32_ptr)reinterpret_cast<uint32_t *>(at) + wave_in_block * 64u;
+    ((lds_u32_ptr)reinterpret_cast<uint32_t *>(at))[tid] = 0u;
+    at += (size_t)PT_STACK_COUNT_LDS;
+#endif
     float4 *lds_recs = reinterpret_cast<float4 *>(at);
     const bool cost_on = PT_COST_LDS_BYTES != 0 && A->T.cost != nullptr;
     uint32_t *const slot_cost = A->S.cost;
@@ -1004,6 +1068,10 @@
     __syncthreads();
 
     Tracer<STACK_LDS, IN_LDS> tr;
+#ifdef PT_STACK_COUNTS
+    tr.cnt_l = count_base;
+    tr.cnt_on = true;
+#endif
     if(IN_LDS) {
         tr.recs = (typename RecPtr<IN_LDS>::type)(lds_f4_cptr)lds_recs;
     }
@@ -1041,6 +1109,7 @@
     w.set_t_max(FLT_MAX);
     w.cur = PT_REF_NONE;
     w.sp = 0;
+    w.pos = 0;
     w.occluded = false;
     typename Tracer<STACK_LDS, IN_LDS>::Rec rec;
     rec.r0 = rec.r1 = rec.r2 = rec.r3 = (f4v){0.0f, 0.0f, 0.0f, 0.0f};
@@ -1167,6 +1236,7 @@
             asm volatile("" : "+s"(bind_offset));
             bind_lane((const PtPathArgs *)(args_c4)((const char __attribute__((address_space(4))) *)A4 + bind_offset), lane_afresh());
         }
+        w.pos = tr.ring_of(w.sp);
         bool finished = false;
         for(;;) {
             if(active && w.cur == PT_REF_NONE) {
@@ -1257,6 +1327,9 @@
         }
     }
 
+#ifdef PT_STACK_COUNTS
+    atomicAdd(&pt_stack_counts[lane_afresh()], (unsigned long long)count_base[lane_afresh()]);
+#endif
     for(int off = 32; off > 0; off >>= 1) {
         n_rays += __shfl_down(n_rays, off);
         n_shadow += __shfl_down(n_shadow, off);
@@ -1512,6 +1585,7 @@
     w.set_t_max(FLT_MAX);
     w.cur = PT_REF_NONE;
     w.sp = 0;
+    w.pos = 0;
     w.occluded = false;
     typename Tracer<STACK_LDS, false>::Rec rec;
     rec.r0 = rec.r1 = rec.r2 = rec.r3 = (f4v){0.0f, 0.0f, 0.0f, 0.0f};
@@ -1578,7 +1652,7 @@
     }
     const uint32_t waves = n_logs * parts;
     hipLaunchKernelGGL((pt_replay_kernel<STACK_LDS, WAVES>), dim3((waves + 3) / 4), dim3(256), lds, stream, scene, Q, n_logs, parts, cfg.refill_idle,
-                       cfg.burst_steps, cfg.leaf_min, spill, cfg.spill_depth, out);
+                       cfg.burst_steps, cfg.leaf_min, spill, pt_aux_spill_depth(cfg), out);
     return blocks;
 }
 
@@ -1597,7 +1671,7 @@
 template<int STACK_LDS, bool IN_LDS>
 void launch_closest(hipStream_t stream, const PtDevScene &scene, const float *rays6, uint32_t n, uint2 *out, const PtPathConfig &cfg) {
     const size_t lds = (size_t)STACK_LDS * 256 * sizeof(uint2) + (IN_LDS ? ((size_t)scene.n_lds_pairs + scene.pair_base) * 64 : 0);
-    hipLaunchKernelGGL((pt_closest_kernel<STACK_LDS, IN_LDS>), dim3((n + 255) / 256), dim3(256), lds, stream, scene, rays6, n, out, cfg.spill, cfg.spill_depth);
+    hipLaunchKernelGGL((pt_closest_kernel<STACK_LDS, IN_LDS>), dim3((n + 255) / 256), dim3(256), lds, stream, scene, rays6, n, out, cfg.spill, pt_aux_spill_depth(cfg));
 }
 
 template<int STACK_LDS, bool IN_LDS>
@@ -1607,11 +1681,11 @@
     const size_t n = (size_t)width * (size_t)height;
     if(views != nullptr) {
         hipLaunchKernelGGL((pt_feature_kernel<STACK_LDS, IN_LDS, true>), dim3((unsigned)((n + 255) / 256)), dim3(256), lds, stream, scene, cam, width, height, out,
-                           cfg.spill, cfg.spill_depth, views, view_height);
+                           cfg.spill, pt_aux_spill_depth(cfg), views, view_height);
     }
     else {
         hipLaunchKernelGGL((pt_feature_kernel<STACK_LDS, IN_LDS, false>), dim3((unsigned)((n + 255) / 256)), dim3(256), lds, stream, scene, cam, width, height, out,
-                           cfg.spill, cfg.spill_depth, nullptr, 0);
+                           cfg.spill, pt_aux_spill_depth(cfg), nullptr, 0);
     }
 }
 
@@ -1637,10 +1711,10 @@
         }                                                                           \
         else {                                                                      \
             if((cfg).wide) {                                                        \
-                fn<true, false, PT_PATH_STACK_LDS>(__VA_ARGS__);                    \
+                fn<true, false, PT_PATH_STACK_HBM_WIDE>(__VA_ARGS__);               \
             }                                                                       \
             else {                                                                  \
-                fn<false, false, PT_PATH_STACK_LDS>(__VA_ARGS__);                   \
+                fn<false, false, PT_PATH_STACK_HBM>(__VA_ARGS__);                   \
             }                                                                       \
         }                                                                           \
     } while(0)
@@ -1674,6 +1748,20 @@
     a.wave_counters = cfg.wave_counters;
     (void)hipMemcpyAsync(d_args, host_args, sizeof(PtPathArgs), hipMemcpyHostToDevice, stream);
     PT_DISPATCH_PATH(launch_path, cfg, stream, cfg, d_args);
+#ifdef PT_STACK_COUNTS
+    {
+        unsigned long long c[64];
+        const unsigned long long zero[64] = {};
+        if(hipStreamSynchronize(stream) == hipSuccess && hipMemcpyFromSymbol(c, HIP_SYMBOL(pt_stack_counts), sizeof(c)) == hipSuccess) {
+            std::fprintf(stderr, "[pt] stack counts W=%d:", cfg.stack_lds);
+            for(int k = 0; k < 49; k++) {
+                std::fprintf(stderr, " %llu", c[k]);
+            }
+            std::fprintf(stderr, "\n");
+        }
+        (void)hipMemcpyToSymbol(HIP_SYMBOL(pt_stack_counts), zero, sizeof(zero));
+    }
+#endif
 }
 
 void pt_launch_steptime(hipStream_t stream, const PtDevScene &scene, const float *rays6, uint32_t n, uint32_t lanes_per_wave, uint4 *out, uint2 *spill, uint32_t spill_depth, int flags) {
@@ -1747,7 +1835,7 @@
 
 size_t pt_path_lds_bytes(int wide, int rows, int stack_lds, uint32_t n_lds_pairs, uint32_t n_lds_leaf_records) {
     const size_t scene = ((size_t)n_lds_pairs + n_lds_leaf_records) * 64;
-    return (size_t)stack_lds * 256 * sizeof(uint2) + (size_t)4 * rows * 64 * (sizeof(uint2) + (wide ? sizeof(unsigned long long) : sizeof(uint32_t))) + PT_LDS_TABLE_BYTES + PT_COST_LDS_BYTES + scene;
+    return (size_t)stack_lds * 256 * sizeof(uint2) + (size_t)4 * rows * 64 * (sizeof(uint2) + (wide ? sizeof(unsigned long long) : sizeof(uint32_t))) + PT_LDS_TABLE_BYTES + PT_COST_LDS_BYTES + PT_STACK_COUNT_LDS + scene;
 }
 
 int pt_path_blocks_per_cu(const PtPathConfig &cfg) {
@@ -1756,6 +1844,18 @@
     return blocks;
 }
 
-int pt_path_stack_lds(int in_lds, size_t lds_bytes_with_default_window) {
-    return (in_lds && lds_bytes_with_default_window > 40960) ? PT_PATH_STACK_LDS_SMALL : PT_PATH_STACK_LDS;
-}
+int pt_path_stack_lds(int in_lds, int wide, size_t lds_bytes_with_default_window) {
+    if(!in_lds) {
+        return wide ? PT_PATH_STACK_HBM_WIDE : PT_PATH_STACK_HBM;
+    }
+    return lds_bytes_with_default_window > 40960 ? PT_PATH_STACK_LDS_SMALL : PT_PATH_STACK_LDS;
+}
+
+int pt_aux_stack_lds(const PtPathConfig &cfg) {
+    return (cfg.in_lds && cfg.stack_lds == PT_PATH_STACK_LDS_SMALL) ? PT_PATH_STACK_LDS_SMALL : PT_PATH_STACK_LDS;
+}
+
+uint32_t pt_aux_spill_depth(const PtPathConfig &cfg) {
+    const int aux = pt_aux_stack_lds(cfg);
+    return cfg.spill_depth + (uint32_t)(cfg.stack_lds > aux ? cfg.stack_lds - aux : 0);
+}
diff --git a/cpupathtrace_amd/csrc/pt_render.cpp b/cpupathtrace_amd/csrc/pt_render.cpp
--- a/cpupathtrace_amd/csrc/pt_render.cpp
+++ b/cpupathtrace_amd/csrc/pt_render.cpp
@@ -10,7 +10,7 @@
     cfg.in_lds = (s->dev.n_lds_pairs == s->dev.n_pairs && s->dev.n_lds_tris == s->dev.n_tris && s->dev.n_lds_pairs + s->dev.n_lds_tris > 0) ? 1 : 0;
     cfg.wide = s->dev.n_lights + s->dev.n_object_samples > 8U ? 1 : 0;
     cfg.rows = std::min(std::max(env_int("PT_ROWS", 4), 1), PT_MAX_ROWS);
-    cfg.stack_lds = pt_path_stack_lds(cfg.in_lds, pt_path_lds_bytes(cfg.wide, cfg.rows, 8, cfg.in_lds ? s->dev.n_lds_pairs : 0U, cfg.in_lds ? s->dev.pair_base : 0U));
+    cfg.stack_lds = pt_path_stack_lds(cfg.in_lds, cfg.wide, pt_path_lds_bytes(cfg.wide, cfg.rows, 8, cfg.in_lds ? s->dev.n_lds_pairs : 0U, cfg.in_lds ? s->dev.pair_base : 0U));
     if(cfg.in_lds && env_int("PT_STACK_WINDOW", 0) > 0) {
         cfg.stack_lds = env_int("PT_STACK_WINDOW", 0) <= 4 ? 4 : 8;
     }
@@ -29,7 +29,7 @@
     cfg.burst_steps = 24;
     cfg.leaf_min = 8;
     if(env_int("PT_DEBUG", 0) != 0) {
-        std::fprintf(stderr, "[pt] path kernel: %d CUs x %d workgroups, %d rows of slots per wavefront, stack_lds %d, scene %s, lds %zu B, spill depth %u\n", s->cu_count,
+        std::fprintf(stderr, "[pt] path kernel: %d CUs x %d workgroups, %d rows of slots per wavefront, stack window W = %d, scene %s, lds %zu B, spill depth %u\n", s->cu_count,
                      s->path_blocks_per_cu, cfg.rows, cfg.stack_lds, cfg.in_lds ? "in LDS" : "in HBM", cfg.lds_bytes, cfg.spill_depth);
     }
     return PT_OK;
@@ -496,10 +496,10 @@
     PT_HIP(d_rays.ensure(6 * n));
     PT_HIP(d_out.ensure(5 * n));
     PT_HIP(hipMemsetAsync(d_out.ptr, 0, 5 * n * sizeof(uint4), s->stream));
-    PT_HIP(d_spill.ensure(threads * s->path_cfg.spill_depth));
+    PT_HIP(d_spill.ensure(threads * pt_aux_spill_depth(s->path_cfg)));
     hipStream_t st = s->stream;
     PT_HIP(hipMemcpyAsync(d_rays.ptr, rays, 6 * n * sizeof(float), hipMemcpyHostToDevice, st));
-    pt_launch_steptime(st, s->dev, d_rays.ptr, static_cast<uint32_t>(n), static_cast<uint32_t>(lanes_per_wave), d_out.ptr, d_spill.ptr, s->path_cfg.spill_depth, flags);
+    pt_launch_steptime(st, s->dev, d_rays.ptr, static_cast<uint32_t>(n), static_cast<uint32_t>(lanes_per_wave), d_out.ptr, d_spill.ptr, pt_aux_spill_depth(s->path_cfg), flags);
     PT_HIP(hipGetLastError());
     PT_HIP(hipMemcpyAsync(out, d_out.ptr, 5 * n * sizeof(uint4), hipMemcpyDeviceToHost, st));
     PT_HIP(hipStreamSynchronize(st));
@@ -514,7 +514,7 @@
     PT_HIP(hipSetDevice(s->device));
     PtPathConfig cfg = s->path_cfg;
     const uint32_t waves = s->path_waves * static_cast<uint32_t>(parts);
-    PT_HIP(s->path_spill.ensure(static_cast<size_t>(waves) * 64U * cfg.spill_depth));
+    PT_HIP(s->path_spill.ensure(static_cast<size_t>(waves) * 64U * pt_aux_spill_depth(cfg)));
     PT_HIP(s->path_wave_counters.ensure(8));
     PT_HIP(hipMemsetAsync(s->path_wave_counters.ptr, 0, 8 * sizeof(unsigned long long), s->stream));
     PtLocalQueue Q{};
```

After: 473.9, median of 6. About the same (+0.7%).
